# chzchzchz/raftsql

Hardware: AMD Instinct MI355X
Metric: quorum decisions/sec (commit+vote) across G groups (higher is better)
Workload: dtype u64

## Files before the change

### go/raftq/engine_more.go

```go
package raftq

import "C"

import "unsafe"

func ABIVersion() int { return int(C.raftq_abi_version()) }

func Quorum(peers uint32) uint32 { return uint32(C.raftq_quorum(C.uint32_t(peers))) }

func (e *Engine) NGroups() uint64 { return uint64(C.raftq_groups(e.h)) }
func (e *Engine) NPeers() uint32  { return uint32(C.raftq_peers(e.h)) }

func (e *Engine) SelfMax() (int, error) {
	var slot C.int32_t
	if err := e.err(C.raftq_self_max(e.h, &slot)); err != nil {
		return -1, err
	}
	return int(slot), nil
}

func (e *Engine) SetStream(stream unsafe.Pointer) error { return e.err(C.raftq_set_stream(e.h, stream)) }
func (e *Engine) Stream() unsafe.Pointer                { return C.raftq_get_stream(e.h) }

type TermDelta struct{ Group, CurTerm, FirstIdxCurTerm uint64 }

func (e *Engine) ApplyTermDeltas(d []TermDelta) error {
	if len(d) == 0 {
		return nil
	}
	return e.err(C.raftq_apply_term_deltas(e.h, (*C.raftq_term_delta_t)(unsafe.Pointer(&d[0])), C.uint64_t(len(d))))
}

func (e *Engine) CommitAdvance(gated bool, committedOut []uint64) (changed uint64, err error) {
	var p *C.uint64_t
	if committedOut != nil {
		p = (*C.uint64_t)(unsafe.Pointer(&committedOut[0]))
	}
	g := C.int(0)
	if gated {
		g = 1
	}
	var n C.uint64_t
	err = e.err(C.raftq_commit_advance(e.h, g, p, &n))
	return uint64(n), err
}

func (e *Engine) VoteTally(outcomeOut []uint8) (Counts, error) {
	var p *C.uint8_t
	if outcomeOut != nil {
		p = (*C.uint8_t)(unsafe.Pointer(&outcomeOut[0]))
	}
	var c C.raftq_counts_t
	if err := e.err(C.raftq_vote_tally(e.h, p, &c)); err != nil {
		return Counts{}, err
	}
	return Counts{uint64(c.n_changed), uint64(c.n_won), uint64(c.n_lost)}, nil
}

func (e *Engine) ReadVotes(out []uint8) error {
	return e.err(C.raftq_read_votes(e.h, (*C.uint8_t)(unsafe.Pointer(&out[0]))))
}

func (e *Engine) SetTimers(electionTick, heartbeatTick uint32, seed uint64) error {
	return e.err(C.raftq_set_timers(e.h, C.uint32_t(electionTick), C.uint32_t(heartbeatTick), C.uint64_t(seed)))
}

type TickCounts struct{ Hup, Beat uint64 }

func (e *Engine) Tick(wantCounts bool) (TickCounts, error) {
	var c C.raftq_tick_counts_t
	if !wantCounts {
		return TickCounts{}, e.err(C.raftq_tick(e.h, nil))
	}
	err := e.err(C.raftq_tick(e.h, &c))
	return TickCounts{uint64(c.n_hup), uint64(c.n_beat)}, err
}

func (e *Engine) CollectHups(out []uint64) (uint64, error) {
	var n C.uint64_t
	var p *C.uint64_t
	if len(out) > 0 {
		p = (*C.uint64_t)(unsafe.Pointer(&out[0]))
	}
	rc := C.raftq_collect_hups(e.h, p, C.uint64_t(len(out)), &n)
	return uint64(n), e.err(rc)
}

func (e *Engine) TickCollect(hups, beats []uint64) (nHup, nBeat uint64, err error) {
	var hp, bp *C.uint64_t
	if len(hups) > 0 {
		hp = (*C.uint64_t)(unsafe.Pointer(&hups[0]))
	}
	if len(beats) > 0 {
		bp = (*C.uint64_t)(unsafe.Pointer(&beats[0]))
	}
	var nh, nb C.uint64_t
	err = e.err(C.raftq_tick_collect(e.h, hp, C.uint64_t(len(hups)), &nh, bp, C.uint64_t(len(beats)), &nb))
	return uint64(nh), uint64(nb), err
}

const TickBeatBitmap = uint(C.RAFTQ_TICK_BEAT_BITMAP)

// ... 202 lines not shown
```

### include/raftq.h

```cpp
#ifndef RAFTQ_H
#define RAFTQ_H

#include <stddef.h>
#include <stdint.h>

#ifdef __cplusplus
extern "C" {
#endif

#define RAFTQ_ABI_VERSION 1
#define RAFTQ_MAX_PEERS 9

#define RAFTQ_OK 0
#define RAFTQ_EINVAL (-1)
#define RAFTQ_ENOMEM (-2)
#define RAFTQ_EHIP (-3)
#define RAFTQ_ESTATE (-4)
#define RAFTQ_ENODEV (-5)

#define RAFTQ_SWEEP_COMMIT 0x01u
#define RAFTQ_SWEEP_GATED 0x02u
#define RAFTQ_SWEEP_VOTES 0x04u
#define RAFTQ_SWEEP_NO_ADOPT 0x08u
#define RAFTQ_SWEEP_LDS 0x10u
// ... 14 lines not shown
typedef struct raftq_delta {
  uint64_t group;
  uint64_t match;
  uint32_t peer;
  uint32_t _pad;
} raftq_delta_t;

typedef struct raftq_vote_delta {
  uint64_t group;
  uint32_t peer;
  uint8_t vote;
  uint8_t _pad[3];
} raftq_vote_delta_t;

typedef struct raftq_term_delta {
  uint64_t group;
  uint64_t cur_term;
  uint64_t first_idx_cur_term;
} raftq_term_delta_t;

typedef struct raftq_advance {
  uint64_t group;
  uint64_t old_commit;
  uint64_t new_commit;
} raftq_advance_t;

typedef struct raftq_delta16 {
  uint64_t match;
  uint32_t group;
  uint32_t peer;
} raftq_delta16_t;
typedef struct raftq_advance16 {
  uint64_t new_commit;
  uint32_t group;
  uint32_t advanced_by;
} raftq_advance16_t;

int raftq_abi_version(void);
int raftq_device_count(int* n);
uint32_t raftq_quorum(uint32_t n_peers);

#define RAFTQ_MAX_GROUPS (1ull << 30)
int raftq_create(int device, uint64_t n_groups, uint32_t n_peers, raftq_t** out);
void raftq_destroy(raftq_t* h);
uint64_t raftq_groups(const raftq_t* h);
uint32_t raftq_peers(const raftq_t* h);
const char* raftq_last_error(const raftq_t* h);

int raftq_set_stream(raftq_t* h, void* stream);
void* raftq_get_stream(const raftq_t* h);

int raftq_load_match(raftq_t* h, const uint64_t* match ,
                     const uint64_t* committed );
int raftq_load_terms(raftq_t* h, const uint64_t* cur_term ,
                     const uint64_t* first_idx_cur_term );
int raftq_load_votes(raftq_t* h, const uint8_t* votes );

int raftq_apply_deltas(raftq_t* h, const raftq_delta_t* d, uint64_t n);
int raftq_apply_vote_deltas(raftq_t* h, const raftq_vote_delta_t* d, uint64_t n);
int raftq_apply_term_deltas(raftq_t* h, const raftq_term_delta_t* d, uint64_t n);

typedef struct raftq_voter_delta {
  uint64_t group;
  uint16_t voters;
  uint16_t reset;
  uint32_t _pad;
} raftq_voter_delta_t;
int raftq_load_voters(raftq_t* h, const uint16_t* voters);
int raftq_apply_voter_deltas(raftq_t* h, const raftq_voter_delta_t* d, uint64_t n);
int raftq_read_voters(raftq_t* h, uint16_t* voters_out);

int raftq_step_async(raftq_t* h, unsigned flags);
int raftq_wait(raftq_t* h, raftq_counts_t* counts);

int raftq_commit_advance(raftq_t* h, int gated, uint64_t* committed_out ,
                         uint64_t* n_changed );
int raftq_vote_tally(raftq_t* h, uint8_t* outcome_out ,
                     raftq_counts_t* counts );

int raftq_read_committed(raftq_t* h, uint64_t* committed_out );
int raftq_read_outcome(raftq_t* h, uint8_t* outcome_out );
int raftq_read_match(raftq_t* h, uint64_t* match_out );
int raftq_self_max(raftq_t* h, int32_t* slot_out);
int raftq_read_votes(raftq_t* h, uint8_t* votes_out );
int raftq_collect_changed(raftq_t* h, raftq_advance_t* out, uint64_t cap, uint64_t* n);

#define RAFTQ_ROLE_FOLLOWER 0
#define RAFTQ_ROLE_CANDIDATE 1
#define RAFTQ_ROLE_LEADER 2
typedef struct raftq_tick_counts {
  uint64_t n_hup;
  uint64_t n_beat;
} raftq_tick_counts_t;
int raftq_set_timers(raftq_t* h, uint32_t election_tick, uint32_t heartbeat_tick, uint64_t seed);
int raftq_load_roles(raftq_t* h, const uint8_t* role , const uint32_t* elapsed );
int raftq_tick(raftq_t* h, raftq_tick_counts_t* counts);
int raftq_read_tick(raftq_t* h, uint8_t* action , uint32_t* elapsed , uint8_t* role );
int raftq_collect_hups(raftq_t* h, uint64_t* groups, uint64_t cap, uint64_t* n);
int raftq_collect_beats(raftq_t* h, uint64_t* groups, uint64_t cap, uint64_t* n);
int raftq_tick_collect(raftq_t* h, uint64_t* hups, uint64_t hup_cap, uint64_t* n_hup, uint64_t* beats, uint64_t beat_cap,
                       uint64_t* n_beat);

#define RAFTQ_TICK_BEAT_BITMAP 1u
int raftq_tick_collect_lists(raftq_t* h, unsigned flags, uint64_t hup_cap, uint64_t beat_cap, uint64_t* n_hup, uint64_t* n_beat);
int raftq_last_tick_lists(raftq_t* h, const uint32_t** hups, uint64_t* n_hups, const uint32_t** beats, uint64_t* n_beats,
                          const uint64_t** beat_bitmap, uint64_t* bitmap_words);
int raftq_campaign(raftq_t* h, const uint64_t* groups, uint64_t n, uint32_t self_peer);

int raftq_cycle(raftq_t* h, const raftq_delta_t* deltas, uint64_t n_deltas,
                const raftq_vote_delta_t* vote_deltas, uint64_t n_vote_deltas, unsigned flags,
                raftq_advance_t* advances_out, uint64_t cap, uint64_t* n_advanced,
                raftq_counts_t* counts);

int raftq_stage(raftq_t* h, uint64_t n_deltas, uint64_t n_vote_deltas, raftq_delta_t** deltas,
                raftq_vote_delta_t** vote_deltas);
int raftq_last_advances(raftq_t* h, const raftq_advance_t** list, uint64_t* n_listed);

int raftq_cycle_packed(raftq_t* h, const raftq_delta16_t* deltas, uint64_t n_deltas,
                       const raftq_vote_delta_t* vote_deltas, uint64_t n_vote_deltas, unsigned flags,
                       raftq_advance16_t* advances_out, uint64_t cap, uint64_t* n_advanced,
                       raftq_counts_t* counts);
int raftq_stage_packed(raftq_t* h, uint64_t n_deltas, uint64_t n_vote_deltas, raftq_delta16_t** deltas,
                       raftq_vote_delta_t** vote_deltas);
int raftq_last_advances_packed(raftq_t* h, const raftq_advance16_t** list, uint64_t* n_listed);

#define RAFTQ_CYCLE_SEGMENTED 0x200u
int raftq_last_advance_segments(raftq_t* h, const raftq_advance16_t** recs, const uint32_t** counts, uint32_t* n_segments,
                                uint64_t* stride);

typedef struct raftq_set raftq_set_t;
#define RAFTQ_SET_GRID 0
#define RAFTQ_SET_PERSISTENT 1
int raftq_set_create(raftq_t* const* handles, uint32_t n, raftq_set_t** out);
void raftq_set_destroy(raftq_set_t* s);
uint32_t raftq_set_size(const raftq_set_t* s);
const char* raftq_set_last_error(const raftq_set_t* s);
void* raftq_set_get_stream(const raftq_set_t* s);
int raftq_set_mode(raftq_set_t* s, int mode, uint32_t persist_workgroups);
int raftq_set_sweep_async(raftq_set_t* s, unsigned flags);
int raftq_set_tick(raftq_set_t* s);
int raftq_set_wait(raftq_set_t* s, raftq_counts_t* per_member, raftq_counts_t* total);
int raftq_set_timer_begin(raftq_set_t* s);
int raftq_set_timer_end(raftq_set_t* s, float* elapsed_ms);
int raftq_sweep_many_async(raftq_t* const* handles, uint32_t n, unsigned flags);
int raftq_clone_state(raftq_t* dst, raftq_t* src);

int raftq_timer_begin(raftq_t* h);
int raftq_timer_end(raftq_t* h, float* elapsed_ms);

int raftq_host_alloc(void** p, uint64_t bytes);
void raftq_host_free(void* p);

#ifdef __cplusplus
}
#endif
#endif
```

### raftsql_amd/_lib.py

```python
from __future__ import annotations

import ctypes as C
import os

_HERE = os.path.dirname(os.path.abspath(__file__))
LIB_PATH = os.environ.get("RAFTQ_LIB") or os.path.join(_HERE, "libraftq.so")

RAFTQ_OK = 0
RAFTQ_EINVAL, RAFTQ_ENOMEM, RAFTQ_EHIP, RAFTQ_ESTATE, RAFTQ_ENODEV = -1, -2, -3, -4, -5

SWEEP_COMMIT = 0x01
SWEEP_GATED = 0x02
SWEEP_VOTES = 0x04
SWEEP_NO_ADOPT = 0x08
SWEEP_LDS = 0x10
SWEEP_CHANGED = 0x20
SWEEP_STREAM = 0x40
SWEEP_CACHED = 0x80
CYCLE_TRUSTED = 0x100
TICK_BEAT_BITMAP = 1
CYCLE_SEGMENTED = 0x200
SET_GRID, SET_PERSISTENT = 0, 1

MAX_PEERS = 9


class Counts(C.Structure):
    _fields_ = [("n_changed", C.c_uint64), ("n_won", C.c_uint64), ("n_lost", C.c_uint64)]


class TickCounts(C.Structure):
    _fields_ = [("n_hup", C.c_uint64), ("n_beat", C.c_uint64)]


class Delta(C.Structure):
    _fields_ = [("group", C.c_uint64), ("match", C.c_uint64), ("peer", C.c_uint32), ("_pad", C.c_uint32)]


class VoteDelta(C.Structure):
    _fields_ = [("group", C.c_uint64), ("peer", C.c_uint32), ("vote", C.c_uint8), ("_pad", C.c_uint8 * 3)]


class VoterDelta(C.Structure):
    _fields_ = [("group", C.c_uint64), ("voters", C.c_uint16), ("reset", C.c_uint16), ("_pad", C.c_uint32)]


class Advance(C.Structure):
    _fields_ = [("group", C.c_uint64), ("old_commit", C.c_uint64), ("new_commit", C.c_uint64)]


_H = C.c_void_p
_SIGS = [
    ("raftq_abi_version", C.c_int, []),
    ("raftq_device_count", C.c_int, [C.POINTER(C.c_int)]),
    ("raftq_quorum", C.c_uint32, [C.c_uint32]),
    ("raftq_create", C.c_int, [C.c_int, C.c_uint64, C.c_uint32, C.POINTER(_H)]),
    ("raftq_destroy", None, [_H]),
    ("raftq_groups", C.c_uint64, [_H]),
    ("raftq_peers", C.c_uint32, [_H]),
    ("raftq_last_error", C.c_char_p, [_H]),
    ("raftq_set_stream", C.c_int, [_H, C.c_void_p]),
    ("raftq_get_stream", C.c_void_p, [_H]),
    ("raftq_load_match", C.c_int, [_H, C.c_void_p, C.c_void_p]),
    ("raftq_load_terms", C.c_int, [_H, C.c_void_p, C.c_void_p]),
    ("raftq_load_votes", C.c_int, [_H, C.c_void_p]),
    ("raftq_apply_deltas", C.c_int, [_H, C.c_void_p, C.c_uint64]),
    ("raftq_apply_vote_deltas", C.c_int, [_H, C.c_void_p, C.c_uint64]),
    ("raftq_apply_term_deltas", C.c_int, [_H, C.c_void_p, C.c_uint64]),
    ("raftq_load_voters", C.c_int, [_H, C.c_void_p]),
    ("raftq_apply_voter_deltas", C.c_int, [_H, C.c_void_p, C.c_uint64]),
    ("raftq_read_voters", C.c_int, [_H, C.c_void_p]),
    ("raftq_step_async", C.c_int, [_H, C.c_uint]),
    ("raftq_wait", C.c_int, [_H, C.POINTER(Counts)]),
    ("raftq_commit_advance", C.c_int, [_H, C.c_int, C.c_void_p, C.POINTER(C.c_uint64)]),
    ("raftq_vote_tally", C.c_int, [_H, C.c_void_p, C.POINTER(Counts)]),
    ("raftq_read_committed", C.c_int, [_H, C.c_void_p]),
    ("raftq_read_outcome", C.c_int, [_H, C.c_void_p]),
    ("raftq_read_match", C.c_int, [_H, C.c_void_p]),
    ("raftq_self_max", C.c_int, [_H, C.POINTER(C.c_int32)]),
    ("raftq_read_votes", C.c_int, [_H, C.c_void_p]),
    ("raftq_collect_changed", C.c_int, [_H, C.c_void_p, C.c_uint64, C.POINTER(C.c_uint64)]),
    ("raftq_set_timers", C.c_int, [_H, C.c_uint32, C.c_uint32, C.c_uint64]),
    ("raftq_load_roles", C.c_int, [_H, C.c_void_p, C.c_void_p]),
    ("raftq_tick", C.c_int, [_H, C.POINTER(TickCounts)]),
    ("raftq_read_tick", C.c_int, [_H, C.c_void_p, C.c_void_p, C.c_void_p]),
    ("raftq_collect_hups", C.c_int, [_H, C.c_void_p, C.c_uint64, C.POINTER(C.c_uint64)]),
    ("raftq_collect_beats", C.c_int, [_H, C.c_void_p, C.c_uint64, C.POINTER(C.c_uint64)]),
    ("raftq_tick_collect", C.c_int, [_H, C.c_void_p, C.c_uint64, C.POINTER(C.c_uint64), C.c_void_p, C.c_uint64, C.POINTER(C.c_uint64)]),
    ("raftq_tick_collect_lists", C.c_int, [_H, C.c_uint, C.c_uint64, C.c_uint64, C.POINTER(C.c_uint64), C.POINTER(C.c_uint64)]),
    ("raftq_last_tick_lists", C.c_int, [_H, C.POINTER(C.c_void_p), C.POINTER(C.c_uint64), C.POINTER(C.c_void_p), C.POINTER(C.c_uint64),
                                        C.POINTER(C.c_void_p), C.POINTER(C.c_uint64)]),
    ("raftq_campaign", C.c_int, [_H, C.c_void_p, C.c_uint64, C.c_uint32]),
    ("raftq_cycle", C.c_int, [_H, C.c_void_p, C.c_uint64, C.c_void_p, C.c_uint64, C.c_uint, C.c_void_p, C.c_uint64,
                              C.POINTER(C.c_uint64), C.POINTER(Counts)]),
    ("raftq_stage", C.c_int, [_H, C.c_uint64, C.c_uint64, C.POINTER(C.c_void_p), C.POINTER(C.c_void_p)]),
    ("raftq_last_advances", C.c_int, [_H, C.POINTER(C.c_void_p), C.POINTER(C.c_uint64)]),
    ("raftq_cycle_packed", C.c_int, [_H, C.c_void_p, C.c_uint64, C.c_void_p, C.c_uint64, C.c_uint, C.c_void_p, C.c_uint64,
                                     C.POINTER(C.c_uint64), C.POINTER(Counts)]),
    ("raftq_stage_packed", C.c_int, [_H, C.c_uint64, C.c_uint64, C.POINTER(C.c_void_p), C.POINTER(C.c_void_p)]),
    ("raftq_last_advances_packed", C.c_int, [_H, C.POINTER(C.c_void_p), C.POINTER(C.c_uint64)]),
    ("raftq_last_advance_segments", C.c_int, [_H, C.POINTER(C.c_void_p), C.POINTER(C.c_void_p), C.POINTER(C.c_uint32), C.POINTER(C.c_uint64)]),
    ("raftq_set_create", C.c_int, [C.POINTER(_H), C.c_uint32, C.POINTER(_H)]),
    ("raftq_set_destroy", None, [_H]),
    ("raftq_set_size", C.c_uint32, [_H]),
    ("raftq_set_last_error", C.c_char_p, [_H]),
    ("raftq_set_get_stream", C.c_void_p, [_H]),
    ("raftq_set_mode", C.c_int, [_H, C.c_int, C.c_uint32]),
    ("raftq_set_sweep_async", C.c_int, [_H, C.c_uint]),
    ("raftq_set_wait", C.c_int, [_H, C.c_void_p, C.POINTER(Counts)]),
    ("raftq_set_tick", C.c_int, [_H]),
    ("raftq_set_timer_begin", C.c_int, [_H]),
    ("raftq_set_timer_end", C.c_int, [_H, C.POINTER(C.c_float)]),
    ("raftq_sweep_many_async", C.c_int, [C.POINTER(_H), C.c_uint32, C.c_uint]),
    ("raftq_clone_state", C.c_int, [_H, _H]),
    ("raftq_timer_begin", C.c_int, [_H]),
    ("raftq_timer_end", C.c_int, [_H, C.POINTER(C.c_float)]),
    ("raftq_host_alloc", C.c_int, [C.POINTER(C.c_void_p), C.c_uint64]),
    ("raftq_host_free", None, [C.c_void_p]),
]
EXPORTS = [s[0] for s in _SIGS]


class StepCounts(C.Structure):
    _fields_ = [("n_msgs", C.c_uint64), ("n_groups_touched", C.c_uint64)]


_STEP_SIGS = [
    ("raftq_set_self", C.c_int, [_H, C.c_uint32]),
    ("raftq_load_node", C.c_int, [_H, C.c_void_p, C.c_void_p, C.c_void_p, C.c_void_p, C.c_void_p]),
    ("raftq_read_node", C.c_int, [_H, C.c_void_p, C.c_void_p, C.c_void_p, C.c_void_p, C.c_void_p, C.c_void_p]),
    ("raftq_step_batch", C.c_int, [_H, C.c_void_p, C.c_uint64, C.c_void_p, C.POINTER(StepCounts)]),
    ("raftq_apply_log_deltas", C.c_int, [_H, C.c_void_p, C.c_uint64, C.c_void_p]),
    ("raftq_apply_log_deltas_nowait", C.c_int, [_H, C.c_void_p, C.c_uint64]),
    ("raftq_step_submit", C.c_int, [_H, C.c_void_p, C.c_uint64]),
    ("raftq_step_collect", C.c_int, [_H, C.c_void_p, C.POINTER(StepCounts)]),
    ("raftq_step_stage", C.c_int, [_H, C.c_uint64, C.POINTER(C.c_void_p)]),
    ("raftq_step_stage_packed", C.c_int, [_H, C.c_uint64, C.POINTER(C.c_void_p)]),
    ("raftq_step_submit_packed", C.c_int, [_H, C.c_void_p, C.c_uint64]),
    ("raftq_step_results", C.c_int, [_H, C.POINTER(C.c_void_p), C.POINTER(C.c_uint64)]),
    ("raftq_step_set_compact", C.c_int, [_H, C.c_int]),
    ("raftq_step_set_msg_flags", C.c_int, [_H, C.c_int]),
    ("raftq_step_set_voters", C.c_int, [_H, C.c_int]),
    ("raftq_step_results_c", C.c_int, [_H, C.POINTER(C.c_void_p), C.POINTER(C.c_uint64)]),
    ("raftq_step_results_s", C.c_int, [_H, C.POINTER(C.c_void_p), C.POINTER(C.c_uint64)]),
]
STEP_EXPORTS = [s[0] for s in _STEP_SIGS]



class WireCounts(C.Structure):
    _fields_ = [("n_msgs", C.c_uint64), ("n_ents", C.c_uint64), ("n_malformed", C.c_uint64), ("bytes", C.c_uint64)]


class WalCounts(C.Structure):
    _fields_ = [("n_recs", C.c_uint64), ("n_valid", C.c_uint64), ("bytes", C.c_uint64), ("last_crc", C.c_uint32),
                ("_pad", C.c_uint32)]


_WIRE_SIGS = [
    ("raftq_wire_encode", C.c_int, [_H, C.c_void_p, C.c_uint64, C.c_void_p, C.c_uint64, C.c_void_p, C.c_uint64, C.c_void_p,
                                    C.c_uint64, C.c_void_p, C.POINTER(WireCounts)]),
    ("raftq_wire_decode", C.c_int, [_H, C.c_void_p, C.c_uint64, C.c_void_p, C.c_uint64, C.c_void_p, C.c_void_p, C.c_uint64,
# ... 65 lines not shown
```

### raftsql_amd/csrc/raftq_capi.hip

```cpp
#include "raftq.h"

#include <hip/hip_runtime.h>

#include <algorithm>
#include <atomic>
#include <mutex>
#include <chrono>
#include <cstdlib>
#include <cstdio>
#include <cstring>
#include <new>
#include <string>
#include <unordered_set>
#include <vector>

#include "raftq_internal.hpp"

#ifndef RAFTQ_GPL
#define RAFTQ_GPL 4
#endif
#ifndef RAFTQ_AUTO_STREAM_BYTES
#define RAFTQ_AUTO_STREAM_BYTES (128ull << 20)
#endif
#ifndef RAFTQ_LDS_GPL
// ... 123 lines not shown

template <int N, bool COMMIT, bool GATED, bool VOTES>
hipError_t launch_voters_reg(const VoterSweepArgs& a, uint64_t gpad, int nt, hipStream_t s) {
  constexpr int G = voters_gpl(N);
  const dim3 grid((unsigned)(gpad / ((uint64_t)kBlock * G))), block(kBlock);
  if (nt == 3) hipLaunchKernelGGL((sweep_voters_kernel<N, G, COMMIT, GATED, VOTES, kLdNT | kStNT>), grid, block, 0, s, a);
  else if (nt == 1) hipLaunchKernelGGL((sweep_voters_kernel<N, G, COMMIT, GATED, VOTES, kLdNT>), grid, block, 0, s, a);
  else hipLaunchKernelGGL((sweep_voters_kernel<N, G, COMMIT, GATED, VOTES, 0>), grid, block, 0, s, a);
  return hipGetLastError();
}

template <int N>
hipError_t launch_voters_n(const VoterSweepArgs& a, uint64_t gpad, unsigned flags, int nt, hipStream_t s) {
  const bool commit = flags & (RAFTQ_SWEEP_COMMIT | RAFTQ_SWEEP_GATED);
  const bool gated = flags & RAFTQ_SWEEP_GATED;
  const bool votes = flags & RAFTQ_SWEEP_VOTES;
  if (commit && gated) return votes ? launch_voters_reg<N, true, true, true>(a, gpad, nt, s) : launch_voters_reg<N, true, true, false>(a, gpad, nt, s);
  if (commit) return votes ? launch_voters_reg<N, true, false, true>(a, gpad, nt, s) : launch_voters_reg<N, true, false, false>(a, gpad, nt, s);
  return launch_voters_reg<N, false, false, true>(a, gpad, nt, s);
}

hipError_t launch_voters(uint32_t N, const VoterSweepArgs& a, uint64_t gpad, unsigned flags, int nt, hipStream_t s) {
  switch (N) {
    case 1: return launch_voters_n<1>(a, gpad, flags, nt, s);
    case 2: return launch_voters_n<2>(a, gpad, flags, nt, s);
    case 3: return launch_voters_n<3>(a, gpad, flags, nt, s);
    case 4: return launch_voters_n<4>(a, gpad, flags, nt, s);
    case 5: return launch_voters_n<5>(a, gpad, flags, nt, s);
    case 6: return launch_voters_n<6>(a, gpad, flags, nt, s);
    case 7: return launch_voters_n<7>(a, gpad, flags, nt, s);
    case 8: return launch_voters_n<8>(a, gpad, flags, nt, s);
    case 9: return launch_voters_n<9>(a, gpad, flags, nt, s);
    default: return hipErrorInvalidValue;
  }
}

hipError_t launch_sweep(uint32_t N, const SweepLaunch& L, unsigned flags, int nt, hipStream_t s) {
  switch (N) {
    case 1: return launch_n<1>(L, flags, nt, s);
    case 2: return launch_n<2>(L, flags, nt, s);
    case 3: return launch_n<3>(L, flags, nt, s);
    case 4: return launch_n<4>(L, flags, nt, s);
    case 5: return launch_n<5>(L, flags, nt, s);
    case 6: return launch_n<6>(L, flags, nt, s);
    case 7: return launch_n<7>(L, flags, nt, s);
    case 8: return launch_n<8>(L, flags, nt, s);
    case 9: return launch_n<9>(L, flags, nt, s);
    default: return hipErrorInvalidValue;
  }
}

}
static inline void dense_changed(raftq_t* h) { h->node_mirror_fresh = false; }

int raftq_detail::ensure_staging(raftq_t* h, size_t bytes) {
  HIPCHK(h, h->stage.grow(bytes, std::max({bytes, h->stage.cap * 2, (size_t)1 << 20}), &h->stream));
  return RAFTQ_OK;
}

int raftq_detail::ensure_ingest(raftq_t* h, size_t bytes) {
  HIPCHK(h, h->ingest.grow(bytes, std::max({bytes, h->ingest.cap * 2, (size_t)1 << 20}), &h->stream, h->bar));
  return RAFTQ_OK;
}

namespace {
int ensure_adv(raftq_t* h, uint64_t entries) {
  const uint64_t have = h->adv.cap / sizeof(Advance);
  const uint64_t want = std::min<uint64_t>(std::max<uint64_t>({entries, have * 2, 4096}), h->gpad);
  HIPCHK(h, h->adv.grow(entries * sizeof(Advance), want * sizeof(Advance), &h->stream));
  return RAFTQ_OK;
}

}
int raftq_detail::self_max_check(raftq_t* h) {
  if (int rc = use_device(h)) return rc;
  if (h->step_collected != h->step_submitted) {
    HIPCHK(h, hipMemsetAsync(h->self_max, 0, sizeof(uint32_t), h->stream));
    return RAFTQ_OK;
  }
  HIPCHK(h, hipMemsetD32Async((hipDeviceptr_t)h->self_max, (int)(kSelfMaxValid | h->self_peer), 1, h->stream));
  const uint64_t blocks = std::min<uint64_t>((h->G + kBlock - 1) / kBlock, 4096);
  hipLaunchKernelGGL(self_max_check_kernel, dim3((unsigned)std::max<uint64_t>(blocks, 1)), dim3(kBlock), 0, h->stream,
                     (const uint64_t*)h->match, h->ld, h->G, h->N, h->self_peer, h->self_max);
  HIPCHK(h, hipGetLastError());
  return RAFTQ_OK;
}
int raftq_detail::use_device(raftq_t* h) {
  if (!h) return fail(nullptr, RAFTQ_EINVAL, "null handle");
  HIPCHK(h, hipSetDevice(h->device));
  return RAFTQ_OK;
}
int raftq_detail::use_device_idle(raftq_t* h, const char* who) {
  if (int rc = use_device(h)) return rc;
  if (h->step_collected != h->step_submitted)
    return fail(h, RAFTQ_ESTATE, std::string(who) + ": Step batches are in flight; collect them first");
  return RAFTQ_OK;
}
using raftq_detail::ensure_staging;
using raftq_detail::ensure_ingest;
using raftq_detail::use_device;
using raftq_detail::use_device_idle;
using raftq_detail::ensure_tick_state;

template <typename W>
static void pack_votes(const uint8_t* votes, uint64_t G, uint32_t N, W* out) {
  for (uint64_t g = 0; g < G; ++g) out[g] = 0;
  for (uint32_t p = 0; p < N; ++p) {
    const uint8_t* row = votes + (size_t)p * G;
    for (uint64_t g = 0; g < G; ++g) {
      const uint8_t v = row[g];
      out[g] = (W)(out[g] | (W)((v == 1 ? 1u : v == 2 ? 2u : 0u) << (2 * p)));
    }
  }
}
template <typename W>
static void unpack_votes(const W* in, uint64_t G, uint32_t N, uint8_t* votes) {
  for (uint32_t p = 0; p < N; ++p) {
    uint8_t* row = votes + (size_t)p * G;
    for (uint64_t g = 0; g < G; ++g) {
      const uint32_t f = ((uint32_t)in[g] >> (2 * p)) & 3u;
      row[g] = f == 3u ? 0 : (uint8_t)f;
    }
  }
}

extern "C" {

int raftq_abi_version(void) { return RAFTQ_ABI_VERSION; }

uint32_t raftq_quorum(uint32_t n_peers) { return n_peers / 2 + 1; }

int raftq_device_count(int* n) {
  if (!n) return fail(nullptr, RAFTQ_EINVAL, "raftq_device_count: null out");
  int c = 0;
  hipError_t e = hipGetDeviceCount(&c);
  if (e != hipSuccess) {
    *n = 0;
    return fail(nullptr, RAFTQ_ENODEV, std::string("hipGetDeviceCount: ") + hipGetErrorString(e));
  }
  *n = c;
  return RAFTQ_OK;
}

const char* raftq_last_error(const raftq_t* h) { return h ? h->err.c_str() : g_err.c_str(); }

uint64_t raftq_groups(const raftq_t* h) { return h ? h->G : 0; }
uint32_t raftq_peers(const raftq_t* h) { return h ? h->N : 0; }

int raftq_create(int device, uint64_t n_groups, uint32_t n_peers, raftq_t** out) {
  if (!out) return fail(nullptr, RAFTQ_EINVAL, "raftq_create: null out");
  *out = nullptr;
  if (n_groups == 0 || n_groups > RAFTQ_MAX_GROUPS)
    return fail(nullptr, RAFTQ_EINVAL, "raftq_create: n_groups out of range (1 .. RAFTQ_MAX_GROUPS = 2^30 per handle)");
  if (n_peers < 1 || n_peers > RAFTQ_MAX_PEERS) return fail(nullptr, RAFTQ_EINVAL, "raftq_create: n_peers must be 1..9");
  int ndev = 0;
  if (hipGetDeviceCount(&ndev) != hipSuccess || ndev <= 0)
    return fail(nullptr, RAFTQ_ENODEV, "raftq_create: no HIP device (this library has no CPU path)");
  if (device < 0 || device >= ndev) return fail(nullptr, RAFTQ_ENODEV, "raftq_create: device index out of range");
  raftq_t* h = new (std::nothrow) raftq();
  if (!h) return fail(nullptr, RAFTQ_ENOMEM, "raftq_create: host allocation failed");
  h->device = device;
  h->G = n_groups;
  h->N = n_peers;
  h->last_gpl = kGPL;
  h->gpad = (n_groups + kTileMax - 1) / kTileMax * kTileMax;
  h->ld = h->gpad + kRowStagger;
  const uint64_t ld = h->ld;
  h->max_partials = h->gpad / (kBlock * 2) * kWaves;
  int rc = RAFTQ_OK;
  do {
    if ((rc = use_device(h))) break;
    hipError_t e = hipStreamCreateWithFlags(&h->stream, hipStreamNonBlocking);
    if (e != hipSuccess) { rc = fail(h, RAFTQ_EHIP, std::string("hipStreamCreate: ") + hipGetErrorString(e)); break; }
    h->own_stream = true;
    {
      int large_bar = 0;
      (void)hipDeviceGetAttribute(&large_bar, hipDeviceAttributeIsLargeBar, device);
      const char* st = std::getenv("RAFTQ_STAGE");
      h->bar.staging = large_bar == 1 && !(st && std::strcmp(st, "host") == 0);
    }
    e = raftq_buf::alloc_group({{(void**)&h->match, (size_t)n_peers * ld * 8},
                                {(void**)&h->committed[0], ld * 8},
                                {(void**)&h->committed[1], ld * 8},
                                {(void**)&h->first_idx, ld * 8},
                                {(void**)&h->votes, (size_t)vote_word_bytes((int)n_peers) * ld},
                                {(void**)&h->outcome, ld / 4 + 64},
                                {(void**)&h->changed_bits, h->gpad / 8},
                                {(void**)&h->partials, h->max_partials * sizeof(uint4)},
                                {(void**)&h->offsets, (h->max_partials + 1) * 8},
                                {(void**)&h->self_max, 64}},
                               h->stream);
    if (e != hipSuccess) {
      rc = fail(h, e == hipErrorOutOfMemory ? RAFTQ_ENOMEM : RAFTQ_EHIP, std::string("device arrays: ") + hipGetErrorString(e));
      break;
    }
    e = hipMemsetD32Async((hipDeviceptr_t)h->self_max, (int)(kSelfMaxValid | 0u), 1, h->stream);
    if (e != hipSuccess) { rc = fail(h, RAFTQ_EHIP, std::string("hipMemsetD32Async: ") + hipGetErrorString(e)); break; }
    e = raftq_buf::alloc_group({{(void**)&h->h_partials, h->max_partials * sizeof(uint4), raftq_buf::Kind::pinned},
                                {(void**)&h->h_total, 64, raftq_buf::Kind::mapped_coherent, (void**)&h->d_total}},
                               h->stream);
    if (e != hipSuccess) { rc = fail(h, RAFTQ_ENOMEM, std::string("page-locked memory: ") + hipGetErrorString(e)); break; }
    e = hipEventCreate(&h->ev0);
    if (e == hipSuccess) e = hipEventCreate(&h->ev1);
    if (e != hipSuccess) { rc = fail(h, RAFTQ_EHIP, std::string("hipEventCreate: ") + hipGetErrorString(e)); break; }
    e = hipStreamSynchronize(h->stream);
    if (e != hipSuccess) { rc = fail(h, RAFTQ_EHIP, std::string("hipStreamSynchronize: ") + hipGetErrorString(e)); break; }
  } while (0);
  if (rc != RAFTQ_OK) {
    std::string keep = h->err;
    raftq_destroy(h);
    g_err = keep;
    return rc;
  }
  *out = h;
  return RAFTQ_OK;
}

void raftq_destroy(raftq_t* h) {
  if (!h) return;
  if (h->in_set) {
    raftq_set_t* s = h->in_set;
    s->broken = true;
    s->members.erase(std::remove(s->members.begin(), s->members.end(), h), s->members.end());
    (void)hipSetDevice(h->device);
    (void)hipStreamSynchronize(s->stream);
    h->stream = nullptr;
    h->own_stream = false;
  }
  if (h->prof_n && std::getenv("RAFTQ_PROFILE"))
    std::fprintf(stderr,
                 "[raftq] cycle phases, avg us over %llu calls: stage/validate %.1f | enqueue scatter %.1f | enqueue sweep "
                 "%.1f | enqueue collect %.1f | sync %.1f | copy-out %.1f | turns that ended in the blocking wait instead of the "
                 "polled flag: %llu\n",
                 (unsigned long long)h->prof_n, h->prof[0] / h->prof_n, h->prof[1] / h->prof_n, h->prof[2] / h->prof_n,
                 h->prof[3] / h->prof_n, h->prof[4] / h->prof_n, h->prof[5] / h->prof_n, (unsigned long long)h->flag_fallbacks);
  (void)hipSetDevice(h->device);
  if (h->stream) (void)hipStreamSynchronize(h->stream);
  if (h->many_aux) (void)hipStreamSynchronize(h->many_aux);
  raftq_detail::free_node_state(h);
  raftq_detail::free_wire_state(h);
  raftq_buf::free_device(h->match, h->committed[0], h->committed[1], h->first_idx, h->votes, h->voters, h->outcome, h->changed_bits,
                         h->partials, h->offsets, h->self_max, h->claim, h->delta_bad, h->role, h->elapsed, h->action, h->hup_bits,
                         h->beat_bits, h->tick_partials, h->tick_offsets2);
  raftq_buf::free_host(h->h_partials, h->h_total);
  if (h->ev0) (void)hipEventDestroy(h->ev0);
  if (h->ev1) (void)hipEventDestroy(h->ev1);
  if (h->many_aux) {
    (void)hipEventDestroy(h->many_fork);
    (void)hipEventDestroy(h->many_join);
  }
  const hipStream_t streams[4] = {h->many_aux, h->step_s_in, h->step_s_out, h->own_stream ? h->stream : nullptr};
  delete h;
  for (hipStream_t st : streams)
    if (st) (void)hipStreamDestroy(st);
}

int raftq_set_stream(raftq_t* h, void* stream) {
  if (int rc = use_device_idle(h, "raftq_set_stream")) return rc;
  if (h->in_set) return fail(h, RAFTQ_ESTATE, "raftq_set_stream: the handle is a member of a sweep set, which owns its stream");
  HIPCHK(h, hipStreamSynchronize(h->stream));
  if (h->own_stream) HIPCHK(h, hipStreamDestroy(h->stream));
  h->stream = (hipStream_t)stream;
  h->own_stream = false;
  return RAFTQ_OK;
}

void* raftq_get_stream(const raftq_t* h) { return h ? (void*)h->stream : nullptr; }

int raftq_load_match(raftq_t* h, const uint64_t* match, const uint64_t* committed) {
  if (int rc = use_device_idle(h, "raftq_load_match")) return rc;
  if (!match && !committed) return fail(h, RAFTQ_EINVAL, "raftq_load_match: nothing to load");
  if (match) {
    for (uint32_t p = 0; p < h->N; ++p)
      HIPCHK(h, hipMemcpyAsync(h->match + (size_t)p * h->ld, match + (size_t)p * h->G, h->G * 8, hipMemcpyHostToDevice, h->stream));
    if (int rc = raftq_detail::self_max_check(h)) return rc;
  }
  dense_changed(h);
  if (committed)
    HIPCHK(h, hipMemcpyAsync(h->committed[h->cur], committed, h->G * 8, hipMemcpyHostToDevice, h->stream));
  HIPCHK(h, hipStreamSynchronize(h->stream));
  return RAFTQ_OK;
}

int raftq_load_terms(raftq_t* h, const uint64_t* cur_term, const uint64_t* first_idx_cur_term) {
  if (int rc = use_device_idle(h, "raftq_load_terms")) return rc;
  if (!cur_term || !first_idx_cur_term) return fail(h, RAFTQ_EINVAL, "raftq_load_terms: null argument");
  std::vector<uint64_t> f;
  try {
    f.assign(first_idx_cur_term, first_idx_cur_term + h->G);
  } catch (...) {
    return fail(h, RAFTQ_ENOMEM, "raftq_load_terms: host allocation failed");
  }
  for (uint64_t g = 0; g < h->G; ++g)
    if (cur_term[g] == 0) f[g] = 0;
  HIPCHK(h, hipMemcpyAsync(h->first_idx, f.data(), h->G * 8, hipMemcpyHostToDevice, h->stream));
  dense_changed(h);
  HIPCHK(h, hipStreamSynchronize(h->stream));
  h->have_terms = true;
  return RAFTQ_OK;
}

int raftq_load_votes(raftq_t* h, const uint8_t* votes) {
  if (int rc = use_device_idle(h, "raftq_load_votes")) return rc;
  if (!votes) return fail(h, RAFTQ_EINVAL, "raftq_load_votes: null argument");
  const size_t wb = (size_t)vote_word_bytes((int)h->N);
  std::vector<uint8_t> packed;
  try {
    packed.resize(h->G * wb);
  } catch (...) {
    return fail(h, RAFTQ_ENOMEM, "raftq_load_votes: host allocation failed");
  }
  if (wb == 2) pack_votes(votes, h->G, h->N, reinterpret_cast<uint16_t*>(packed.data()));
  else pack_votes(votes, h->G, h->N, reinterpret_cast<uint32_t*>(packed.data()));
  HIPCHK(h, hipMemcpyAsync(h->votes, packed.data(), packed.size(), hipMemcpyHostToDevice, h->stream));
  HIPCHK(h, hipStreamSynchronize(h->stream));
  return RAFTQ_OK;
}

static int ensure_delta_dev(raftq_t* h, size_t bytes) {
  if (!h->delta_bad) HIPCHK(h, raftq_buf::alloc_zeroed((void**)&h->delta_bad, 64, h->stream));
  HIPCHK(h, h->delta_dev.grow(bytes, std::max(bytes * 2, (size_t)1 << 20), &h->stream));
  return RAFTQ_OK;
}

static int check_deltas(raftq_t* h, bool trusted = false) {
  int rc = RAFTQ_OK;
  const char* what = trusted ? "; that record was dropped, every other record of the turn was applied (RAFTQ_CYCLE_TRUSTED)"
                             : "; nothing applied";
  if (h->delta_check[0] && h->h_total[1] == h->delta_check[0])
    rc = fail(h, RAFTQ_EINVAL, std::string("a match delta is out of range (group >= G or peer >= N)") + what);
  if (h->delta_check[1] && h->h_total[2] == h->delta_check[1])
    rc = fail(h, RAFTQ_EINVAL, std::string("a vote delta is invalid (group/peer out of range or vote not 1/2)") + what);
  h->delta_check[0] = h->delta_check[1] = 0;
  return rc;
}

}

template <typename Rec, typename AbiRec>
static int enqueue_ingest(raftq_t* h, const AbiRec* d, uint64_t n, const raftq_vote_delta_t* vd, uint64_t nv, size_t off_votes,
                          bool trusted = false) {
  static_assert(sizeof(Rec) == sizeof(AbiRec), "ABI struct mismatch");
  static_assert(sizeof(VoteDeltaRec) == sizeof(raftq_vote_delta_t), "ABI struct mismatch");
  if (nv > 0xfffffffeull) return fail(h, RAFTQ_EINVAL, "vote delta batch too large");
  auto inside = [&](const void* q) {
    return (const uint8_t*)q >= (const uint8_t*)h->ingest.h && (const uint8_t*)q < (const uint8_t*)h->ingest.h + h->ingest.cap;
  };
  if (n) {
    AbiRec* dst = (AbiRec*)h->ingest.h;
    if ((const void*)d != (const void*)dst) {
      if (inside(d)) return fail(h, RAFTQ_EINVAL, "match deltas staged with other counts / another record layout than this call's");
      std::memcpy(dst, d, (size_t)n * sizeof(AbiRec));
    }
  }
  if (nv) {
    raftq_vote_delta_t* dst = (raftq_vote_delta_t*)((uint8_t*)h->ingest.h + off_votes);
    if ((const void*)vd != (const void*)dst) {
      if (inside(vd)) return fail(h, RAFTQ_EINVAL, "vote deltas staged with other counts / another record layout than this call's");
      std::memcpy(dst, vd, (size_t)nv * sizeof(raftq_vote_delta_t));
    }
    if (!h->claim) {
      HIPCHK(h, raftq_buf::alloc_filled((void**)&h->claim, (size_t)h->N * h->ld * sizeof(uint32_t), 0xff, h->stream));
    }
  }
  h->ingest.publish();
  if (int rc = ensure_delta_dev(h, h->ingest.cap)) return rc;
  const unsigned long long em = n ? ++h->delta_epoch : kNoEpoch, ev = nv ? ++h->delta_epoch : kNoEpoch;
  h->delta_check[0] = n ? em : 0;
  h->delta_check[1] = nv ? ev : 0;
  Rec* dev_m = (Rec*)h->delta_dev.d;
  VoteDeltaRec* dev_v = (VoteDeltaRec*)((uint8_t*)h->delta_dev.d + off_votes);
  const unsigned long long* bad = h->delta_bad;
  const dim3 gm((unsigned)((n + kBlock - 1) / kBlock)), gv((unsigned)((nv + kBlock - 1) / kBlock));
  if (n) dense_changed(h);
  if (n && trusted)
    hipLaunchKernelGGL((deltas_in_apply_kernel<Rec>), gm, dim3(kBlock), 0, h->stream, (const Rec*)h->ingest.d, n, h->match, h->ld,
                       h->G, h->N, h->delta_bad, h->d_total + 1, em, h->self_max);
  else if (n)
    hipLaunchKernelGGL((deltas_in_kernel<Rec>), gm, dim3(kBlock), 0, h->stream, (const Rec*)h->ingest.d, dev_m, n, h->G, h->N,
                       h->delta_bad, h->d_total + 1, em);
  if (nv)
    hipLaunchKernelGGL(vote_deltas_in_kernel, gv, dim3(kBlock), 0, h->stream,
                       (const VoteDeltaRec*)((uint8_t*)h->ingest.d + off_votes), dev_v, nv, h->G, h->N, h->delta_bad + 1,
                       h->d_total + 2, ev);
  if (n && !trusted)
    hipLaunchKernelGGL((apply_deltas_kernel<Rec>), gm, dim3(kBlock), 0, h->stream, h->match, h->ld, (const Rec*)dev_m, n, bad, em,
                       ev, h->self_max);
  if (nv) {
    const unsigned long long em_gate = trusted ? kNoEpoch : em;
    hipLaunchKernelGGL(vote_claim_kernel, gv, dim3(kBlock), 0, h->stream, h->claim, h->ld, (const VoteDeltaRec*)dev_v, nv, bad,
                       em_gate, ev, h->G, h->N, trusted ? 1 : 0);
    hipLaunchKernelGGL(vote_apply_kernel, gv, dim3(kBlock), 0, h->stream, h->votes, h->N > 8 ? 1 : 0, h->claim, h->ld,
                       (const VoteDeltaRec*)dev_v, nv, bad, em_gate, ev, h->G, h->N, trusted ? 1 : 0);
  }
  HIPCHK(h, hipGetLastError());
  return RAFTQ_OK;
}

extern "C" {

int raftq_apply_deltas(raftq_t* h, const raftq_delta_t* d, uint64_t n) {
  if (int rc = use_device_idle(h, "raftq_apply_deltas")) return rc;
  if (n == 0) return RAFTQ_OK;
  if (!d) return fail(h, RAFTQ_EINVAL, "raftq_apply_deltas: null argument");
  if (int rc = ensure_ingest(h, (size_t)n * sizeof(raftq_delta_t))) return rc;
  if (int rc = enqueue_ingest<DeltaRec>(h, d, n, nullptr, 0, 0)) return rc;
  HIPCHK(h, hipStreamSynchronize(h->stream));
  return check_deltas(h);
}

int raftq_apply_term_deltas(raftq_t* h, const raftq_term_delta_t* d, uint64_t n) {
  static_assert(sizeof(TermDeltaRec) == sizeof(raftq_term_delta_t), "ABI struct mismatch");
  if (int rc = use_device_idle(h, "raftq_apply_term_deltas")) return rc;
  if (n == 0) return RAFTQ_OK;
  if (!d) return fail(h, RAFTQ_EINVAL, "raftq_apply_term_deltas: null argument");
  for (uint64_t i = 0; i < n; ++i)
    if (d[i].group >= h->G) return fail(h, RAFTQ_EINVAL, "a term delta is out of range; nothing applied");
  if (int rc = ensure_staging(h, (size_t)n * sizeof(raftq_term_delta_t))) return rc;
  raftq_term_delta_t* dst = (raftq_term_delta_t*)h->stage.h;
  uint64_t m = 0;
  {
    std::unordered_set<uint64_t> seen;
    seen.reserve((size_t)n * 2);
    std::vector<uint64_t> keep;
    keep.reserve(n);
    for (uint64_t i = n; i-- > 0;)
      if (seen.insert(d[i].group).second) keep.push_back(i);
    for (auto it = keep.rbegin(); it != keep.rend(); ++it) dst[m++] = d[*it];
  }
  const dim3 grid((unsigned)((m + kBlock - 1) / kBlock));
  dense_changed(h);
  hipLaunchKernelGGL(apply_term_deltas_kernel, grid, dim3(kBlock), 0, h->stream, h->first_idx,
                     (const TermDeltaRec*)h->stage.d, m);
  HIPCHK(h, hipGetLastError());
  HIPCHK(h, hipStreamSynchronize(h->stream));
  h->have_terms = true;
  return RAFTQ_OK;
}

int raftq_apply_vote_deltas(raftq_t* h, const raftq_vote_delta_t* d, uint64_t n) {
  if (int rc = use_device_idle(h, "raftq_apply_vote_deltas")) return rc;
  if (n == 0) return RAFTQ_OK;
  if (!d) return fail(h, RAFTQ_EINVAL, "raftq_apply_vote_deltas: null argument");
  if (int rc = ensure_ingest(h, (size_t)n * sizeof(raftq_vote_delta_t))) return rc;
  if (int rc = enqueue_ingest<DeltaRec>(h, (const raftq_delta_t*)nullptr, 0, d, n, 0)) return rc;
  HIPCHK(h, hipStreamSynchronize(h->stream));
  return check_deltas(h);
}

}

static int ensure_voters(raftq_t* h) {
  if (h->voters) return RAFTQ_OK;
  HIPCHK(h, raftq_buf::alloc_zeroed((void**)&h->voters, h->ld * sizeof(uint16_t), h->stream));
  return RAFTQ_OK;
}
static int drop_voters(raftq_t* h) {
  if (!h->voters) return RAFTQ_OK;
  HIPCHK(h, hipStreamSynchronize(h->stream));
  raftq_buf::free_device(h->voters);
  return RAFTQ_OK;
}
static int voters_not_in_set(raftq_t* h, const char* who) {
  if (!h->in_set) return RAFTQ_OK;
  return fail(h, RAFTQ_ESTATE, std::string(who) + ": the handle is a member of a sweep set, whose dispatches count every slot "
                                                  "(voter masks on set members are out of scope)");
}
int raftq_detail::refuse_voters(raftq_t* h, const char* who, bool step_family) {
  if (!h || !h->voters) return RAFTQ_OK;
  if (h->step_voters) {
    if (step_family) return RAFTQ_OK;
    return fail(h, RAFTQ_ESTATE, std::string(who) + ": the handle has voter masks loaded; the broadcasts built on the device go to N - 1 slots, "
                                                    "not to a group's membership (out of scope, whatever raftq_step_set_voters says)");
  }
  return fail(h, RAFTQ_ESTATE, std::string(who) + ": the handle has voter masks loaded; Step's maybeCommit / poll on the device "
                                                  "count every slot (out of scope: raftq_load_voters(h, NULL) first)");
}

extern "C" {

int raftq_load_voters(raftq_t* h, const uint16_t* voters) {
  if (int rc = use_device_idle(h, "raftq_load_voters")) return rc;
  if (int rc = voters_not_in_set(h, "raftq_load_voters")) return rc;
  if (!voters) return drop_voters(h);
  const uint32_t beyond = 0xffffu & ~((1u << h->N) - 1u);
  for (uint64_t g = 0; g < h->G; ++g)
    if (voters[g] & beyond) return fail(h, RAFTQ_EINVAL, "raftq_load_voters: a mask names a peer slot >= N; nothing loaded");
  if (int rc = ensure_voters(h)) return rc;
  HIPCHK(h, hipMemcpyAsync(h->voters, voters, h->G * sizeof(uint16_t), hipMemcpyHostToDevice, h->stream));
  HIPCHK(h, hipStreamSynchronize(h->stream));
  return RAFTQ_OK;
}

int raftq_read_voters(raftq_t* h, uint16_t* voters_out) {
  if (int rc = use_device_idle(h, "raftq_read_voters")) return rc;
  if (!voters_out) return fail(h, RAFTQ_EINVAL, "raftq_read_voters: null argument");
  if (!h->voters) {
    std::fill(voters_out, voters_out + h->G, (uint16_t)((1u << h->N) - 1u));
    return RAFTQ_OK;
  }
  HIPCHK(h, hipMemcpyAsync(voters_out, h->voters, h->G * sizeof(uint16_t), hipMemcpyDeviceToHost, h->stream));
  HIPCHK(h, hipStreamSynchronize(h->stream));
  return RAFTQ_OK;
}

int raftq_apply_voter_deltas(raftq_t* h, const raftq_voter_delta_t* d, uint64_t n) {
  static_assert(sizeof(VoterDeltaRec) == sizeof(raftq_voter_delta_t), "ABI struct mismatch");
  if (int rc = use_device_idle(h, "raftq_apply_voter_deltas")) return rc;
  if (int rc = voters_not_in_set(h, "raftq_apply_voter_deltas")) return rc;
  if (n == 0) return RAFTQ_OK;
  if (!d) return fail(h, RAFTQ_EINVAL, "raftq_apply_voter_deltas: null argument");
  const uint32_t beyond = 0xffffu & ~((1u << h->N) - 1u);
  for (uint64_t i = 0; i < n; ++i)
    if (d[i].group >= h->G || ((d[i].voters | d[i].reset) & beyond))
      return fail(h, RAFTQ_EINVAL, "a voter delta is out of range (group >= G or a bit >= N); nothing applied");
  if (int rc = ensure_staging(h, (size_t)n * sizeof(raftq_voter_delta_t))) return rc;
  raftq_voter_delta_t* dst = (raftq_voter_delta_t*)h->stage.h;
  uint64_t m = 0;
  try {
    std::unordered_set<uint64_t> seen;
    seen.reserve((size_t)n * 2);
    std::vector<uint64_t> keep;
    keep.reserve(n);
    for (uint64_t i = n; i-- > 0;)
      if (seen.insert(d[i].group).second) keep.push_back(i);
    for (auto it = keep.rbegin(); it != keep.rend(); ++it) dst[m++] = d[*it];
  } catch (...) {
    return fail(h, RAFTQ_ENOMEM, "raftq_apply_voter_deltas: host allocation failed");
  }
  if (!h->voters) {
    if (int rc = ensure_voters(h)) return rc;
    hipLaunchKernelGGL(fill_voters_kernel, dim3((unsigned)((h->G + kBlock - 1) / kBlock)), dim3(kBlock), 0, h->stream, h->voters, h->G,
                       (uint16_t)((1u << h->N) - 1u));
    HIPCHK(h, hipGetLastError());
  }
  dense_changed(h);
  hipLaunchKernelGGL(apply_voter_deltas_kernel, dim3((unsigned)((m + kBlock - 1) / kBlock)), dim3(kBlock), 0, h->stream, h->voters, h->match,
                     h->ld, h->votes, h->N > 8 ? 1 : 0, h->N, (const VoterDeltaRec*)h->stage.d, m, h->self_max);
  HIPCHK(h, hipGetLastError());
  HIPCHK(h, hipStreamSynchronize(h->stream));
  return RAFTQ_OK;
}

static int sweep_check(raftq_t* h, unsigned flags, const char* who) {
  const unsigned known = RAFTQ_SWEEP_COMMIT | RAFTQ_SWEEP_GATED | RAFTQ_SWEEP_VOTES | RAFTQ_SWEEP_NO_ADOPT |
                         RAFTQ_SWEEP_LDS | RAFTQ_SWEEP_CHANGED | RAFTQ_SWEEP_STREAM | RAFTQ_SWEEP_CACHED;
  const std::string w(who);
  if (flags & ~known) return fail(h, RAFTQ_EINVAL, w + ": unknown flag");
  const bool commit = flags & (RAFTQ_SWEEP_COMMIT | RAFTQ_SWEEP_GATED);
  const bool votes = flags & RAFTQ_SWEEP_VOTES;
  if (!commit && !votes) return fail(h, RAFTQ_EINVAL, w + ": nothing to sweep");
  if ((flags & RAFTQ_SWEEP_GATED) && !h->have_terms)
    return fail(h, RAFTQ_ESTATE, w + ": gated sweep before raftq_load_terms");
  if ((flags & RAFTQ_SWEEP_STREAM) && (flags & RAFTQ_SWEEP_CACHED))
    return fail(h, RAFTQ_EINVAL, w + ": RAFTQ_SWEEP_STREAM and RAFTQ_SWEEP_CACHED are exclusive");
  if ((flags & RAFTQ_SWEEP_CHANGED) && !commit)
    return fail(h, RAFTQ_EINVAL, w + ": RAFTQ_SWEEP_CHANGED needs a commit sweep");
  if ((flags & RAFTQ_SWEEP_LDS) && h->voters)
    return fail(h, RAFTQ_EINVAL, w + ": RAFTQ_SWEEP_LDS has no form for a handle with voter masks loaded (the A/B variant counts every slot)");
  return RAFTQ_OK;
}

static SweepArgs sweep_args(const raftq_t* h, int cur, bool want_bits) {
  SweepArgs a;
  a.match = h->match;
  a.committed = h->committed[cur];
  a.committed_out = h->committed[cur ^ 1];
  a.first_idx = h->first_idx;
  a.votes = h->votes;
  a.outcome = h->outcome;
  a.changed_bits = want_bits ? h->changed_bits : nullptr;
  a.partials = h->partials;
  a.ld = h->ld;
  a.self_max = h->self_max;
  return a;
}

static uint64_t sweep_footprint(const raftq_t* h) { return h->ld * (8ull * h->N + 24 + vote_word_bytes((int)h->N) + 1 + (h->voters ? 2 : 0)); }

static int sweep_policy(unsigned flags, uint64_t footprint) {
  const bool stream = (flags & RAFTQ_SWEEP_STREAM) ? true
                      : (flags & RAFTQ_SWEEP_CACHED) ? false
                                                     : footprint >= RAFTQ_AUTO_STREAM_BYTES;
  return !stream ? 0 : footprint >= RAFTQ_AUTO_STREAM_BYTES ? 3 : 1;
}

static void sweep_done(raftq_t* h, unsigned flags, int gpl) {
  const bool commit = flags & (RAFTQ_SWEEP_COMMIT | RAFTQ_SWEEP_GATED);
  h->n_partials = h->gpad / ((uint64_t)kBlock * gpl) * kWaves;
  h->last_flags = flags;
  h->last_gpl = gpl;
  if (commit) {
    h->last_old = h->committed[h->cur];
    h->last_new = h->committed[h->cur ^ 1];
    if (!(flags & RAFTQ_SWEEP_NO_ADOPT)) {
      h->cur ^= 1;
      dense_changed(h);
    }
  }
}

static int sweep_on(raftq_t* h, unsigned flags, hipStream_t s, const char* who) {
  if (int rc = use_device_idle(h, who)) return rc;
  if (int rc = sweep_check(h, flags, who)) return rc;
  const bool commit = flags & (RAFTQ_SWEEP_COMMIT | RAFTQ_SWEEP_GATED);
  const SweepArgs a = sweep_args(h, h->cur, flags & RAFTQ_SWEEP_CHANGED);
  if (h->voters) {
    VoterSweepArgs va;
    va.s = a;
    va.voters = h->voters;
    HIPCHK(h, launch_voters(h->N, va, h->gpad, flags, sweep_policy(flags, sweep_footprint(h)), s));
    sweep_done(h, flags, voters_gpl((int)h->N));
    return RAFTQ_OK;
  }
  const bool lds = (flags & RAFTQ_SWEEP_LDS) && commit;
  SweepLaunch L;
  L.one = &a;
  L.gpad = h->gpad;
  HIPCHK(h, launch_sweep(h->N, L, flags, sweep_policy(flags, sweep_footprint(h)), s));
  sweep_done(h, flags, lds ? kLdsGPL : kGPL);
  return RAFTQ_OK;
}

int raftq_step_async(raftq_t* h, unsigned flags) {
  if (!h) return fail(nullptr, RAFTQ_EINVAL, "null handle");
  return sweep_on(h, flags, h->stream, "raftq_step_async");
}


int raftq_sweep_many_async(raftq_t* const* handles, uint32_t n, unsigned flags) {
  if (!handles && n) return fail(nullptr, RAFTQ_EINVAL, "raftq_sweep_many_async: null handle array");
  bool alternate = n >= 2;
  for (uint32_t i = 0; alternate && i < n; ++i) {
    if (!handles[i] || handles[i]->stream != handles[0]->stream || handles[i]->device != handles[0]->device) alternate = false;
    for (uint32_t j = 0; alternate && j < i; ++j)
      if (handles[j] == handles[i]) alternate = false;
  }
  if (!alternate) {
    for (uint32_t i = 0; i < n; ++i)
      if (int rc = raftq_step_async(handles[i], flags)) return rc;
    return RAFTQ_OK;
  }
  raftq_t* h0 = handles[0];
  if (int rc = use_device(h0)) return rc;
  if (!h0->many_aux) {
    HIPCHK(h0, hipStreamCreateWithFlags(&h0->many_aux, hipStreamNonBlocking));
    HIPCHK(h0, hipEventCreateWithFlags(&h0->many_fork, hipEventDisableTiming));
    HIPCHK(h0, hipEventCreateWithFlags(&h0->many_join, hipEventDisableTiming));
  }
  HIPCHK(h0, hipEventRecord(h0->many_fork, h0->stream));
  HIPCHK(h0, hipStreamWaitEvent(h0->many_aux, h0->many_fork, 0));
  int rc = RAFTQ_OK;
  for (uint32_t i = 0; i < n && rc == RAFTQ_OK; ++i)
    rc = sweep_on(handles[i], flags, (i & 1) ? h0->many_aux : h0->stream, "raftq_sweep_many_async");
  HIPCHK(h0, hipEventRecord(h0->many_join, h0->many_aux));
  HIPCHK(h0, hipStreamWaitEvent(h0->stream, h0->many_join, 0));
  return rc;
}

int raftq_wait(raftq_t* h, raftq_counts_t* counts) {
  if (int rc = use_device_idle(h, "raftq_wait")) return rc;
  if (counts) {
    if (h->n_partials == 0) return fail(h, RAFTQ_ESTATE, "raftq_wait: no sweep to report on");
    HIPCHK(h, hipMemcpyAsync(h->h_partials, h->partials, h->n_partials * sizeof(uint4), hipMemcpyDeviceToHost, h->stream));
  }
  HIPCHK(h, hipStreamSynchronize(h->stream));
  if (counts) {
    uint64_t c = 0, w = 0, l = 0;
    for (uint64_t i = 0; i < h->n_partials; ++i) {
      c += h->h_partials[i].x;
      w += h->h_partials[i].y;
      l += h->h_partials[i].z;
    }
    const bool commit = h->last_flags & (RAFTQ_SWEEP_COMMIT | RAFTQ_SWEEP_GATED);
    const bool votes = h->last_flags & RAFTQ_SWEEP_VOTES;
    counts->n_changed = commit ? c : 0;
    counts->n_won = votes ? w : 0;
    counts->n_lost = votes ? l : 0;
  }
  return RAFTQ_OK;
}

int raftq_read_committed(raftq_t* h, uint64_t* out) {
  if (int rc = use_device_idle(h, "raftq_read_committed")) return rc;
  if (!out) return fail(h, RAFTQ_EINVAL, "raftq_read_committed: null argument");
  const uint64_t* src = (h->last_flags & RAFTQ_SWEEP_NO_ADOPT) && h->last_new ? h->last_new : h->committed[h->cur];
  HIPCHK(h, hipMemcpyAsync(out, src, h->G * 8, hipMemcpyDeviceToHost, h->stream));
  HIPCHK(h, hipStreamSynchronize(h->stream));
  return RAFTQ_OK;
}

int raftq_read_outcome(raftq_t* h, uint8_t* out) {
  if (int rc = use_device_idle(h, "raftq_read_outcome")) return rc;
  if (!out) return fail(h, RAFTQ_EINVAL, "raftq_read_outcome: null argument");
  std::vector<uint8_t> packed;
  try {
    packed.resize((h->G + 3) / 4);
  } catch (...) {
    return fail(h, RAFTQ_ENOMEM, "raftq_read_outcome: host allocation failed");
  }
  HIPCHK(h, hipMemcpyAsync(packed.data(), h->outcome, packed.size(), hipMemcpyDeviceToHost, h->stream));
  HIPCHK(h, hipStreamSynchronize(h->stream));
  for (uint64_t g = 0; g < h->G; ++g) out[g] = (uint8_t)((packed[g >> 2] >> (2 * (g & 3))) & 3u);
  return RAFTQ_OK;
}

int raftq_self_max(raftq_t* h, int32_t* slot) {
  if (int rc = use_device_idle(h, "raftq_self_max")) return rc;
  if (!slot) return fail(h, RAFTQ_EINVAL, "raftq_self_max: null argument");
  uint32_t w = 0;
  HIPCHK(h, hipMemcpyAsync(&w, h->self_max, sizeof w, hipMemcpyDeviceToHost, h->stream));
  HIPCHK(h, hipStreamSynchronize(h->stream));
  *slot = (w & kSelfMaxValid) ? (int32_t)(w & 0xffu) : -1;
  return RAFTQ_OK;
}

int raftq_read_match(raftq_t* h, uint64_t* out) {
  if (int rc = use_device_idle(h, "raftq_read_match")) return rc;
  if (!out) return fail(h, RAFTQ_EINVAL, "raftq_read_match: null argument");
  for (uint32_t p = 0; p < h->N; ++p)
    HIPCHK(h, hipMemcpyAsync(out + (size_t)p * h->G, h->match + (size_t)p * h->ld, h->G * 8, hipMemcpyDeviceToHost, h->stream));
  HIPCHK(h, hipStreamSynchronize(h->stream));
  return RAFTQ_OK;
}

int raftq_read_votes(raftq_t* h, uint8_t* out) {
  if (int rc = use_device_idle(h, "raftq_read_votes")) return rc;
  if (!out) return fail(h, RAFTQ_EINVAL, "raftq_read_votes: null argument");
  const size_t wb = (size_t)vote_word_bytes((int)h->N);
  std::vector<uint8_t> packed;
  try {
    packed.resize(h->G * wb);
  } catch (...) {
    return fail(h, RAFTQ_ENOMEM, "raftq_read_votes: host allocation failed");
  }
  HIPCHK(h, hipMemcpyAsync(packed.data(), h->votes, packed.size(), hipMemcpyDeviceToHost, h->stream));
  HIPCHK(h, hipStreamSynchronize(h->stream));
  if (wb == 2) unpack_votes(reinterpret_cast<const uint16_t*>(packed.data()), h->G, h->N, out);
  else unpack_votes(reinterpret_cast<const uint32_t*>(packed.data()), h->G, h->N, out);
  return RAFTQ_OK;
}

int raftq_commit_advance(raftq_t* h, int gated, uint64_t* committed_out, uint64_t* n_changed) {
  if (int rc = raftq_step_async(h, gated ? (RAFTQ_SWEEP_COMMIT | RAFTQ_SWEEP_GATED) : RAFTQ_SWEEP_COMMIT)) return rc;
  raftq_counts_t c;
  if (int rc = raftq_wait(h, &c)) return rc;
  if (n_changed) *n_changed = c.n_changed;
  if (committed_out) return raftq_read_committed(h, committed_out);
  return RAFTQ_OK;
}

int raftq_vote_tally(raftq_t* h, uint8_t* outcome_out, raftq_counts_t* counts) {
  if (int rc = raftq_step_async(h, RAFTQ_SWEEP_VOTES)) return rc;
  raftq_counts_t c;
  if (int rc = raftq_wait(h, &c)) return rc;
  if (counts) *counts = c;
  if (outcome_out) return raftq_read_outcome(h, outcome_out);
  return RAFTQ_OK;
}

}

int raftq_detail::ensure_tick_state(raftq_t* h) {
  if (h->role) return RAFTQ_OK;
  HIPCHK(h, raftq_buf::alloc_group({{(void**)&h->role, h->ld},
                                    {(void**)&h->elapsed, h->ld * 4},
                                    {(void**)&h->action, h->ld},
                                    {(void**)&h->hup_bits, h->gpad / 8},
                                    {(void**)&h->beat_bits, h->gpad / 8},
                                    {(void**)&h->tick_partials, h->gpad / 256 * sizeof(uint4)}},
                                   h->stream));
  return RAFTQ_OK;
}

static int ensure_tick_offsets2(raftq_t* h, uint64_t nw);
static hipError_t wait_turn(raftq_t* h, uint64_t flag_epoch, int kind = 0);

extern "C" {

int raftq_set_timers(raftq_t* h, uint32_t election_tick, uint32_t heartbeat_tick, uint64_t seed) {
  if (!h) return fail(nullptr, RAFTQ_EINVAL, "null handle");
  if (election_tick == 0 || heartbeat_tick == 0)
    return fail(h, RAFTQ_EINVAL, "raftq_set_timers: ticks must be >= 1");
  h->election_tick = election_tick;
  h->heartbeat_tick = heartbeat_tick;
  h->tick_seed = seed;
  return RAFTQ_OK;
}

int raftq_load_roles(raftq_t* h, const uint8_t* role, const uint32_t* elapsed) {
  if (int rc = use_device_idle(h, "raftq_load_roles")) return rc;
  if (!role) return fail(h, RAFTQ_EINVAL, "raftq_load_roles: null role array");
  for (uint64_t g = 0; g < h->G; ++g)
    if (role[g] > RAFTQ_ROLE_LEADER) return fail(h, RAFTQ_EINVAL, "raftq_load_roles: role must be 0, 1 or 2");
  if (int rc = ensure_tick_state(h)) return rc;
  HIPCHK(h, hipMemcpyAsync(h->role, role, h->G, hipMemcpyHostToDevice, h->stream));
// ... 698 lines not shown
  auto bail = [&](int rc) {
    std::string keep = s->err;
    raftq_set_destroy(s);
    g_set_err = keep;
    return rc;
  };
  hipError_t e = hipSetDevice(s->device);
  if (e == hipSuccess) e = hipStreamCreateWithFlags(&s->stream, hipStreamNonBlocking);
  for (int k = 0; k < 3 && e == hipSuccess; ++k) e = hipMalloc((void**)&s->tab[k], (size_t)n * sizeof(SweepArgs));
  if (e == hipSuccess) e = hipMalloc((void**)&s->counts_d, (size_t)n * 32);
  if (e == hipSuccess) e = hipMalloc((void**)&s->np_d, (size_t)n * 8);
  if (e == hipSuccess) e = hipHostMalloc((void**)&s->counts_h, (size_t)n * 32, hipHostMallocDefault);
  if (e == hipSuccess) e = hipEventCreate(&s->ev0);
  if (e == hipSuccess) e = hipEventCreate(&s->ev1);
  if (e != hipSuccess)
    return bail(sfail(s, e == hipErrorOutOfMemory ? RAFTQ_ENOMEM : RAFTQ_EHIP, std::string("raftq_set_create: ") + hipGetErrorString(e)));
  for (uint32_t i = 0; i < n; ++i) {
    raftq_t* h = handles[i];
    e = hipStreamSynchronize(h->stream);
    if (e == hipSuccess && h->own_stream) e = hipStreamDestroy(h->stream);
    if (e != hipSuccess) return bail(sfail(s, RAFTQ_EHIP, std::string("raftq_set_create: ") + hipGetErrorString(e)));
    h->stream = s->stream;
    h->own_stream = false;
    h->in_set = s;
    s->members.push_back(h);
  }
  for (int cur = 0; cur < 2; ++cur) {
    set_fill_table(s, cur, s->tab_host);
    e = hipMemcpy(s->tab[cur], s->tab_host.data(), (size_t)n * sizeof(SweepArgs), hipMemcpyHostToDevice);
    if (e != hipSuccess) return bail(sfail(s, RAFTQ_EHIP, std::string("raftq_set_create: ") + hipGetErrorString(e)));
  }
  int cus = 0;
  (void)hipDeviceGetAttribute(&cus, hipDeviceAttributeMultiprocessorCount, s->device);
  s->persist_wgs = (uint32_t)std::max(cus, 1) * 3u;
  *out = s;
  return RAFTQ_OK;
}

void raftq_set_destroy(raftq_set_t* s) {
  if (!s) return;
  (void)hipSetDevice(s->device);
  if (s->stream) (void)hipStreamSynchronize(s->stream);
  for (raftq_t* h : s->members) {
    h->in_set = nullptr;
    h->stream = nullptr;
    h->own_stream = false;
    if (hipStreamCreateWithFlags(&h->stream, hipStreamNonBlocking) == hipSuccess) h->own_stream = true;
  }
  for (int k = 0; k < 3; ++k) (void)hipFree(s->tab[k]);
  (void)hipFree(s->counts_d);
  (void)hipFree(s->np_d);
  (void)hipFree(s->tick_tab);
  if (s->counts_h) (void)hipHostFree(s->counts_h);
  if (s->ev0) (void)hipEventDestroy(s->ev0);
  if (s->ev1) (void)hipEventDestroy(s->ev1);
  if (s->stream) (void)hipStreamDestroy(s->stream);
  delete s;
}

uint32_t raftq_set_size(const raftq_set_t* s) { return s ? (uint32_t)s->members.size() : 0; }
const char* raftq_set_last_error(const raftq_set_t* s) { return s ? s->err.c_str() : g_set_err.c_str(); }
void* raftq_set_get_stream(const raftq_set_t* s) { return s ? (void*)s->stream : nullptr; }

int raftq_set_mode(raftq_set_t* s, int mode, uint32_t persist_workgroups) {
  if (!s) return sfail(nullptr, RAFTQ_EINVAL, "raftq_set_mode: null set");
  if (mode != RAFTQ_SET_GRID && mode != RAFTQ_SET_PERSISTENT) return sfail(s, RAFTQ_EINVAL, "raftq_set_mode: unknown mode");
  s->mode = mode;
  if (persist_workgroups) s->persist_wgs = persist_workgroups;
  return RAFTQ_OK;
}

int raftq_set_sweep_async(raftq_set_t* s, unsigned flags) {
  if (int rc = set_ready(s, "raftq_set_sweep_async")) return rc;
  if (flags & RAFTQ_SWEEP_LDS) return sfail(s, RAFTQ_EINVAL, "raftq_set_sweep_async: RAFTQ_SWEEP_LDS sweeps one handle at a time");
  uint64_t footprint = 0;
  int cur = s->members[0]->cur;
  for (raftq_t* h : s->members) {
    if (h->step_collected != h->step_submitted)
      return sfail(s, RAFTQ_ESTATE, "raftq_set_sweep_async: a member has Step batches in flight; collect them first");
    if (int rc = sweep_check(h, flags, "raftq_set_sweep_async")) return sfail(s, rc, h->err);
    footprint += sweep_footprint(h);
    if (h->cur != cur) cur = -1;
  }
  const SweepArgs* tab = s->tab[cur < 0 ? 2 : cur];
  if (cur < 0) {
    set_fill_table(s, -1, s->tab_host);
    SETCHK(s, hipMemcpyAsync(s->tab[2], s->tab_host.data(), s->tab_host.size() * sizeof(SweepArgs), hipMemcpyHostToDevice,
                             s->stream));
  }
  SweepLaunch L;
  L.tab = tab;
  L.members = (uint32_t)s->members.size();
  L.want_bits = (flags & RAFTQ_SWEEP_CHANGED) ? 1u : 0u;
  L.persist_wgs = s->mode == RAFTQ_SET_PERSISTENT ? s->persist_wgs : 0u;
  L.gpad = s->gpad;
  int nt = sweep_policy(flags, footprint);
  if (nt == 1) nt = 3;
  SETCHK(s, launch_sweep(s->N, L, flags, nt, s->stream));
  const int gpl = s->mode == RAFTQ_SET_PERSISTENT ? kGPL : set_gpl((int)s->N);
  for (raftq_t* h : s->members) sweep_done(h, flags, gpl);
  s->swept = true;
  s->last_flags = flags;
  return RAFTQ_OK;
}

int raftq_set_tick(raftq_set_t* s) {
  if (int rc = set_ready(s, "raftq_set_tick")) return rc;
  const size_t K = s->members.size();
  bool stale = s->tick_tab == nullptr || s->tick_host.size() != K;
  for (size_t m = 0; m < K; ++m) {
    raftq_t* h = s->members[m];
    if (h->step_collected != h->step_submitted)
      return sfail(s, RAFTQ_ESTATE, "raftq_set_tick: a member has Step batches in flight; collect them first");
    const bool fresh = h->role == nullptr;
    if (int rc = ensure_tick_state(h)) return sfail(s, rc, h->err);
    if (stale || fresh) {
      stale = true;
      continue;
    }
    const TickArgs now = tick_args(h, h->tick_no), &was = s->tick_host[m];
    if (now.role != was.role || now.seed != was.seed || now.election_tick != was.election_tick || now.heartbeat_tick != was.heartbeat_tick ||
        now.tick_no != was.tick_no + s->tick_since)
      stale = true;
  }
  if (stale) {
    if (!s->tick_tab) SETCHK(s, hipMalloc((void**)&s->tick_tab, K * sizeof(TickArgs)));
    s->tick_host.resize(K);
    for (size_t m = 0; m < K; ++m) s->tick_host[m] = tick_args(s->members[m], s->members[m]->tick_no);
    SETCHK(s, hipMemcpyAsync(s->tick_tab, s->tick_host.data(), K * sizeof(TickArgs), hipMemcpyHostToDevice, s->stream));
    s->tick_since = 0;
  }
  const uint64_t n_blocks = s->gpad / 1024;
  int shape_now = 1;
  if (const char* e = std::getenv("RAFTQ_TICK_SHAPE"))
    shape_now = std::strcmp(e, "narrow") == 0 ? 0 : std::strcmp(e, "wide2") == 0 ? 2 : std::strcmp(e, "wide4") == 0 ? 4 : 1;
  auto wide_grid = [&](int r) { return dim3((unsigned)((n_blocks + (uint64_t)kWaves * r - 1) / ((uint64_t)kWaves * r)), (unsigned)K); };
  switch (shape_now) {
    case 0:
      hipLaunchKernelGGL(tick_set_kernel, dim3((unsigned)((n_blocks + kTickSetRounds - 1) / kTickSetRounds), (unsigned)K), dim3(kBlock), 0, s->stream,
                         (const TickArgs*)s->tick_tab, s->tick_since, n_blocks);
      break;
    case 2:
      hipLaunchKernelGGL((tick_set_wide_kernel<2>), wide_grid(2), dim3(kBlock), 0, s->stream, (const TickArgs*)s->tick_tab, s->tick_since, n_blocks);
      break;
    case 4:
      hipLaunchKernelGGL((tick_set_wide_kernel<4>), wide_grid(4), dim3(kBlock), 0, s->stream, (const TickArgs*)s->tick_tab, s->tick_since, n_blocks);
      break;
    default:
      hipLaunchKernelGGL((tick_set_wide_kernel<kTickWideBlocks>), wide_grid(kTickWideBlocks), dim3(kBlock), 0, s->stream, (const TickArgs*)s->tick_tab,
                         s->tick_since, n_blocks);
  }
  SETCHK(s, hipGetLastError());
  ++s->tick_since;
  for (raftq_t* h : s->members) {
    h->tl_valid = false;
    ++h->tick_no;
    h->ticked = true;
  }
  return RAFTQ_OK;
}

int raftq_set_wait(raftq_set_t* s, raftq_counts_t* per_member, raftq_counts_t* total) {
  if (int rc = set_ready(s, "raftq_set_wait")) return rc;
  const bool want = per_member || total;
  const size_t n = s->members.size();
  if (want) {
    if (!s->swept) return sfail(s, RAFTQ_ESTATE, "raftq_set_wait: no set sweep to report on");
    set_fill_table(s, -1, s->tab_host);
    SETCHK(s, hipMemcpyAsync(s->tab[2], s->tab_host.data(), n * sizeof(SweepArgs), hipMemcpyHostToDevice, s->stream));
    s->np_host.resize(n);
    for (size_t i = 0; i < n; ++i) s->np_host[i] = s->members[i]->n_partials;
    SETCHK(s, hipMemcpyAsync(s->np_d, s->np_host.data(), n * 8, hipMemcpyHostToDevice, s->stream));
    hipLaunchKernelGGL(set_counts_kernel, dim3((unsigned)n), dim3(kBlock), 0, s->stream, (const SweepArgs*)s->tab[2],
                       (const uint64_t*)s->np_d, s->counts_d);
    SETCHK(s, hipGetLastError());
    SETCHK(s, hipMemcpyAsync(s->counts_h, s->counts_d, n * 32, hipMemcpyDeviceToHost, s->stream));
  }
  SETCHK(s, hipStreamSynchronize(s->stream));
  if (want) {
    raftq_counts_t t{0, 0, 0};
    for (size_t i = 0; i < n; ++i) {
      const unsigned f = s->members[i]->last_flags;
      const bool commit = f & (RAFTQ_SWEEP_COMMIT | RAFTQ_SWEEP_GATED);
      const bool votes = f & RAFTQ_SWEEP_VOTES;
      raftq_counts_t c{commit ? s->counts_h[4 * i] : 0, votes ? s->counts_h[4 * i + 1] : 0, votes ? s->counts_h[4 * i + 2] : 0};
      if (per_member) per_member[i] = c;
      t.n_changed += c.n_changed;
      t.n_won += c.n_won;
      t.n_lost += c.n_lost;
    }
    if (total) *total = t;
  }
  return RAFTQ_OK;
}

int raftq_set_timer_begin(raftq_set_t* s) {
  if (int rc = set_ready(s, "raftq_set_timer_begin")) return rc;
  SETCHK(s, hipEventRecord(s->ev0, s->stream));
  return RAFTQ_OK;
}

int raftq_set_timer_end(raftq_set_t* s, float* elapsed_ms) {
  if (int rc = set_ready(s, "raftq_set_timer_end")) return rc;
  if (!elapsed_ms) return sfail(s, RAFTQ_EINVAL, "raftq_set_timer_end: null argument");
  SETCHK(s, hipEventRecord(s->ev1, s->stream));
  SETCHK(s, hipEventSynchronize(s->ev1));
  SETCHK(s, hipEventElapsedTime(elapsed_ms, s->ev0, s->ev1));
  return RAFTQ_OK;
}

int raftq_clone_state(raftq_t* dst, raftq_t* src) {
  if (int rc = use_device_idle(dst, "raftq_clone_state")) return rc;
  if (!src) return fail(dst, RAFTQ_EINVAL, "raftq_clone_state: null source");
  if (src == dst) return RAFTQ_OK;
  if (src->device != dst->device || src->N != dst->N || src->G != dst->G)
    return fail(dst, RAFTQ_EINVAL, "raftq_clone_state: source and destination must have the same device, groups and peers");
  if (src->step_collected != src->step_submitted)
    return fail(dst, RAFTQ_ESTATE, "raftq_clone_state: the source has Step batches in flight");
  if (src->voters && dst->in_set)
    return fail(dst, RAFTQ_ESTATE, "raftq_clone_state: the source has voter masks loaded and the destination is a member of a sweep "
                                   "set, whose dispatches count every slot (out of scope)");
  if (src->voters) {
    if (int rc = ensure_voters(dst)) return rc;
  } else if (int rc = drop_voters(dst)) {
    return rc;
  }
  HIPCHK(dst, hipStreamSynchronize(src->stream));
  const uint64_t ld = dst->ld;
  HIPCHK(dst, hipMemcpyAsync(dst->match, src->match, (size_t)dst->N * ld * 8, hipMemcpyDeviceToDevice, dst->stream));
  HIPCHK(dst, hipMemcpyAsync(dst->committed[dst->cur], src->committed[src->cur], ld * 8, hipMemcpyDeviceToDevice, dst->stream));
  HIPCHK(dst, hipMemcpyAsync(dst->first_idx, src->first_idx, ld * 8, hipMemcpyDeviceToDevice, dst->stream));
  HIPCHK(dst, hipMemcpyAsync(dst->votes, src->votes, (size_t)vote_word_bytes((int)dst->N) * ld, hipMemcpyDeviceToDevice,
                             dst->stream));
  HIPCHK(dst, hipMemcpyAsync(dst->self_max, src->self_max, sizeof(uint32_t), hipMemcpyDeviceToDevice, dst->stream));
  if (src->voters) HIPCHK(dst, hipMemcpyAsync(dst->voters, src->voters, ld * sizeof(uint16_t), hipMemcpyDeviceToDevice, dst->stream));
  HIPCHK(dst, hipStreamSynchronize(dst->stream));
  dst->have_terms = src->have_terms;
  dense_changed(dst);
  return RAFTQ_OK;
}

}
```

### raftsql_amd/csrc/raftq_internal.hpp

```cpp
#pragma once
#include <hip/hip_runtime.h>

#include <string>
#include <vector>

#include "raftq.h"
#include "raftq_wire.h"
#include "raftq_kernels.hpp"
#include "raftq_buffers.hpp"

struct raftq {
  int device = 0;
  uint64_t G = 0, gpad = 0, ld = 0;
  uint32_t N = 0;
  hipStream_t stream = nullptr;
  bool own_stream = false;
  struct raftq_set* in_set = nullptr;
  uint64_t* match = nullptr;
  uint64_t* committed[2] = {nullptr, nullptr};
  int cur = 0;
  uint64_t* first_idx = nullptr;
  uint8_t* votes = nullptr;
  uint16_t* voters = nullptr;
  uint8_t* outcome = nullptr;
  uint64_t* changed_bits = nullptr;
  uint4* partials = nullptr;
  uint4* h_partials = nullptr;
  uint64_t n_partials = 0;
  uint64_t max_partials = 0;
  uint64_t* offsets = nullptr;
  uint64_t* h_total = nullptr;
  raftq_buf::Buffer<> stage{raftq_buf::Kind::mapped};
  raftq_buf::HostWritable ingest;
  raftq_buf::BarRule bar;
  std::vector<uint64_t> ld_mark, ld_start;
  struct LdNowait {
    raftq_buf::Buffer<> buf{raftq_buf::Kind::mapped};
    hipEvent_t ev = nullptr;
  };
  LdNowait ld_nowait[2];
  uint32_t ld_nowait_next = 0;
  std::vector<uint32_t> ld_round, ld_pos;
  uint32_t ld_epoch = 0;
  raftq_buf::Buffer<raftqk::Advance> adv{raftq_buf::Kind::mapped_coherent};
  uint64_t adv_listed = 0;
  bool adv_packed = false;
  bool adv_segmented = false;
  raftq_buf::Buffer<uint32_t> seg_h{raftq_buf::Kind::mapped_coherent};
  raftq_buf::Buffer<unsigned int> seg_d{raftq_buf::Kind::device};
  uint32_t seg_tiles = 0, seg_stride = 0, seg_one = 0;
  uint64_t flag_mask = ~0ull;
  uint32_t* self_max = nullptr;
  uint64_t compact_epoch = 0;
  uint64_t compact_epoch_armed = 0;
  uint32_t flag_misses[2] = {0, 0}, flag_rested[2] = {0, 0};
  uint64_t flag_fallbacks = 0;
  uint32_t* claim = nullptr;
  raftq_buf::Buffer<> delta_dev{raftq_buf::Kind::device};
  unsigned long long* delta_bad = nullptr;
  unsigned long long delta_epoch = 0;
  unsigned long long delta_check[2] = {0, 0};
  uint8_t* role = nullptr;
  uint32_t* elapsed = nullptr;
  uint8_t* action = nullptr;
  uint64_t* hup_bits = nullptr;
  uint64_t* beat_bits = nullptr;
  uint4* tick_partials = nullptr;
  raftq_buf::Buffer<uint32_t> tl{raftq_buf::Kind::mapped_coherent};
  uint64_t tl_hup_cap = 0, tl_beat_cap = 0, tl_beat_at = 0, tl_map_off = 0;
  uint64_t tl_n_hup = 0, tl_n_beat = 0;
  unsigned tl_flags = 0;
  bool tl_valid = false;
  uint64_t* tick_offsets2 = nullptr;
  uint32_t election_tick = 10, heartbeat_tick = 1;
  uint64_t tick_seed = 0x1000, tick_no = 0;
  bool ticked = false;
  uint64_t* d_total = nullptr;
  bool have_terms = false;
  unsigned last_flags = 0;
  int last_gpl = 0;
  const uint64_t* last_old = nullptr;
  const uint64_t* last_new = nullptr;
  uint32_t self_peer = 0;
  bool self_set = false;
  bool node_mirror_fresh = false;
  uint64_t node_mirror_refreshes = 0;
  void* node_rec = nullptr;
  unsigned int* step_stall = nullptr;
  uint8_t step_compact = 0;
  bool step_msg_flags = false;
  bool step_voters = false;
  int step_walk_mode = 1;
  uint32_t step_stalls_in_a_row = 0, step_sorted_left = 0;
  uint64_t step_replays = 0;
  static constexpr int kStepSlots = 3;
  struct StepSlot {
    raftq_buf::Buffer<> in_h{raftq_buf::Kind::pinned};
    raftq_buf::HostWritable in_bar;
    raftq_buf::Buffer<> dev{raftq_buf::Kind::device};
    raftq_buf::Buffer<> out{raftq_buf::Kind::mapped};
    uint64_t n = 0;
    hipEvent_t ev_in = nullptr, ev_out = nullptr;
    bool busy = false;
    bool lists = false;
    bool replayed = false;
    bool copy_pending = false;
    const void* w_off_in_place = nullptr;
    const void* w_stream_in_place = nullptr;
    size_t w_stage_stream_off = 0;
    const void* msgs_in_place = nullptr;
    const void* outs_d = nullptr;
    uint64_t out_quads = 0;
    int end_bit = 0;
    uint32_t rec = 64;
    bool tail_zeroed = false;
    uint64_t tail_n = 0;
    uint32_t tail_rec = 0;
    const void* tail_dev = nullptr;
    uint64_t w_nbytes = 0;
    bool wire = false;
    uint8_t recs = 0;
    void* w_msgs_d = nullptr;
    void* w_ents_d = nullptr;
    const uint64_t* w_ent_total_d = nullptr;
    uint64_t w_ents_cap = 0;
    raftq_buf::Buffer<> w_pin{raftq_buf::Kind::pinned};
    bool w_msgs_fetched = false, w_ents_fetched = false;
    uint64_t w_n_ents = 0;
  } step_slot[kStepSlots];
  int step_last_slot = -1;
  uint64_t step_submitted = 0, step_collected = 0;
  hipStream_t step_s_in = nullptr, step_s_out = nullptr;
  bool step_defer_copy = true;
  const void* step_last_out = nullptr;
  uint64_t step_last_n = 0;
  uint32_t step_last_rec = 64;
  hipEvent_t ev0 = nullptr, ev1 = nullptr;
  hipStream_t many_aux = nullptr;
  hipEvent_t many_fork = nullptr, many_join = nullptr;
  raftq_buf::Buffer<> wire_dev{raftq_buf::Kind::device};
  raftq_buf::Buffer<> wire_out{raftq_buf::Kind::device};
  uint64_t* wire_pin = nullptr;
  uint64_t* wire_pin_d = nullptr;
  unsigned long long* wire_flags = nullptr;
  raftq_buf::Buffer<unsigned long long> wire_lb{raftq_buf::Kind::device};
  uint64_t wire_lb_tiles = 0;
  uint32_t wire_ticket_base = 0, wire_epoch = 0;
  uint32_t wire_chunk_base = 0, wire_chunk_pending = 0;
  bool wire_chunk_unknown = false;
  unsigned int prop_stamp = 0;
  raftq_buf::Buffer<> resp_dev{raftq_buf::Kind::device};
  bool resp_on = false;
  uint32_t resp_stamp = 0;
  const uint64_t* resp_at_tail_d = nullptr;
  bool wal_pending = false, wal_pending_done = false;
  bool wal_pending_waited = false;
  uint64_t wal_pending_n = 0, wal_pending_cap = 0;
  uint32_t wal_pending_prev = 0;
  int wal_pending_rc = 0;
  raftq_wal_counts_t wal_pending_counts{};
  std::string wal_pending_err;
  std::string err;
  double prof[6] = {0, 0, 0, 0, 0, 0};
  uint64_t prof_n = 0;
};


struct raftq_set {
  int device = 0;
  uint32_t N = 0;
  uint64_t gpad = 0;
  std::vector<raftq_t*> members;
  hipStream_t stream = nullptr;
  raftqk::SweepArgs* tab[3] = {nullptr, nullptr, nullptr};
  std::vector<raftqk::SweepArgs> tab_host;
  uint64_t* counts_d = nullptr;
  uint64_t* np_d = nullptr;
  std::vector<uint64_t> np_host;
  uint64_t* counts_h = nullptr;
  bool swept = false;
  bool broken = false;
  unsigned last_flags = 0;
  int mode = 0;
  uint32_t persist_wgs = 0;
  hipEvent_t ev0 = nullptr, ev1 = nullptr;
  raftqk::TickArgs* tick_tab = nullptr;
  std::vector<raftqk::TickArgs> tick_host;
  uint64_t tick_since = 0;
  std::string err;
};


struct raftq_wire_counts;
namespace raftqk {
struct NodeArrays;
}
namespace raftq_detail {
int node_arrays_of(raftq_t* h, raftqk::NodeArrays* out);
int fail(raftq_t* h, int code, const std::string& msg);
int use_device(raftq_t* h);
int use_device_idle(raftq_t* h, const char* who);
int refuse_voters(raftq_t* h, const char* who, bool step_family = false);
int self_max_check(raftq_t* h);
int ensure_staging(raftq_t* h, size_t bytes);
int ensure_ingest(raftq_t* h, size_t bytes);
int ensure_tick_state(raftq_t* h);
void free_node_state(raftq_t* h);
void free_wire_state(raftq_t* h);
struct PackedDst {
  int form;
  uint32_t head_types;
  void* wide;
  uint64_t wide_cap;
};
int wire_frames_enqueue(raftq_t* h, const void* stream, uint64_t nbytes, const uint64_t* frame_off, uint64_t n, void* msgs, void* ents,
                        uint64_t ents_cap, void* msgs_d, int tail_appends, void* zero2 ,
                        const PackedDst* packed = nullptr);
uint64_t wire_frames_n_wide(raftq_t* h);
int wire_frames_finish(raftq_t* h, const uint64_t* frame_off, uint64_t n, bool have_ents, uint64_t ents_cap, ::raftq_wire_counts* counts);
struct RespPlan {
  uint64_t n = 0, n_max = 0, cap = 0;
  void* v_out = nullptr;
  uint64_t* v_resp_off = nullptr;
  uint64_t* peer_off = nullptr;
};
int respond_prepare(raftq_t* h, const void* stream, uint64_t nbytes, const uint64_t* frame_off, const void* msgs, const void* ents,
                    const uint64_t* at_tail, void* out, uint64_t cap, uint64_t* resp_off, uint64_t* peer_off, uint64_t n, RespPlan* p);
int respond_enqueue(raftq_t* h, const RespPlan& p);
int respond_finish(raftq_t* h, const RespPlan& p, ::raftq_wire_counts* resp_counts);
struct TickLists {
  unsigned flags;
  uint64_t cap_h, cap_b, beat_at, map_off;
  const uint64_t* off_beat;
  const uint64_t* off_h = nullptr;
};
int tick_lists_prepare(raftq_t* h, const char* who, unsigned flags, uint64_t hup_cap, uint64_t beat_cap, TickLists* tl);
int tick_lists_enqueue(raftq_t* h, TickLists* tl);
int tick_lists_finish(raftq_t* h, const char* who, const TickLists& tl, uint64_t* n_hup, uint64_t* n_beat);
int node_records_of(raftq_t* h, const char* who, raftqk::NodeArrays* out);
int respond_pass_ok(raftq_t* h);
hipError_t wait_call(raftq_t* h);
}

#define HIPCHK(h, expr)                                                                        \
  do {                                                                                         \
    hipError_t _e = (expr);                                                                    \
    if (_e != hipSuccess) {                                                                    \
      return raftq_detail::fail((h), _e == hipErrorOutOfMemory ? RAFTQ_ENOMEM : RAFTQ_EHIP,    \
                                std::string(#expr) + ": " + hipGetErrorString(_e));            \
    }                                                                                          \
  } while (0)
```

### raftsql_amd/csrc/raftq_kernels.hpp

```cpp
#pragma once
#include <hip/hip_runtime.h>
#include <stdint.h>

#include <utility>

namespace raftqk {

typedef unsigned long long u64x2 __attribute__((ext_vector_type(2)));

constexpr int kBlock = 256;
constexpr int kWaves = kBlock / 64;
constexpr int kMaxPeers = 9;
constexpr int kTileMax = 2048;

struct SweepArgs {
  const uint64_t* match;
  const uint64_t* committed;
  uint64_t* committed_out;
  const uint64_t* first_idx;
  const uint8_t* votes;
  uint8_t* outcome;
  uint64_t* changed_bits;
  uint4* partials;
  uint64_t ld;
  const uint32_t* self_max = nullptr;
};

constexpr uint32_t kSelfMaxValid = 0x80000000u;

__device__ __forceinline__ void ce_desc(uint64_t& a, uint64_t& b) {
  const bool gt = a > b;
  const uint64_t hi = gt ? a : b;
  const uint64_t lo = gt ? b : a;
  a = hi;
  b = lo;
}

template <int N>
__device__ __forceinline__ uint64_t select_quorum_network(uint64_t (&v)[N]) {
#define CE(i, j) ce_desc(v[i], v[j])
  if constexpr (N == 2) { CE(0, 1); }
  if constexpr (N == 3) { CE(0, 2); CE(0, 1); CE(1, 2); }
  if constexpr (N == 4) { CE(0, 2); CE(1, 3); CE(0, 1); CE(2, 3); CE(1, 2); }
  if constexpr (N == 5) {
    CE(0, 3); CE(1, 4); CE(0, 2); CE(1, 3); CE(0, 1); CE(2, 4); CE(1, 2); CE(3, 4); CE(2, 3);
  }
  if constexpr (N == 6) {
    CE(0, 5); CE(1, 3); CE(2, 4); CE(1, 2); CE(3, 4); CE(0, 3);
    CE(2, 5); CE(0, 1); CE(2, 3); CE(4, 5); CE(1, 2); CE(3, 4);
  }
  if constexpr (N == 7) {
    CE(0, 6); CE(2, 3); CE(4, 5); CE(0, 2); CE(1, 4); CE(3, 6); CE(0, 1); CE(2, 5);
    CE(3, 4); CE(1, 2); CE(4, 6); CE(2, 3); CE(4, 5); CE(1, 2); CE(3, 4); CE(5, 6);
  }
  if constexpr (N == 8) {
    CE(0, 2); CE(1, 3); CE(4, 6); CE(5, 7); CE(0, 4); CE(1, 5); CE(2, 6); CE(3, 7); CE(0, 1); CE(2, 3);
    CE(4, 5); CE(6, 7); CE(2, 4); CE(3, 5); CE(1, 4); CE(3, 6); CE(1, 2); CE(3, 4); CE(5, 6);
  }
  if constexpr (N == 9) {
    CE(0, 3); CE(1, 7); CE(2, 5); CE(4, 8); CE(0, 7); CE(2, 4); CE(3, 8); CE(5, 6); CE(0, 2);
    CE(1, 3); CE(4, 5); CE(7, 8); CE(1, 4); CE(3, 6); CE(5, 7); CE(0, 1); CE(2, 4); CE(3, 5);
    CE(6, 8); CE(2, 3); CE(4, 5); CE(6, 7); CE(1, 2); CE(3, 4); CE(5, 6);
  }
#undef CE
  return v[N / 2];
}

template <int N>
__device__ __forceinline__ uint64_t select_other_network(uint64_t (&v)[N]) {
#define CE(i, j) ce_desc(v[i], v[j])
  if constexpr (N == 3) { CE(0, 1); }
  if constexpr (N == 4) { CE(0, 2); CE(0, 1); CE(1, 2); }
  if constexpr (N == 5) { CE(0, 2); CE(1, 3); CE(0, 1); CE(2, 3); CE(1, 2); }
  if constexpr (N == 6) {
    CE(0, 3); CE(1, 4); CE(0, 2); CE(1, 3); CE(0, 1); CE(2, 4); CE(1, 2); CE(3, 4); CE(2, 3);
  }
  if constexpr (N == 7) {
    CE(0, 5); CE(1, 3); CE(2, 4); CE(1, 2); CE(3, 4); CE(0, 3); CE(2, 5); CE(0, 1); CE(2, 3); CE(1, 2);
  }
  if constexpr (N == 8) {
    CE(0, 6); CE(2, 3); CE(4, 5); CE(0, 2); CE(1, 4); CE(3, 6); CE(0, 1);
    CE(2, 5); CE(3, 4); CE(1, 2); CE(4, 6); CE(2, 3); CE(4, 5); CE(3, 4);
  }
  if constexpr (N == 9) {
    CE(0, 2); CE(1, 3); CE(4, 6); CE(5, 7); CE(0, 4); CE(1, 5); CE(2, 6); CE(3, 7); CE(0, 1);
    CE(2, 3); CE(4, 5); CE(6, 7); CE(2, 4); CE(3, 5); CE(1, 4); CE(3, 6); CE(3, 4);
  }
#undef CE
  return v[N / 2 - 1];
}

template <int N>
__device__ __forceinline__ uint64_t select_quorum_oddeven(uint64_t (&v)[N]) {
#pragma unroll
  for (int r = 0; r < N; ++r) {
#pragma unroll
    for (int i = (r & 1); i + 1 < N; i += 2) ce_desc(v[i], v[i + 1]);
  }
  return v[N / 2];
}

template <bool GATED>
__device__ __forceinline__ uint64_t maybe_commit(uint64_t mci, uint64_t committed, uint64_t first_idx) {
  bool adv = mci > committed;
  if constexpr (GATED) adv = adv && (first_idx != 0) && (mci >= first_idx);
  return adv ? mci : committed;
}

__device__ __forceinline__ uint64_t bytes_equal(uint64_t v, uint64_t pattern) {
  const uint64_t k7f = 0x7f7f7f7f7f7f7f7full;
  const uint64_t x = v ^ pattern;
  uint64_t y = (x & k7f) + k7f;
  y = ~(y | x | k7f);
  return y >> 7;
}

__host__ __device__ constexpr int vote_word_bytes(int n_peers) { return n_peers <= 8 ? 2 : 4; }
typedef unsigned int u32x4p __attribute__((ext_vector_type(4)));

template <int N>
__device__ __forceinline__ uint32_t poll_word(uint32_t w) {
  constexpr uint32_t kLow = 0x55555555u & ((N >= 16) ? 0xffffffffu : ((1u << (2 * N)) - 1u));
  constexpr uint32_t q = N / 2 + 1;
  const uint32_t granted = __popc(w & ~(w >> 1) & kLow);
  const uint32_t rejected = __popc((w >> 1) & ~w & kLow);
  const uint32_t won = granted >= q ? 1u : 0u;
  const uint32_t lost = (won == 0u && rejected >= q) ? 2u : 0u;
  return won | lost;
}

template <typename T>
__device__ __forceinline__ T ld_stream(const T* p) {
  return __builtin_nontemporal_load(p);
}
template <typename T>
__device__ __forceinline__ void st_stream(T* p, T v) {
  __builtin_nontemporal_store(v, p);
}

#define RAFTQ_GLOBAL __attribute__((address_space(1)))
template <bool NT, typename T>
__device__ __forceinline__ T ldg(const T* p) {
  const RAFTQ_GLOBAL T* g = (const RAFTQ_GLOBAL T*)p;
  if constexpr (NT) return __builtin_nontemporal_load(g);
  else return *g;
}
template <bool NT, typename T>
__device__ __forceinline__ void stg(T* p, T v) {
  RAFTQ_GLOBAL T* g = (RAFTQ_GLOBAL T*)p;
  if constexpr (NT) __builtin_nontemporal_store(v, g);
  else *g = v;
}
typedef unsigned int u32x4 __attribute__((ext_vector_type(4)));
__device__ __forceinline__ void stg_u4(uint4* p, uint4 v) {
  u32x4 t;
  t.x = v.x; t.y = v.y; t.z = v.z; t.w = v.w;
  *(RAFTQ_GLOBAL u32x4*)p = t;
}

__device__ __forceinline__ uint32_t wave_sum_u32(uint32_t x) {
#pragma unroll
  for (int o = 32; o > 0; o >>= 1) x += __shfl_xor(x, o, 64);
  return x;
}

constexpr int kLdNT = 1, kStNT = 2, kNoStore = 4;
constexpr int kNoCompute = 8;

template <int N, int GPL, bool COMMIT, bool GATED, bool VOTES>
struct TileRegs {
  static constexpr int kRounds = GPL / 2;
  u64x2 m[COMMIT ? kRounds : 1][N];
  u64x2 c[COMMIT ? kRounds : 1];
  u64x2 f[COMMIT && GATED ? kRounds : 1];
  u32x4p vw[VOTES ? (N <= 8 ? 1 : 2) : 1];
  uint32_t skip = 0;
};

template <int N, bool COMMIT>
__device__ __forceinline__ uint32_t self_max_skip(const SweepArgs& a) {
  if constexpr (!COMMIT || N < 2) {
    return 0;
  } else {
    if (a.self_max == nullptr) return 0;
    const uint32_t w = __builtin_amdgcn_readfirstlane(ldg<false>(a.self_max));
    return (w & kSelfMaxValid) != 0 ? (w & 0xffu) + 1 : 0;
  }
}

template <int N, int GPL, bool COMMIT, bool GATED, bool VOTES, int POLICY, int BLOCK = kBlock, bool SKIP = false>
__device__ __forceinline__ void tile_load(TileRegs<N, GPL, COMMIT, GATED, VOTES>& r, const SweepArgs& a,
                                          const uint32_t tile) {
  constexpr bool NT = (POLICY & kLdNT) != 0;
  constexpr int kTile = BLOCK * GPL;
  constexpr int kRounds = GPL / 2;
  constexpr int kRows = SKIP && N >= 2 ? N - 1 : N;
  const uint32_t tid = threadIdx.x;
  const uint64_t tile0 = (uint64_t)tile * kTile;
  constexpr int kVoteLanes = kTile / 8;
  if constexpr (VOTES) {
    if (tid < kVoteLanes) {
      const uint8_t* src = a.votes + (tile0 + 8ull * tid) * vote_word_bytes(N);
      r.vw[0] = ldg<NT>(reinterpret_cast<const u32x4p*>(src));
      if constexpr (N > 8) r.vw[1] = ldg<NT>(reinterpret_cast<const u32x4p*>(src + 16));
    }
  }
  if constexpr (COMMIT) {
    const uint64_t* row[kRows];
#pragma unroll
    for (int p = 0; p < kRows; ++p) {
      const uint32_t slot = SKIP ? (uint32_t)p + ((uint32_t)p + 1 >= r.skip ? 1u : 0u) : (uint32_t)p;
      row[p] = a.match + (uint64_t)slot * a.ld;
    }
#pragma unroll
    for (int j = 0; j < kRounds; ++j) {
      const uint64_t g = tile0 + (uint64_t)(tid >> 6) * (64 * GPL) + (uint64_t)j * 128 + 2 * (tid & 63);
#pragma unroll
      for (int p = 0; p < kRows; ++p) {
        r.m[j][p] = ldg<NT>(reinterpret_cast<const u64x2*>(row[p] + g));
      }
      r.c[j] = ldg<NT>(reinterpret_cast<const u64x2*>(a.committed + g));
      if constexpr (GATED) r.f[j] = ldg<NT>(reinterpret_cast<const u64x2*>(a.first_idx + g));
    }
  }
}

template <int N, bool SKIP>
__device__ __forceinline__ uint64_t quorum_select(uint64_t (&v)[N]) {
  if constexpr (N == 1) return v[0];
  else if constexpr (SKIP) return select_other_network<N>(v);
  else return select_quorum_network<N>(v);
}

template <int N, int GPL, bool COMMIT, bool GATED, bool VOTES, int POLICY, bool BITS, int BLOCK = kBlock, bool SKIP = false>
__device__ __forceinline__ void tile_finish(const TileRegs<N, GPL, COMMIT, GATED, VOTES>& r, const SweepArgs& a,
                                            const uint32_t tile) {
  constexpr bool STNT = (POLICY & kStNT) != 0;
  constexpr bool NOSTORE = (POLICY & kNoStore) != 0;
  constexpr int kTile = BLOCK * GPL;
  constexpr int kWavesB = BLOCK / 64;
  constexpr int kRounds = GPL / 2;
  const uint32_t tid = threadIdx.x;
  const uint64_t tile0 = (uint64_t)tile * kTile;
  uint32_t n_changed = 0;
  uint32_t won_lost = 0;
  constexpr int kVoteLanes = kTile / 8;
  const bool vote_lane = VOTES && tid < kVoteLanes;

  if constexpr (COMMIT) {
#pragma unroll
    for (int j = 0; j < kRounds; ++j) {
      const uint64_t g = tile0 + (uint64_t)(tid >> 6) * (64 * GPL) + (uint64_t)j * 128 + 2 * (tid & 63);
      constexpr int kRows = SKIP && N >= 2 ? N - 1 : N;
      uint64_t v0[N], v1[N];
#pragma unroll
      for (int p = 0; p < kRows; ++p) {
        v0[p] = r.m[j][p].x;
        v1[p] = r.m[j][p].y;
      }
      uint64_t mci0, mci1;
      if constexpr ((POLICY & kNoCompute) != 0) {
        mci0 = v0[0];
        mci1 = v1[0];
#pragma unroll
        for (int p = 1; p < kRows; ++p) {
          mci0 ^= v0[p];
          mci1 ^= v1[p];
        }
      } else {
        mci0 = quorum_select<N, SKIP>(v0);
        mci1 = quorum_select<N, SKIP>(v1);
      }
      u64x2 o;
      if constexpr ((POLICY & kNoCompute) != 0) {
        o.x = mci0 ^ r.c[j].x;
        o.y = mci1 ^ r.c[j].y;
      } else {
        o.x = maybe_commit<GATED>(mci0, r.c[j].x, GATED ? r.f[j].x : 0);
        o.y = maybe_commit<GATED>(mci1, r.c[j].y, GATED ? r.f[j].y : 0);
      }
      const bool ch0 = o.x != r.c[j].x;
      const bool ch1 = o.y != r.c[j].y;
      const uint64_t b0 = __ballot(ch0);
      const uint64_t b1 = __ballot(ch1);
      n_changed += __popcll(b0) + __popcll(b1);
      if constexpr (BITS) {
        if (a.changed_bits != nullptr && (tid & 63) == 0) {
          u64x2 w;
          w.x = b0;
          w.y = b1;
          stg<false>(reinterpret_cast<u64x2*>(a.changed_bits + (g >> 6)), w);
        }
      }
      if constexpr (NOSTORE) {
        asm volatile("" ::"v"(o.x), "v"(o.y));
      } else {
        stg<STNT>(reinterpret_cast<u64x2*>(a.committed_out + g), o);
      }
    }
  }

  if constexpr (VOTES) {
    if (vote_lane) {
      const uint64_t g = tile0 + 8ull * tid;
      uint32_t out = 0, n_won = 0, n_lost = 0;
#pragma unroll
      for (int k = 0; k < 8; ++k) {
        uint32_t w;
        if constexpr (N <= 8) {
          const uint32_t pair = k < 2 ? r.vw[0].x : k < 4 ? r.vw[0].y : k < 6 ? r.vw[0].z : r.vw[0].w;
          w = (k & 1) ? pair >> 16 : pair & 0xffffu;
        } else {
          w = k == 0 ? r.vw[0].x : k == 1 ? r.vw[0].y : k == 2 ? r.vw[0].z : k == 3 ? r.vw[0].w
            : k == 4 ? r.vw[1].x : k == 5 ? r.vw[1].y : k == 6 ? r.vw[1].z : r.vw[1].w;
        }
        const uint32_t oc = poll_word<N>(w);
        out |= oc << (2 * k);
        n_won += oc & 1u;
        n_lost += oc >> 1;
      }
      uint16_t* dst = reinterpret_cast<uint16_t*>(a.outcome + (g >> 2));
      if constexpr (NOSTORE) {
        asm volatile("" ::"v"(out));
      } else {
        stg<STNT>(dst, (uint16_t)out);
      }
      won_lost = n_won | (n_lost << 16);
    }
  }

  const uint32_t wl = VOTES ? wave_sum_u32(won_lost) : 0u;
  if ((tid & 63) == 0) {
    uint4 t;
    t.x = n_changed;
    t.y = wl & 0xffffu;
    t.z = wl >> 16;
    t.w = 0;
    stg_u4(a.partials + ((uint64_t)tile * kWavesB + (tid >> 6)), t);
  }
}

template <int N, int GPL, bool COMMIT, bool GATED, bool VOTES, int POLICY, bool BITS, int BLOCK = kBlock>
__device__ __forceinline__ void sweep_tile(const SweepArgs& a, const uint32_t tile) {
  TileRegs<N, GPL, COMMIT, GATED, VOTES> r;
  r.skip = self_max_skip<N, COMMIT>(a);
  if (r.skip != 0) {
    tile_load<N, GPL, COMMIT, GATED, VOTES, POLICY, BLOCK, true>(r, a, tile);
    tile_finish<N, GPL, COMMIT, GATED, VOTES, POLICY, BITS, BLOCK, true>(r, a, tile);
  } else {
    tile_load<N, GPL, COMMIT, GATED, VOTES, POLICY, BLOCK>(r, a, tile);
    tile_finish<N, GPL, COMMIT, GATED, VOTES, POLICY, BITS, BLOCK>(r, a, tile);
  }
}

template <int N, int GPL, bool COMMIT, bool GATED, bool VOTES, int POLICY, bool BITS, int BLOCK = kBlock>
static __global__ __launch_bounds__(BLOCK) void sweep_kernel(SweepArgs a) {
  sweep_tile<N, GPL, COMMIT, GATED, VOTES, POLICY, BITS, BLOCK>(a, blockIdx.x);
}

template <int N, int GPL, bool COMMIT, bool GATED, bool VOTES, int POLICY, bool BITS, int BLOCK = kBlock>
static __global__ __launch_bounds__(BLOCK) void sweep_set_kernel(const SweepArgs* __restrict__ tab, uint32_t want_bits) {
  SweepArgs a = tab[blockIdx.y];
  if (!want_bits) a.changed_bits = nullptr;
  sweep_tile<N, GPL, COMMIT, GATED, VOTES, POLICY, BITS, BLOCK>(a, blockIdx.x);
}

template <int N, int GPL, bool COMMIT, bool GATED, bool VOTES, int POLICY, bool BITS, int MINW = 1>
static __global__ __launch_bounds__(kBlock, MINW) void sweep_persist_kernel(const SweepArgs* __restrict__ tab,
                                                                      uint32_t tiles_per_member, uint32_t total_tiles,
                                                                      uint32_t want_bits) {
  using Regs = TileRegs<N, GPL, COMMIT, GATED, VOTES>;
  const uint32_t stride = gridDim.x;
  uint32_t t = blockIdx.x;
  if (t >= total_tiles) return;
  auto locate = [&](uint32_t lin, SweepArgs& a, uint32_t& tile) {
    const uint32_t m = lin / tiles_per_member;
    tile = lin - m * tiles_per_member;
    a = tab[m];
    if (!want_bits) a.changed_bits = nullptr;
  };
  auto load = [&](Regs& r, const SweepArgs& a, uint32_t tile) {
    r.skip = self_max_skip<N, COMMIT>(a);
    if (r.skip != 0) tile_load<N, GPL, COMMIT, GATED, VOTES, POLICY, kBlock, true>(r, a, tile);
    else tile_load<N, GPL, COMMIT, GATED, VOTES, POLICY>(r, a, tile);
  };
  auto finish = [&](const Regs& r, const SweepArgs& a, uint32_t tile) {
    if (r.skip != 0) tile_finish<N, GPL, COMMIT, GATED, VOTES, POLICY, BITS, kBlock, true>(r, a, tile);
    else tile_finish<N, GPL, COMMIT, GATED, VOTES, POLICY, BITS>(r, a, tile);
  };
  Regs A, B;
  SweepArgs aA, aB;
  uint32_t tileA, tileB;
  locate(t, aA, tileA);
  load(A, aA, tileA);
  while (true) {
    t += stride;
    if (t >= total_tiles) {
      finish(A, aA, tileA);
      break;
    }
    locate(t, aB, tileB);
    load(B, aB, tileB);
    finish(A, aA, tileA);
    t += stride;
    if (t >= total_tiles) {
      finish(B, aB, tileB);
      break;
    }
    locate(t, aA, tileA);
    load(A, aA, tileA);
    finish(B, aB, tileB);
  }
}

static __global__ __launch_bounds__(kBlock) void set_counts_kernel(const SweepArgs* __restrict__ tab,
                                                                    const uint64_t* __restrict__ n_partials_of,
                                                                    uint64_t* __restrict__ out) {
  __shared__ uint64_t red[3][kWaves];
  const uint4* p = tab[blockIdx.x].partials;
  const uint64_t n_partials = n_partials_of[blockIdx.x];
  uint64_t c = 0, w = 0, l = 0;
  for (uint64_t i = threadIdx.x; i < n_partials; i += kBlock) {
    const uint4 v = p[i];
    c += v.x;
    w += v.y;
    l += v.z;
  }
#pragma unroll
  for (int o = 32; o > 0; o >>= 1) {
    c += __shfl_xor(c, o, 64);
    w += __shfl_xor(w, o, 64);
    l += __shfl_xor(l, o, 64);
  }
  if ((threadIdx.x & 63) == 0) {
    red[0][threadIdx.x >> 6] = c;
    red[1][threadIdx.x >> 6] = w;
    red[2][threadIdx.x >> 6] = l;
  }
  __syncthreads();
  if (threadIdx.x < 3) {
    uint64_t t = 0;
    for (int k = 0; k < kWaves; ++k) t += red[threadIdx.x][k];
    out[(uint64_t)blockIdx.x * 4 + threadIdx.x] = t;
  }
  if (threadIdx.x == 3) out[(uint64_t)blockIdx.x * 4 + 3] = 0;
}

typedef __attribute__((address_space(3))) void lds_void_t;
typedef const __attribute__((address_space(1))) void global_cvoid_t;

template <int N, int GPL, bool GATED, bool VOTES, bool BITS>
static __global__ __launch_bounds__(kBlock) void sweep_lds_kernel(SweepArgs a) {
  constexpr int kTile = kBlock * GPL;
  constexpr int kRounds = GPL / 2;
  constexpr int kRows = N + 1 + (GATED ? 1 : 0);
  constexpr int kRowBytes = 64 * 16;
  extern __shared__ __attribute__((aligned(16))) unsigned char smem[];
  const uint32_t tid = threadIdx.x;
  const uint32_t lane = tid & 63;
  const uint32_t wave = tid >> 6;
  unsigned char* wbase = smem + (size_t)wave * (kRounds * kRows * kRowBytes);
  const uint64_t tile0 = (uint64_t)blockIdx.x * kTile;
  uint32_t n_changed = 0;
  uint32_t won_lost = 0;

#pragma unroll
  for (int j = 0; j < kRounds; ++j) {
    const uint64_t g = tile0 + (uint64_t)(tid >> 6) * (64 * GPL) + (uint64_t)j * 128 + 2 * (tid & 63);
    unsigned char* rbase = wbase + (size_t)j * kRows * kRowBytes;
#pragma unroll
// ... 44 lines not shown
  }

  if constexpr (VOTES) {
    constexpr int kVoteLanes = kTile / 8;
    if (tid < kVoteLanes) {
      const uint64_t g = tile0 + 8ull * tid;
      const uint8_t* src = a.votes + g * vote_word_bytes(N);
      uint32_t words[8];
      if constexpr (N <= 8) {
        const u32x4p v = *reinterpret_cast<const u32x4p*>(src);
        const uint32_t pr[4] = {v.x, v.y, v.z, v.w};
#pragma unroll
        for (int k = 0; k < 8; ++k) words[k] = (k & 1) ? pr[k >> 1] >> 16 : pr[k >> 1] & 0xffffu;
      } else {
        const u32x4p v0 = *reinterpret_cast<const u32x4p*>(src), v1 = *reinterpret_cast<const u32x4p*>(src + 16);
        words[0] = v0.x; words[1] = v0.y; words[2] = v0.z; words[3] = v0.w;
        words[4] = v1.x; words[5] = v1.y; words[6] = v1.z; words[7] = v1.w;
      }
      uint32_t out = 0, n_won = 0, n_lost = 0;
#pragma unroll
      for (int k = 0; k < 8; ++k) {
        const uint32_t oc = poll_word<N>(words[k]);
        out |= oc << (2 * k);
        n_won += oc & 1u;
        n_lost += oc >> 1;
      }
      *reinterpret_cast<uint16_t*>(a.outcome + (g >> 2)) = (uint16_t)out;
      won_lost = n_won | (n_lost << 16);
    }
  }
  const uint32_t wl = VOTES ? wave_sum_u32(won_lost) : 0u;
  if (lane == 0) {
    uint4 r;
    r.x = n_changed;
    r.y = wl & 0xffffu;
    r.z = wl >> 16;
    r.w = 0;
    a.partials[(uint64_t)blockIdx.x * kWaves + wave] = r;
  }
}

struct DeltaRec {
  uint64_t group, match;
  uint32_t peer, pad;
};
struct Delta16Rec {
  uint64_t match;
  uint32_t group, peer;
};
struct VoteDeltaRec {
  uint64_t group;
  uint32_t peer;
  uint8_t vote, pad[3];
};

constexpr unsigned long long kNoEpoch = ~0ull;
__device__ __forceinline__ bool batch_is_bad(const unsigned long long* bad, unsigned long long epoch_match,
                                             unsigned long long epoch_votes) {
  return bad[0] == epoch_match || bad[1] == epoch_votes;
}

static __global__ __launch_bounds__(kBlock) void self_max_check_kernel(const uint64_t* __restrict__ match, uint64_t ld,
                                                                       uint64_t n_groups, uint32_t n_peers, uint32_t slot,
                                                                       uint32_t* word) {
  bool broken = false;
  for (uint64_t g = (uint64_t)blockIdx.x * kBlock + threadIdx.x; g < n_groups; g += (uint64_t)gridDim.x * kBlock) {
    const uint64_t own = match[(uint64_t)slot * ld + g];
    for (uint32_t p = 0; p < n_peers; ++p) broken |= match[(uint64_t)p * ld + g] > own;
  }
  if (__ballot(broken) != 0 && (threadIdx.x & 63) == 0) *word = 0u;
}

__device__ __forceinline__ bool breaks_self_max(uint32_t w, const uint64_t* match, uint64_t ld, uint64_t group, uint32_t peer,
                                                uint64_t value) {
  if ((w & kSelfMaxValid) == 0) return false;
  const uint32_t slot = w & 0xffu;
  return peer != slot && value > match[(uint64_t)slot * ld + group];
}
__device__ __forceinline__ void clear_self_max_if(bool broken, uint32_t* word) {
  const uint64_t b = __ballot(broken);
  if (b != 0 && (threadIdx.x & 63) == (uint32_t)(__ffsll((unsigned long long)b) - 1)) *word = 0u;
}

template <typename Rec>
static __global__ __launch_bounds__(kBlock) void deltas_in_kernel(const Rec* __restrict__ src, Rec* __restrict__ dst,
                                                                  uint64_t n, uint64_t n_groups, uint32_t n_peers,
                                                                  unsigned long long* bad_epoch, uint64_t* bad_host,
                                                                  unsigned long long epoch) {
  const uint64_t i = (uint64_t)blockIdx.x * kBlock + threadIdx.x;
  bool bad = false;
  if (i < n) {
    const Rec r = src[i];
    dst[i] = r;
    bad = r.group >= n_groups || r.peer >= n_peers;
  }
  if (__ballot(bad) != 0 && (threadIdx.x & 63) == 0) {
    atomicMax(bad_epoch, epoch);
    *bad_host = epoch;
  }
}

template <typename Rec>
static __global__ __launch_bounds__(kBlock) void deltas_in_apply_kernel(const Rec* __restrict__ src, uint64_t n, uint64_t* match,
                                                                        uint64_t ld, uint64_t n_groups, uint32_t n_peers,
                                                                        unsigned long long* bad_epoch, uint64_t* bad_host,
                                                                        unsigned long long epoch, uint32_t* self_max) {
  const uint64_t i = (uint64_t)blockIdx.x * kBlock + threadIdx.x;
  const uint32_t w = *self_max;
  bool bad = false, broken = false;
  if (i < n) {
    const Rec r = src[i];
    bad = r.group >= n_groups || r.peer >= n_peers;
    if (!bad) {
      broken = breaks_self_max(w, match, ld, r.group, r.peer, r.match);
      atomicMax(reinterpret_cast<unsigned long long*>(match + (uint64_t)r.peer * ld + r.group), (unsigned long long)r.match);
    }
  }
  clear_self_max_if(broken, self_max);
  if (__ballot(bad) != 0 && (threadIdx.x & 63) == 0) {
    atomicMax(bad_epoch, epoch);
    *bad_host = epoch;
  }
}

template <typename Rec>
static __global__ __launch_bounds__(kBlock) void apply_deltas_kernel(uint64_t* match, uint64_t ld,
                                                              const Rec* __restrict__ d, uint64_t n,
                                                              const unsigned long long* bad,
                                                              unsigned long long epoch_match, unsigned long long epoch_votes,
                                                              uint32_t* self_max) {
  if (batch_is_bad(bad, epoch_match, epoch_votes)) return;
  const uint64_t i = (uint64_t)blockIdx.x * kBlock + threadIdx.x;
  const uint32_t w = *self_max;
  bool broken = false;
  if (i < n) {
    const Rec r = d[i];
    broken = breaks_self_max(w, match, ld, r.group, r.peer, r.match);
    atomicMax(reinterpret_cast<unsigned long long*>(match + (uint64_t)r.peer * ld + r.group),
              (unsigned long long)r.match);
  }
  clear_self_max_if(broken, self_max);
}

struct TermDeltaRec {
  uint64_t group, cur_term, first_idx_cur_term;
};
static __global__ __launch_bounds__(kBlock) void apply_term_deltas_kernel(uint64_t* first_idx,
                                                                   const TermDeltaRec* __restrict__ d, uint64_t n) {
  const uint64_t i = (uint64_t)blockIdx.x * kBlock + threadIdx.x;
  if (i >= n) return;
  const TermDeltaRec r = d[i];
  first_idx[r.group] = r.cur_term == 0 ? 0ull : r.first_idx_cur_term;
}

static __global__ __launch_bounds__(kBlock) void vote_deltas_in_kernel(const VoteDeltaRec* __restrict__ src,
                                                                       VoteDeltaRec* __restrict__ dst, uint64_t n,
                                                                       uint64_t n_groups, uint32_t n_peers,
                                                                       unsigned long long* bad_epoch, uint64_t* bad_host,
                                                                       unsigned long long epoch) {
  const uint64_t i = (uint64_t)blockIdx.x * kBlock + threadIdx.x;
  bool bad = false;
  if (i < n) {
    const VoteDeltaRec r = src[i];
    dst[i] = r;
    bad = r.group >= n_groups || r.peer >= n_peers || (unsigned)(r.vote - 1) > 1u;
  }
  if (__ballot(bad) != 0 && (threadIdx.x & 63) == 0) {
    atomicMax(bad_epoch, epoch);
    *bad_host = epoch;
  }
}

__device__ __forceinline__ bool vote_rec_ok(const VoteDeltaRec& r, uint64_t n_groups, uint32_t n_peers) {
  return r.group < n_groups && r.peer < n_peers && (unsigned)(r.vote - 1) <= 1u;
}

static __global__ __launch_bounds__(kBlock) void vote_claim_kernel(uint32_t* claim, uint64_t ld,
                                                            const VoteDeltaRec* __restrict__ d, uint64_t n,
                                                            const unsigned long long* bad, unsigned long long epoch_match,
                                                            unsigned long long epoch_votes, uint64_t n_groups,
                                                            uint32_t n_peers, int each) {
  if (!each && batch_is_bad(bad, epoch_match, epoch_votes)) return;
  const uint64_t i = (uint64_t)blockIdx.x * kBlock + threadIdx.x;
  if (i >= n) return;
  const VoteDeltaRec r = d[i];
  if (each && !vote_rec_ok(r, n_groups, n_peers)) return;
  atomicMin(claim + (uint64_t)r.peer * ld + r.group, (uint32_t)i);
}

static __global__ __launch_bounds__(kBlock) void vote_apply_kernel(uint8_t* votes, int wide, uint32_t* claim, uint64_t ld,
                                                            const VoteDeltaRec* __restrict__ d, uint64_t n,
                                                            const unsigned long long* bad, unsigned long long epoch_match,
                                                            unsigned long long epoch_votes, uint64_t n_groups,
                                                            uint32_t n_peers, int each) {
  if (!each && batch_is_bad(bad, epoch_match, epoch_votes)) return;
  const uint64_t i = (uint64_t)blockIdx.x * kBlock + threadIdx.x;
  if (i >= n) return;
  const VoteDeltaRec r = d[i];
  if (each && !vote_rec_ok(r, n_groups, n_peers)) return;
  const uint64_t slot = (uint64_t)r.peer * ld + r.group;
  if (claim[slot] != (uint32_t)i) return;
  unsigned int* word = reinterpret_cast<unsigned int*>(votes) + (wide ? r.group : r.group >> 1);
  const unsigned sh = (wide ? 0u : (unsigned)(r.group & 1ull) * 16u) + 2u * r.peer;
  const unsigned nv = (unsigned)r.vote << sh;
  unsigned old = *word;
  while (true) {
    const unsigned cur = (old >> sh) & 3u;
    if (cur == 1u || cur == 2u) break;
    const unsigned seen = atomicCAS(word, old, (old & ~(3u << sh)) | nv);
    if (seen == old) break;
    old = seen;
  }
  claim[slot] = 0xffffffffu;
}

struct Advance {
  uint64_t group, old_commit, new_commit;
};
struct Advance16 {
  uint64_t new_commit;
  uint32_t group, advanced_by;
};
__device__ __forceinline__ Advance make_advance(Advance*, uint64_t g, uint64_t o, uint64_t n) { return Advance{g, o, n}; }
__device__ __forceinline__ Advance16 make_advance(Advance16*, uint64_t g, uint64_t o, uint64_t n) {
// ... 41 lines not shown
    for (uint64_t i = lo; i < hi; ++i) {
      offsets[i] = run;
      run += p32[i * 4];
    }
  }
  if (tid == 1023) *total = pre + incl;
}

template <int GPL, typename Adv>
static __global__ __launch_bounds__(kBlock) void compact_changed_kernel(const uint64_t* changed_bits,
                                                                 const uint4* __restrict__ partials,
                                                                 const uint64_t* old_commit,
                                                                 const uint64_t* new_commit,
                                                                 Adv* out, uint64_t cap, uint64_t* total,
                                                                 const uint64_t* __restrict__ wave_offsets) {
  constexpr int kTile = kBlock * GPL;
  constexpr int kRounds = GPL / 2;
  __shared__ uint64_t red[kWaves];
  __shared__ uint32_t mine[kWaves];
  const uint32_t tid = threadIdx.x, lane = tid & 63, wave = tid >> 6;
  const uint64_t first_wave = (uint64_t)blockIdx.x * kWaves;
  const uint32_t* cnt = reinterpret_cast<const uint32_t*>(partials);
  uint64_t acc = 0;
  if (wave_offsets == nullptr) {
    uint32_t a0 = 0, a1 = 0, a2 = 0, a3 = 0;
    uint64_t i = tid;
    for (; i + 3 * kBlock < first_wave; i += 4 * kBlock) {
      a0 += cnt[4 * i];
      a1 += cnt[4 * (i + kBlock)];
      a2 += cnt[4 * (i + 2 * kBlock)];
      a3 += cnt[4 * (i + 3 * kBlock)];
    }
    for (; i < first_wave; i += kBlock) a0 += cnt[4 * i];
    acc = (uint64_t)a0 + a1 + a2 + a3;
#pragma unroll
    for (int o = 32; o > 0; o >>= 1) acc += __shfl_xor(acc, o, 64);
  } else if (lane == 0 && wave == 0) {
    acc = wave_offsets[first_wave];
  }
  if (lane == 0) red[wave] = acc;
  if (tid < kWaves) mine[tid] = cnt[4 * (first_wave + tid)];
  __syncthreads();
  uint64_t pos = 0;
#pragma unroll
  for (int k = 0; k < kWaves; ++k) pos += red[k];
  if (blockIdx.x == gridDim.x - 1 && tid == 0) {
    uint64_t t = pos;
    for (int k = 0; k < kWaves; ++k) t += mine[k];
    *total = t;
  }
  for (uint32_t k = 0; k < wave; ++k) pos += mine[k];
  const uint64_t below = lane == 0 ? 0ull : (~0ull >> (64 - lane));
#pragma unroll
  for (int j = 0; j < kRounds; ++j) {
    const uint64_t g0 = (uint64_t)blockIdx.x * kTile + (uint64_t)wave * (64 * GPL) + (uint64_t)j * 128;
    const uint64_t b0 = changed_bits[(g0 >> 6)];
    const uint64_t b1 = changed_bits[(g0 >> 6) + 1];
    const bool e = (b0 >> lane) & 1, o = (b1 >> lane) & 1;
    const uint64_t rank = __popcll(b0 & below) + __popcll(b1 & below);
    if (e) {
      const uint64_t g = g0 + 2 * lane, s = pos + rank;
      if (s < cap) out[s] = make_advance((Adv*)nullptr, g, old_commit[g], new_commit[g]);
    }
    if (o) {
      const uint64_t g = g0 + 2 * lane + 1, s = pos + rank + (e ? 1 : 0);
      if (s < cap) out[s] = make_advance((Adv*)nullptr, g, old_commit[g], new_commit[g]);
    }
    pos += __popcll(b0) + __popcll(b1);
  }
}

static __global__ void raise_flag_kernel(uint64_t* flag, uint64_t epoch) {
  if (threadIdx.x == 0 && blockIdx.x == 0) __hip_atomic_store(flag, epoch, __ATOMIC_RELAXED, __HIP_MEMORY_SCOPE_SYSTEM);
}

template <int N, int GPL, bool GATED, int POLICY>
static __global__ __launch_bounds__(kBlock) void sweep_segments_kernel(SweepArgs a, Advance16* list, unsigned int* counts_host, unsigned int* counts_dev) {
  constexpr bool STNT = (POLICY & kStNT) != 0;
  constexpr int kTile = kBlock * GPL;
  constexpr int kRounds = GPL / 2;
  __shared__ uint32_t wave_cnt[kWaves];
  const uint32_t tid = threadIdx.x, lane = tid & 63, wave = tid >> 6, tile = blockIdx.x;
  TileRegs<N, GPL, true, GATED, false> r;
  r.skip = self_max_skip<N, true>(a);
  if (r.skip != 0) tile_load<N, GPL, true, GATED, false, POLICY, kBlock, true>(r, a, tile);
  else tile_load<N, GPL, true, GATED, false, POLICY>(r, a, tile);
  const uint64_t tile0 = (uint64_t)tile * kTile;
  u64x2 nw[kRounds];
  uint64_t even[kRounds], odd[kRounds];
  uint32_t n_changed = 0;
#pragma unroll
  for (int j = 0; j < kRounds; ++j) {
    const uint64_t g = tile0 + (uint64_t)wave * (64 * GPL) + (uint64_t)j * 128 + 2 * lane;
    uint64_t v0[N], v1[N];
#pragma unroll
    for (int p = 0; p < N; ++p) {
      v0[p] = r.m[j][p].x;
      v1[p] = r.m[j][p].y;
    }
    uint64_t mci0, mci1;
    if (r.skip != 0) {
      mci0 = quorum_select<N, true>(v0);
      mci1 = quorum_select<N, true>(v1);
    } else {
      mci0 = quorum_select<N, false>(v0);
      mci1 = quorum_select<N, false>(v1);
    }
    u64x2 o;
    o.x = maybe_commit<GATED>(mci0, r.c[j].x, GATED ? r.f[j].x : 0);
    o.y = maybe_commit<GATED>(mci1, r.c[j].y, GATED ? r.f[j].y : 0);
    even[j] = __ballot(o.x != r.c[j].x);
    odd[j] = __ballot(o.y != r.c[j].y);
    n_changed += __popcll(even[j]) + __popcll(odd[j]);
    nw[j] = o;
    if (a.changed_bits != nullptr && lane == 0) {
      u64x2 w;
      w.x = even[j];
      w.y = odd[j];
      stg<false>(reinterpret_cast<u64x2*>(a.changed_bits + (g >> 6)), w);
    }
    stg<STNT>(reinterpret_cast<u64x2*>(a.committed_out + g), o);
  }
  if (lane == 0) {
    uint4 t;
    t.x = n_changed;
    t.y = t.z = t.w = 0;
    stg_u4(a.partials + ((uint64_t)tile * kWaves + wave), t);
    wave_cnt[wave] = n_changed;
  }
  __syncthreads();
  uint64_t pos = tile0;
  for (uint32_t k = 0; k < wave; ++k) pos += wave_cnt[k];
  if (tid == 0) {
    uint32_t tile_cnt = 0;
#pragma unroll
    for (int k = 0; k < kWaves; ++k) tile_cnt += wave_cnt[k];
    counts_host[tile] = tile_cnt;
    counts_dev[tile] = tile_cnt;
  }
  const uint64_t below = lane == 0 ? 0ull : (~0ull >> (64 - lane));
#pragma unroll
  for (int j = 0; j < kRounds; ++j) {
    const uint64_t g0 = tile0 + (uint64_t)wave * (64 * GPL) + (uint64_t)j * 128;
    const bool e = (even[j] >> lane) & 1, o = (odd[j] >> lane) & 1;
    const uint64_t rank = __popcll(even[j] & below) + __popcll(odd[j] & below);
    if (e) list[pos + rank] = make_advance((Advance16*)nullptr, g0 + 2 * lane, r.c[j].x, nw[j].x);
    if (o) list[pos + rank + (e ? 1 : 0)] = make_advance((Advance16*)nullptr, g0 + 2 * lane + 1, r.c[j].y, nw[j].y);
    pos += __popcll(even[j]) + __popcll(odd[j]);
  }
}

static __global__ __launch_bounds__(kBlock) void raise_flag_segments_kernel(uint64_t* flag, uint32_t epoch, const unsigned int* counts_dev, uint32_t n_tiles) {
  __shared__ uint32_t red[kWaves];
  uint32_t acc = 0;
  for (uint32_t i = threadIdx.x; i < n_tiles; i += kBlock) acc += counts_dev[i];
#pragma unroll
  for (int o = 32; o > 0; o >>= 1) acc += __shfl_xor(acc, o, 64);
  if ((threadIdx.x & 63) == 0) red[threadIdx.x >> 6] = acc;
  __syncthreads();
  if (threadIdx.x == 0) {
    uint32_t total = 0;
#pragma unroll
    for (int k = 0; k < kWaves; ++k) total += red[k];
    __hip_atomic_store(flag, ((uint64_t)epoch << 32) | total, __ATOMIC_RELAXED, __HIP_MEMORY_SCOPE_SYSTEM);
  }
}

struct VoterSweepArgs {
  SweepArgs s;
  const uint16_t* voters;
};

__device__ __forceinline__ uint64_t sel_u64(bool c, uint64_t a, uint64_t b) { return c ? a : b; }

template <int N, int... I>
__device__ __forceinline__ uint64_t pick_sorted(const uint64_t (&v)[N], uint32_t idx, std::integer_sequence<int, I...>) {
  uint64_t r = v[0];
  ((r = sel_u64(idx == (uint32_t)(I + 1), v[I + 1], r)), ...);
  return r;
}
template <int N, int... I>
__device__ __forceinline__ void zero_non_voters(uint64_t (&v)[N], uint32_t mask, std::integer_sequence<int, I...>) {
  ((v[I] = sel_u64(((mask >> I) & 1u) != 0, v[I], 0ull)), ...);
}

template <int N>
__device__ __forceinline__ uint64_t select_quorum_voters(uint64_t (&v)[N], uint32_t mask) {
  zero_non_voters<N>(v, mask, std::make_integer_sequence<int, N>{});
  if constexpr (N >= 2) (void)select_quorum_network<N>(v);
// ... 42 lines not shown
      const uint64_t g = tile0 + (uint64_t)(tid >> 6) * (64 * GPL) + (uint64_t)j * 128 + 2 * (tid & 63);
      cmask[j] = ldg<NT>(reinterpret_cast<const uint32_t*>(va.voters + g));
    }
  }

  uint32_t n_changed = 0;
  uint32_t won_lost = 0;
  if constexpr (COMMIT) {
#pragma unroll
    for (int j = 0; j < kRounds; ++j) {
      const uint64_t g = tile0 + (uint64_t)(tid >> 6) * (64 * GPL) + (uint64_t)j * 128 + 2 * (tid & 63);
      uint64_t v0[N], v1[N];
#pragma unroll
      for (int p = 0; p < N; ++p) {
        v0[p] = r.m[j][p].x;
        v1[p] = r.m[j][p].y;
      }
      const uint64_t mci0 = select_quorum_voters<N>(v0, cmask[j] & 0xffffu);
      const uint64_t mci1 = select_quorum_voters<N>(v1, cmask[j] >> 16);
      u64x2 o;
      o.x = maybe_commit<GATED>(mci0, r.c[j].x, GATED ? r.f[j].x : 0);
      o.y = maybe_commit<GATED>(mci1, r.c[j].y, GATED ? r.f[j].y : 0);
      const uint64_t b0 = __ballot(o.x != r.c[j].x);
      const uint64_t b1 = __ballot(o.y != r.c[j].y);
      n_changed += __popcll(b0) + __popcll(b1);
      if (a.changed_bits != nullptr && (tid & 63) == 0) {
        u64x2 w;
        w.x = b0;
        w.y = b1;
        stg<false>(reinterpret_cast<u64x2*>(a.changed_bits + (g >> 6)), w);
      }
      stg<STNT>(reinterpret_cast<u64x2*>(a.committed_out + g), o);
    }
  }

  if constexpr (VOTES) {
    if (vote_lane) {
      const uint64_t g = tile0 + 8ull * tid;
      uint32_t out = 0, n_won = 0, n_lost = 0;
#pragma unroll
      for (int k = 0; k < 8; ++k) {
        uint32_t w;
        if constexpr (N <= 8) {
          const uint32_t pair = k < 2 ? r.vw[0].x : k < 4 ? r.vw[0].y : k < 6 ? r.vw[0].z : r.vw[0].w;
          w = (k & 1) ? pair >> 16 : pair & 0xffffu;
        } else {
          w = k == 0 ? r.vw[0].x : k == 1 ? r.vw[0].y : k == 2 ? r.vw[0].z : k == 3 ? r.vw[0].w
            : k == 4 ? r.vw[1].x : k == 5 ? r.vw[1].y : k == 6 ? r.vw[1].z : r.vw[1].w;
        }
        const uint32_t mpair = k < 2 ? vmask.x : k < 4 ? vmask.y : k < 6 ? vmask.z : vmask.w;
        const uint32_t oc = poll_word_voters(w, (k & 1) ? mpair >> 16 : mpair & 0xffffu);
        out |= oc << (2 * k);
        n_won += oc & 1u;
        n_lost += oc >> 1;
      }
      stg<STNT>(reinterpret_cast<uint16_t*>(a.outcome + (g >> 2)), (uint16_t)out);
      won_lost = n_won | (n_lost << 16);
    }
  }

  const uint32_t wl = VOTES ? wave_sum_u32(won_lost) : 0u;
  if ((tid & 63) == 0) {
    uint4 t;
    t.x = n_changed;
    t.y = wl & 0xffffu;
    t.z = wl >> 16;
    t.w = 0;
    stg_u4(a.partials + ((uint64_t)tile * kWaves + (tid >> 6)), t);
  }
}

static __global__ __launch_bounds__(kBlock) void fill_voters_kernel(uint16_t* voters, uint64_t n_groups, uint16_t full) {
  const uint64_t g = (uint64_t)blockIdx.x * kBlock + threadIdx.x;
  if (g < n_groups) voters[g] = full;
}

struct VoterDeltaRec {
  uint64_t group;
  uint16_t voters, reset;
  uint32_t pad;
};
static __global__ __launch_bounds__(kBlock) void apply_voter_deltas_kernel(uint16_t* voters, uint64_t* match, uint64_t ld, uint8_t* votes,
                                                                           int wide, uint32_t n_peers, const VoterDeltaRec* __restrict__ d,
                                                                           uint64_t n, uint32_t* self_max) {
  const uint64_t i = (uint64_t)blockIdx.x * kBlock + threadIdx.x;
  bool resets = false;
  if (i < n) {
    const VoterDeltaRec r = d[i];
    voters[r.group] = r.voters;
    resets = r.reset != 0;
    if (resets) {
      const uint32_t fields = spread_even(r.reset) * 3u;
      for (uint32_t p = 0; p < n_peers; ++p)
        if ((r.reset >> p) & 1u) match[(uint64_t)p * ld + r.group] = 0ull;
      if (wide) reinterpret_cast<uint32_t*>(votes)[r.group] &= ~fields;
      else reinterpret_cast<uint16_t*>(votes)[r.group] &= (uint16_t)~fields;
    }
  }
  clear_self_max_if(resets, self_max);
}

struct TickArgs {
  const uint8_t* role;
  uint32_t* elapsed;
  uint8_t* action;
  uint64_t* hup_bits;
  uint64_t* beat_bits;
  uint4* partials;
  uint64_t n_groups;
  uint64_t seed, tick_no;
  uint32_t election_tick, heartbeat_tick;
  uint32_t et_magic;
};

__device__ __forceinline__ uint64_t tick_key(uint64_t seed, uint64_t tick_no) {
  uint64_t z = seed ^ (tick_no * 0xD1B54A32D192ED03ull);
  z += 0x9E3779B97F4A7C15ull;
  z = (z ^ (z >> 30)) * 0xBF58476D1CE4E5B9ull;
  z = (z ^ (z >> 27)) * 0x94D049BB133111EBull;
  return z ^ (z >> 31);
}
__device__ __forceinline__ uint32_t tick_rand(uint64_t key, uint32_t group ) {
  uint32_t x = group ^ (uint32_t)key;
  x ^= x >> 16;
  x *= 0x85EBCA6Bu;
  x ^= x >> 13;
  x *= 0xC2B2AE35u;
  x ^= x >> 16;
  return x ^ (uint32_t)(key >> 32);
}

__device__ __forceinline__ uint32_t tick_mod(uint32_t x, uint32_t d, uint32_t magic) {
  uint32_t r = x - __umulhi(x, magic) * d;
  r = r >= d ? r - d : r;
  return r >= d ? r - d : r;
}

template <int L>
__device__ __forceinline__ uint32_t write_lane(uint32_t v, uint32_t x ) {
  asm("v_writelane_b32 %0, %1, %2" : "+v"(v) : "s"(x), "n"(L));
  return v;
}

__device__ __forceinline__ void tick_chunk_out(const TickArgs& a, uint64_t chunk , uint32_t lane, const uint64_t (&hb)[4],
                                               const uint64_t (&bb)[4], uint32_t n_hup, uint32_t n_beat) {
  uint32_t v = 0;
  v = write_lane<0>(v, (uint32_t)hb[0]);  v = write_lane<1>(v, (uint32_t)(hb[0] >> 32));
  v = write_lane<2>(v, (uint32_t)hb[1]);  v = write_lane<3>(v, (uint32_t)(hb[1] >> 32));
  v = write_lane<4>(v, (uint32_t)hb[2]);  v = write_lane<5>(v, (uint32_t)(hb[2] >> 32));
  v = write_lane<6>(v, (uint32_t)hb[3]);  v = write_lane<7>(v, (uint32_t)(hb[3] >> 32));
  v = write_lane<8>(v, (uint32_t)bb[0]);  v = write_lane<9>(v, (uint32_t)(bb[0] >> 32));
  v = write_lane<10>(v, (uint32_t)bb[1]); v = write_lane<11>(v, (uint32_t)(bb[1] >> 32));
  v = write_lane<12>(v, (uint32_t)bb[2]); v = write_lane<13>(v, (uint32_t)(bb[2] >> 32));
  v = write_lane<14>(v, (uint32_t)bb[3]); v = write_lane<15>(v, (uint32_t)(bb[3] >> 32));
  v = write_lane<16>(v, n_hup);
  v = write_lane<17>(v, n_beat);
  const uint64_t at_hup = (uint64_t)(uintptr_t)a.hup_bits + chunk * 32 + 4ull * lane;
  const uint64_t at_beat = (uint64_t)(uintptr_t)a.beat_bits + chunk * 32 + 4ull * lane - 32;
  const uint64_t at_part = (uint64_t)(uintptr_t)a.partials + chunk * 16 + 4ull * lane - 64;
  const uint64_t at = lane < 8 ? at_hup : (lane < 16 ? at_beat : at_part);
  if (lane < 20) stg<false>(reinterpret_cast<uint32_t*>((uintptr_t)at), v);
}

template <int R, bool NT = false>
__device__ __forceinline__ void tick_tile(const TickArgs& a, uint64_t n_blocks) {
  const uint32_t tid = threadIdx.x, lane = tid & 63, wave = tid >> 6;
  const uint64_t key = tick_key(a.seed, a.tick_no);
  uint32_t roles[R];
  uint4 el[R];
#pragma unroll
  for (int r = 0; r < R; ++r) {
    const uint64_t blk = (uint64_t)blockIdx.x * R + r;
    if (blk < n_blocks) {
      const uint64_t g = (blk * kBlock + tid) * 4;
      roles[r] = ldg<NT>(reinterpret_cast<const uint32_t*>(a.role + g));
      const u32x4 v = ldg<NT>(reinterpret_cast<const u32x4*>(a.elapsed + g));
      el[r].x = v.x; el[r].y = v.y; el[r].z = v.z; el[r].w = v.w;
    }
  }
#pragma unroll
  for (int r = 0; r < R; ++r) {
    const uint64_t blk = (uint64_t)blockIdx.x * R + r;
// ... 361 lines not shown
```

### raftsql_amd/csrc/raftq_step_kernels.hpp

```cpp
#pragma once
#include <hip/hip_runtime.h>
#include <stdint.h>

#include "raftq_kernels.hpp"

namespace raftqk {

struct MsgRec {
  uint64_t group, term, log_term, index, commit, reject_hint;
  uint32_t from;
  uint8_t type, reject, pad[2];
  uint64_t resv;
};
struct StepOutRec {
  uint64_t group, term, index, log_term, commit, last_index;
  uint32_t to, vote, lead;
  uint8_t type, reject, flags, role;
};
struct LogDeltaRec {
  uint64_t group, last_index, last_term, commit_to;
};
struct StepOutC {
  uint64_t term, index, commit, aux;
  uint8_t vote, lead, type, reject, flags, role, pad[2];
// ... 144 lines not shown
}

static __global__ __launch_bounds__(kBlock) void step_keys_kernel(const MsgRec* __restrict__ msgs,
                                                                  uint64_t* __restrict__ keys,
                                                                  uint32_t* __restrict__ order, uint64_t n,
                                                                  uint64_t n_groups, uint32_t n_peers,
                                                                  unsigned int* bad, bool msg_flags, uint8_t recs,
                                                                  void* __restrict__ out, uint8_t compact) {
  const uint64_t i = (uint64_t)blockIdx.x * kBlock + threadIdx.x;
  bool is_bad = false;
  if (i < n) {
    const RecClass c = classify(msgs[i], n_groups, n_peers, msg_flags, recs);
    is_bad = c == kBad;
    keys[i] = c == kTake ? msgs[i].group : c == kSkip ? n_groups : 0;
    order[i] = (uint32_t)i;
    if (c == kSkip) put_skipped(out, i, compact);
  }
  if (__ballot(is_bad) != 0 && (threadIdx.x & 63) == 0) atomicOr(bad, 1u);
}

constexpr uint32_t kMaxRun = 32;
constexpr uint32_t kNil = 0xffffffffu;

template <bool MASKED>
struct NodeT {
  const NodeArrays& a;
  uint64_t g;
  uint64_t term, last_index, last_term, committed, first_idx;
  uint64_t mt[kMaxPeers];
  uint32_t mt_dirty = 0;
  uint32_t vote, lead;
  uint32_t vw = 0;
  uint32_t lst_head, lst_cnt, lst_min;
  uint8_t role;
  bool held = false;
  bool at_tail = false, host_owns = false;
  uint64_t committed0, first_idx0;
  uint8_t role0;
  bool vw_known = false, vw_dirty = false, elapsed_reset = false;
  uint32_t vmask = 0;

  __device__ NodeT(const NodeArrays& arr, uint64_t group, const uint16_t* voters = nullptr) : a(arr), g(group) {
    if constexpr (MASKED) vmask = voters[g];
    const NodeRec r = a.rec[g];
    term = r.term; last_index = r.last_index; last_term = r.last_term;
    vote = r.vote; lead = r.lead;
    lst_head = r.lst_head; lst_cnt = r.lst_cnt; lst_min = r.lst_min;
    committed = committed0 = r.committed;
    first_idx = first_idx0 = r.first_idx;
    role = role0 = r.role;
#pragma unroll
    for (int p = 0; p < kMaxPeers; ++p) mt[p] = r.match[p];
    if (a.at_tail != nullptr) at_tail = ((a.at_tail[g >> 6] >> (g & 63)) & 1ull) != 0;
  }
  __device__ void store(bool list_reset = true) const {
    NodeRec r;
    r.term = term; r.last_index = last_index; r.last_term = last_term;
    r.vote = (uint8_t)vote; r.lead = (uint8_t)lead;
    r.role = role; r.pad = 0;
    r.lst_head = list_reset ? kNil : lst_head;
    r.lst_cnt = list_reset ? 0u : lst_cnt;
    r.lst_min = list_reset ? kNil : lst_min;
    r.committed = committed;
    r.first_idx = first_idx;
#pragma unroll
    for (int p = 0; p < kMaxPeers; ++p) r.match[p] = mt[p];
    a.rec[g] = r;
    if (committed != committed0) a.committed[g] = committed;
    if (role != role0) a.role[g] = role;
    if (first_idx != first_idx0) a.first_idx[g] = first_idx;
#pragma unroll
    for (int p = 0; p < kMaxPeers; ++p)
      if ((mt_dirty >> p) & 1u) a.match[(uint64_t)p * a.ld + g] = mt[p];
    if (mt_dirty != 0 && a.self_max != nullptr) {
      const uint32_t w = *a.self_max;
      if ((w & kSelfMaxValid) != 0) {
        const uint64_t own = match(w & 0xffu);
        bool broken = false;
#pragma unroll
        for (uint32_t p = 0; p < (uint32_t)kMaxPeers; ++p) broken |= p < a.n_peers && mt[p] > own;
        if (broken) *a.self_max = 0u;
      }
    }
    if (elapsed_reset) a.elapsed[g] = 0;
    if (vw_dirty) {
      if (a.n_peers <= 8) reinterpret_cast<uint16_t*>(a.votes)[g] = (uint16_t)vw;
      else reinterpret_cast<uint32_t*>(a.votes)[g] = vw;
    }
  }
  __device__ void set_first_idx(uint64_t v) { first_idx = v; }
  __device__ uint64_t get_first_idx() const { return first_idx; }
  __device__ void set_votes(uint32_t w) {
    vw = w;
    vw_known = vw_dirty = true;
  }
  __device__ uint32_t get_votes() {
    if (!vw_known) {
      vw = a.n_peers <= 8 ? (uint32_t)reinterpret_cast<const uint16_t*>(a.votes)[g] : reinterpret_cast<const uint32_t*>(a.votes)[g];
      vw_known = true;
    }
    return vw;
  }
  __device__ uint64_t match(uint32_t p) const {
    uint64_t v = 0;
#pragma unroll
    for (uint32_t k = 0; k < (uint32_t)kMaxPeers; ++k) v = k == p ? mt[k] : v;
    return v;
  }
  __device__ void set_match(uint32_t p, uint64_t v) {
#pragma unroll
    for (uint32_t k = 0; k < (uint32_t)kMaxPeers; ++k) mt[k] = k == p ? v : mt[k];
    mt_dirty |= 1u << p;
  }
  __device__ uint32_t quorum() const {
    if constexpr (MASKED) return ((uint32_t)__popc(vmask) >> 1) + 1u;
    else return a.n_peers / 2 + 1;
  }
  __device__ bool counts(uint32_t p, uint32_t n) const {
    if constexpr (MASKED) return ((vmask >> p) & 1u) != 0;
    else return p < n;
  }

  __device__ void reset(uint64_t t) {
    if (term != t) { term = t; vote = 0; }
    lead = 0;
    elapsed_reset = true;
    set_votes(0);
#pragma unroll
    for (uint32_t p = 0; p < (uint32_t)kMaxPeers; ++p)
      if (p < a.n_peers) {
        const uint64_t v = p == a.self ? last_index : 0;
        if (mt[p] != v) mt_dirty |= 1u << p;
        mt[p] = v;
      }
  }
  __device__ void become_follower(uint64_t t, uint32_t new_lead) {
    reset(t);
    lead = new_lead;
    role = kFollower;
    set_first_idx(0);
  }
  __device__ void become_candidate() {
    reset(term + 1);
    vote = a.self + 1;
    role = kCandidate;
    set_first_idx(0);
  }
  __device__ bool maybe_commit() {
    uint64_t m[kMaxPeers];
    const uint32_t n = a.n_peers, q = quorum();
#pragma unroll
    for (uint32_t p = 0; p < kMaxPeers; ++p) m[p] = counts(p, n) ? mt[p] : 0;
    uint64_t mci = 0;
#pragma unroll
    for (uint32_t c = 0; c < kMaxPeers; ++c) {
      uint32_t ge = 0;
#pragma unroll
      for (uint32_t p = 0; p < kMaxPeers; ++p) ge += (counts(p, n) && m[p] >= m[c]) ? 1u : 0u;
      if (counts(c, n) && ge >= q && m[c] > mci) mci = m[c];
    }
    if (mci > committed) {
      const uint64_t fi = get_first_idx();
      if (fi != 0 && mci >= fi) {
        committed = mci;
        return true;
      }
// ... 293 lines not shown
```

### raftsql_amd/engine.py

```python
from __future__ import annotations

import ctypes as C
from dataclasses import dataclass
from typing import Optional

import numpy as np

from . import _lib
from ._lib import (SWEEP_CACHED, SWEEP_CHANGED, SWEEP_COMMIT, SWEEP_GATED, SWEEP_LDS, SWEEP_NO_ADOPT,
                   SWEEP_STREAM, SWEEP_VOTES, Advance, Counts, Delta, RaftqError, VoteDelta)

__all__ = ["QuorumEngine", "SweepSet", "sweep_many_async", "SweepCounts", "device_count", "RaftqError", "pinned_empty", "pinned_copy", "SWEEP_COMMIT", "SWEEP_GATED",
           "SWEEP_VOTES", "SWEEP_NO_ADOPT", "SWEEP_LDS", "SWEEP_CHANGED", "SWEEP_STREAM", "SWEEP_CACHED"]


@dataclass
class SweepCounts:
    n_changed: int
    n_won: int
    n_lost: int


def device_count() -> int:
    lib = _lib.load()
# ... 259 lines not shown
        self._chk(self._lib.raftq_last_advances(self._h, C.byref(p), C.byref(n)))
        if n.value == 0:
            return np.empty(0, dtype=self._ADV_DT)
        buf = (C.c_char * (n.value * self._ADV_DT.itemsize)).from_address(p.value)
        return np.frombuffer(buf, dtype=self._ADV_DT, count=n.value)

    def cycle_inplace(self, flags: int, deltas: Optional[np.ndarray], vote_deltas: Optional[np.ndarray],
                      cap: int):
        nd = 0 if deltas is None else len(deltas)
        nv = 0 if vote_deltas is None else len(vote_deltas)
        n = C.c_uint64(0)
        self._chk(self._lib.raftq_cycle(
            self._h, _ptr(deltas) if nd else None, nd, _ptr(vote_deltas) if nv else None, nv, flags,
            None, int(cap), C.byref(n), None))
        return int(n.value)

    def cycle(self, flags: int, deltas: Optional[np.ndarray] = None, vote_deltas: Optional[np.ndarray] = None,
              cap: Optional[int] = None, out: Optional[np.ndarray] = None, want_counts: bool = True):
        nd = 0 if deltas is None else len(deltas)
        nv = 0 if vote_deltas is None else len(vote_deltas)
        if nd:
            assert deltas.dtype == self._DELTA_DT and deltas.flags.c_contiguous
        if nv:
            assert vote_deltas.dtype == self._VDELTA_DT and vote_deltas.flags.c_contiguous
        cap = (self.n_groups if cap is None else int(cap))
        if out is None:
            out = np.empty(cap, dtype=self._ADV_DT)
        n = C.c_uint64(0)
        c = Counts()
        self._chk(self._lib.raftq_cycle(
            self._h, _ptr(deltas) if nd else None, nd, _ptr(vote_deltas) if nv else None, nv, flags,
            _ptr(out) if cap else None, cap, C.byref(n), C.byref(c) if want_counts else None))
        total = int(n.value)
        cnt = SweepCounts(int(c.n_changed), int(c.n_won), int(c.n_lost)) if want_counts else None
        return out[: min(total, cap)], total, cnt

    def step_async(self, flags: int) -> None:
        self._chk(self._lib.raftq_step_async(self._h, flags))

    def wait(self, want_counts: bool = False) -> Optional[SweepCounts]:
        if not want_counts:
            self._chk(self._lib.raftq_wait(self._h, None))
            return None
        c = Counts()
        self._chk(self._lib.raftq_wait(self._h, C.byref(c)))
        return SweepCounts(int(c.n_changed), int(c.n_won), int(c.n_lost))

    def sweep(self, flags: int) -> SweepCounts:
        self.step_async(flags)
        return self.wait(want_counts=True)

    def commit_advance(self, gated: bool = False):
        out = np.empty(self.n_groups, dtype=np.uint64)
        n = C.c_uint64(0)
        self._chk(self._lib.raftq_commit_advance(self._h, int(gated), _ptr(out), C.byref(n)))
        return out, int(n.value)

    def vote_tally(self):
        out = np.empty(self.n_groups, dtype=np.uint8)
        c = Counts()
        self._chk(self._lib.raftq_vote_tally(self._h, _ptr(out), C.byref(c)))
        return out, SweepCounts(int(c.n_changed), int(c.n_won), int(c.n_lost))

    def read_committed(self) -> np.ndarray:
        out = np.empty(self.n_groups, dtype=np.uint64)
        self._chk(self._lib.raftq_read_committed(self._h, _ptr(out)))
        return out

    def read_outcome(self) -> np.ndarray:
        out = np.empty(self.n_groups, dtype=np.uint8)
        self._chk(self._lib.raftq_read_outcome(self._h, _ptr(out)))
        return out

    def read_match(self) -> np.ndarray:
        out = np.empty((self.n_peers, self.n_groups), dtype=np.uint64)
        self._chk(self._lib.raftq_read_match(self._h, _ptr(out)))
        return out

    def self_max(self) -> int:
        s = C.c_int32(-1)
        self._chk(self._lib.raftq_self_max(self._h, C.byref(s)))
        return int(s.value)

    def read_votes(self) -> np.ndarray:
        out = np.empty((self.n_peers, self.n_groups), dtype=np.uint8)
        self._chk(self._lib.raftq_read_votes(self._h, _ptr(out)))
        return out

    def collect_changed(self, cap: Optional[int] = None):
        cap = self.n_groups if cap is None else int(cap)
        arr = (Advance * cap)()
        n = C.c_uint64(0)
        self._chk(self._lib.raftq_collect_changed(self._h, C.addressof(arr) if cap else None, cap, C.byref(n)))
        a = np.frombuffer(arr, dtype=np.dtype([("group", "<u8"), ("old_commit", "<u8"), ("new_commit", "<u8")]))
        return a[: min(int(n.value), cap)].copy(), int(n.value)

    def set_timers(self, election_tick: int = 10, heartbeat_tick: int = 1, seed: int = 0x1000) -> None:
        self._chk(self._lib.raftq_set_timers(self._h, election_tick, heartbeat_tick, seed))

    def load_roles(self, role: np.ndarray, elapsed: Optional[np.ndarray] = None) -> None:
        r = np.ascontiguousarray(role, dtype=np.uint8)
        if r.shape != (self.n_groups,):
            raise ValueError("role must be [G]")
        e = None if elapsed is None else np.ascontiguousarray(elapsed, dtype=np.uint32)
        self._chk(self._lib.raftq_load_roles(self._h, _ptr(r), _ptr(e) if e is not None else None))

    def tick(self, want_counts: bool = True):
        if not want_counts:
            self._chk(self._lib.raftq_tick(self._h, None))
            return None
        c = _lib.TickCounts()
        self._chk(self._lib.raftq_tick(self._h, C.byref(c)))
        return int(c.n_hup), int(c.n_beat)

    def read_tick(self):
        a = np.empty(self.n_groups, dtype=np.uint8)
        e = np.empty(self.n_groups, dtype=np.uint32)
        r = np.empty(self.n_groups, dtype=np.uint8)
        self._chk(self._lib.raftq_read_tick(self._h, _ptr(a), _ptr(e), _ptr(r)))
        return a, e, r

    def collect_hups(self, cap: Optional[int] = None):
        cap = self.n_groups if cap is None else int(cap)
        out = np.empty(cap, dtype=np.uint64)
        n = C.c_uint64(0)
        self._chk(self._lib.raftq_collect_hups(self._h, _ptr(out) if cap else None, cap, C.byref(n)))
        return out[: min(cap, int(n.value))], int(n.value)

    def collect_beats(self, cap: Optional[int] = None):
        cap = self.n_groups if cap is None else int(cap)
        out = np.empty(cap, dtype=np.uint64)
        n = C.c_uint64(0)
        self._chk(self._lib.raftq_collect_beats(self._h, _ptr(out) if cap else None, cap, C.byref(n)))
        return out[: min(cap, int(n.value))], int(n.value)

    def tick_collect(self, hup_cap: Optional[int] = None, beat_cap: Optional[int] = None):
        hc = self.n_groups if hup_cap is None else int(hup_cap)
        bc = self.n_groups if beat_cap is None else int(beat_cap)
        hups, beats = np.empty(hc, dtype=np.uint64), np.empty(bc, dtype=np.uint64)
        nh, nb = C.c_uint64(0), C.c_uint64(0)
        self._chk(self._lib.raftq_tick_collect(self._h, _ptr(hups) if hc else None, hc, C.byref(nh), _ptr(beats) if bc else None, bc,
                                               C.byref(nb)))
        return hups[: min(hc, int(nh.value))], int(nh.value), beats[: min(bc, int(nb.value))], int(nb.value)

    def tick_collect_lists(self, hup_cap: Optional[int] = None, beat_cap: Optional[int] = None, beat_bitmap: bool = False):
        hc = self.n_groups if hup_cap is None else int(hup_cap)
        bc = self.n_groups if beat_cap is None else int(beat_cap)
        nh, nb = C.c_uint64(0), C.c_uint64(0)
        self._chk(self._lib.raftq_tick_collect_lists(self._h, _lib.TICK_BEAT_BITMAP if beat_bitmap else 0, hc, bc, C.byref(nh), C.byref(nb)))
        ph, pb, pm = C.c_void_p(None), C.c_void_p(None), C.c_void_p(None)
        lh, lb, lm = C.c_uint64(0), C.c_uint64(0), C.c_uint64(0)
        self._chk(self._lib.raftq_last_tick_lists(self._h, C.byref(ph), C.byref(lh), C.byref(pb), C.byref(lb), C.byref(pm), C.byref(lm)))

        def view(p, n, dt):
            if not n:
                return np.empty(0, dtype=dt)
            return np.frombuffer((C.c_char * (int(n) * np.dtype(dt).itemsize)).from_address(p.value), dtype=dt)

        hups = view(ph, lh.value, np.uint32)
        second = view(pm, lm.value, np.uint64) if beat_bitmap else view(pb, lb.value, np.uint32)
        return hups, int(nh.value), second, int(nb.value)

    def campaign(self, groups, self_peer: int = 0) -> None:
        g = np.ascontiguousarray(groups, dtype=np.uint64)
        self._chk(self._lib.raftq_campaign(self._h, _ptr(g) if len(g) else None, len(g), self_peer))

# ... 93 lines not shown
```

Measured before the change: 121.1 billion.

## Add narrow 32-bit match offset mirror for commit quorum selection

Keeps a per-group 64-bit anchor (the minimum match) plus 32-bit per-peer offsets, built when match is loaded and updated by the delta-apply kernels. When a device-side valid word is set and N>=3, the commit sweep reads the 32-bit offsets instead of the 64-bit match rows and runs the sorting network on 32-bit values. This halves the bytes read per peer row and makes each compare-exchange cheaper. The cost is extra memory, atomicMax updates on deltas, invalidation paths whenever an offset would overflow, and a table refresh when the new buffers are first allocated.

Result: faster. 129.7 billion (median of 6 runs) (+7.1%).

```diff
diff --git a/go/raftq/engine_more.go b/go/raftq/engine_more.go
--- a/go/raftq/engine_more.go
+++ b/go/raftq/engine_more.go
@@ -18,6 +18,16 @@
 	}
 	return int(slot), nil
 }
+
+func (e *Engine) Narrow() (bool, error) {
+	var valid C.int32_t
+	if err := e.err(C.raftq_narrow(e.h, &valid)); err != nil {
+		return false, err
+	}
+	return valid != 0, nil
+}
+
+func (e *Engine) NarrowRebuild() error { return e.err(C.raftq_narrow_rebuild(e.h)) }
 
 func (e *Engine) SetStream(stream unsafe.Pointer) error { return e.err(C.raftq_set_stream(e.h, stream)) }
 func (e *Engine) Stream() unsafe.Pointer                { return C.raftq_get_stream(e.h) }
diff --git a/include/raftq.h b/include/raftq.h
--- a/include/raftq.h
+++ b/include/raftq.h
@@ -120,6 +120,8 @@
 int raftq_read_outcome(raftq_t* h, uint8_t* outcome_out );
 int raftq_read_match(raftq_t* h, uint64_t* match_out );
 int raftq_self_max(raftq_t* h, int32_t* slot_out);
+int raftq_narrow(raftq_t* h, int32_t* valid_out);
+int raftq_narrow_rebuild(raftq_t* h);
 int raftq_read_votes(raftq_t* h, uint8_t* votes_out );
 int raftq_collect_changed(raftq_t* h, raftq_advance_t* out, uint64_t cap, uint64_t* n);
 
diff --git a/raftsql_amd/_lib.py b/raftsql_amd/_lib.py
--- a/raftsql_amd/_lib.py
+++ b/raftsql_amd/_lib.py
@@ -78,6 +78,8 @@
     ("raftq_read_outcome", C.c_int, [_H, C.c_void_p]),
     ("raftq_read_match", C.c_int, [_H, C.c_void_p]),
     ("raftq_self_max", C.c_int, [_H, C.POINTER(C.c_int32)]),
+    ("raftq_narrow", C.c_int, [_H, C.POINTER(C.c_int32)]),
+    ("raftq_narrow_rebuild", C.c_int, [_H]),
     ("raftq_read_votes", C.c_int, [_H, C.c_void_p]),
     ("raftq_collect_changed", C.c_int, [_H, C.c_void_p, C.c_uint64, C.POINTER(C.c_uint64)]),
     ("raftq_set_timers", C.c_int, [_H, C.c_uint32, C.c_uint32, C.c_uint64]),
diff --git a/raftsql_amd/csrc/raftq_capi.hip b/raftsql_amd/csrc/raftq_capi.hip
--- a/raftsql_amd/csrc/raftq_capi.hip
+++ b/raftsql_amd/csrc/raftq_capi.hip
@@ -229,6 +229,30 @@
   const uint64_t blocks = std::min<uint64_t>((h->G + kBlock - 1) / kBlock, 4096);
   hipLaunchKernelGGL(self_max_check_kernel, dim3((unsigned)std::max<uint64_t>(blocks, 1)), dim3(kBlock), 0, h->stream,
                      (const uint64_t*)h->match, h->ld, h->G, h->N, h->self_peer, h->self_max);
+  HIPCHK(h, hipGetLastError());
+  return RAFTQ_OK;
+}
+int raftq_detail::narrow_build(raftq_t* h) {
+  if (int rc = use_device(h)) return rc;
+  if (h->narrow_off) return RAFTQ_OK;
+  if (h->step_collected != h->step_submitted) {
+    HIPCHK(h, hipMemsetAsync(h->narrow_word(), 0, sizeof(uint32_t), h->stream));
+    return RAFTQ_OK;
+  }
+  if (!h->anchor) {
+    const hipError_t e = raftq_buf::alloc_group({{(void**)&h->anchor, h->ld * sizeof(uint64_t)},
+                                                 {(void**)&h->moff, (size_t)h->N * h->ld * sizeof(uint32_t)}},
+                                                h->stream);
+    if (e != hipSuccess) {
+      (void)hipGetLastError();
+      return RAFTQ_OK;
+    }
+    if (h->in_set) h->in_set->tab_stale = true;
+  }
+  HIPCHK(h, hipMemsetD32Async((hipDeviceptr_t)h->narrow_word(), (int)kNarrowValid, 1, h->stream));
+  const uint64_t blocks = std::min<uint64_t>((h->G + kBlock - 1) / kBlock, 4096);
+  hipLaunchKernelGGL(narrow_build_kernel, dim3((unsigned)std::max<uint64_t>(blocks, 1)), dim3(kBlock), 0, h->stream,
+                     (const uint64_t*)h->match, h->ld, h->G, h->N, h->anchor, h->moff, h->narrow_word());
   HIPCHK(h, hipGetLastError());
   return RAFTQ_OK;
 }
@@ -341,6 +365,10 @@
       rc = fail(h, e == hipErrorOutOfMemory ? RAFTQ_ENOMEM : RAFTQ_EHIP, std::string("device arrays: ") + hipGetErrorString(e));
       break;
     }
+    {
+      const char* nr = std::getenv("RAFTQ_NARROW");
+      h->narrow_off = nr && std::strcmp(nr, "0") == 0;
+    }
     e = hipMemsetD32Async((hipDeviceptr_t)h->self_max, (int)(kSelfMaxValid | 0u), 1, h->stream);
     if (e != hipSuccess) { rc = fail(h, RAFTQ_EHIP, std::string("hipMemsetD32Async: ") + hipGetErrorString(e)); break; }
     e = raftq_buf::alloc_group({{(void**)&h->h_partials, h->max_partials * sizeof(uint4), raftq_buf::Kind::pinned},
@@ -387,7 +415,7 @@
   raftq_detail::free_node_state(h);
   raftq_detail::free_wire_state(h);
   raftq_buf::free_device(h->match, h->committed[0], h->committed[1], h->first_idx, h->votes, h->voters, h->outcome, h->changed_bits,
-                         h->partials, h->offsets, h->self_max, h->claim, h->delta_bad, h->role, h->elapsed, h->action, h->hup_bits,
+                         h->partials, h->offsets, h->self_max, h->anchor, h->moff, h->claim, h->delta_bad, h->role, h->elapsed, h->action, h->hup_bits,
                          h->beat_bits, h->tick_partials, h->tick_offsets2);
   raftq_buf::free_host(h->h_partials, h->h_total);
   if (h->ev0) (void)hipEventDestroy(h->ev0);
@@ -421,6 +449,7 @@
     for (uint32_t p = 0; p < h->N; ++p)
       HIPCHK(h, hipMemcpyAsync(h->match + (size_t)p * h->ld, match + (size_t)p * h->G, h->G * 8, hipMemcpyHostToDevice, h->stream));
     if (int rc = raftq_detail::self_max_check(h)) return rc;
+    if (int rc = raftq_detail::narrow_build(h)) return rc;
   }
   dense_changed(h);
   if (committed)
@@ -522,7 +551,7 @@
   if (n) dense_changed(h);
   if (n && trusted)
     hipLaunchKernelGGL((deltas_in_apply_kernel<Rec>), gm, dim3(kBlock), 0, h->stream, (const Rec*)h->ingest.d, n, h->match, h->ld,
-                       h->G, h->N, h->delta_bad, h->d_total + 1, em, h->self_max);
+                       h->G, h->N, h->delta_bad, h->d_total + 1, em, h->self_max, h->narrow_mirror());
   else if (n)
     hipLaunchKernelGGL((deltas_in_kernel<Rec>), gm, dim3(kBlock), 0, h->stream, (const Rec*)h->ingest.d, dev_m, n, h->G, h->N,
                        h->delta_bad, h->d_total + 1, em);
@@ -532,7 +561,7 @@
                        h->d_total + 2, ev);
   if (n && !trusted)
     hipLaunchKernelGGL((apply_deltas_kernel<Rec>), gm, dim3(kBlock), 0, h->stream, h->match, h->ld, (const Rec*)dev_m, n, bad, em,
-                       ev, h->self_max);
+                       ev, h->self_max, h->narrow_mirror());
   if (nv) {
     const unsigned long long em_gate = trusted ? kNoEpoch : em;
     hipLaunchKernelGGL(vote_claim_kernel, gv, dim3(kBlock), 0, h->stream, h->claim, h->ld, (const VoteDeltaRec*)dev_v, nv, bad,
@@ -683,7 +712,7 @@
   }
   dense_changed(h);
   hipLaunchKernelGGL(apply_voter_deltas_kernel, dim3((unsigned)((m + kBlock - 1) / kBlock)), dim3(kBlock), 0, h->stream, h->voters, h->match,
-                     h->ld, h->votes, h->N > 8 ? 1 : 0, h->N, (const VoterDeltaRec*)h->stage.d, m, h->self_max);
+                     h->ld, h->votes, h->N > 8 ? 1 : 0, h->N, (const VoterDeltaRec*)h->stage.d, m, h->self_max, h->narrow_word());
   HIPCHK(h, hipGetLastError());
   HIPCHK(h, hipStreamSynchronize(h->stream));
   return RAFTQ_OK;
@@ -720,6 +749,9 @@
   a.partials = h->partials;
   a.ld = h->ld;
   a.self_max = h->self_max;
+  a.narrow = h->anchor ? h->narrow_word() : nullptr;
+  a.anchor = h->anchor;
+  a.moff = h->moff;
   return a;
 }
 
@@ -859,6 +891,23 @@
   HIPCHK(h, hipMemcpyAsync(&w, h->self_max, sizeof w, hipMemcpyDeviceToHost, h->stream));
   HIPCHK(h, hipStreamSynchronize(h->stream));
   *slot = (w & kSelfMaxValid) ? (int32_t)(w & 0xffu) : -1;
+  return RAFTQ_OK;
+}
+
+int raftq_narrow(raftq_t* h, int32_t* valid) {
+  if (int rc = use_device_idle(h, "raftq_narrow")) return rc;
+  if (!valid) return fail(h, RAFTQ_EINVAL, "raftq_narrow: null argument");
+  uint32_t w = 0;
+  HIPCHK(h, hipMemcpyAsync(&w, h->narrow_word(), sizeof w, hipMemcpyDeviceToHost, h->stream));
+  HIPCHK(h, hipStreamSynchronize(h->stream));
+  *valid = w == kNarrowValid ? 1 : 0;
+  return RAFTQ_OK;
+}
+
+int raftq_narrow_rebuild(raftq_t* h) {
+  if (int rc = use_device_idle(h, "raftq_narrow_rebuild")) return rc;
+  if (int rc = raftq_detail::narrow_build(h)) return rc;
+  HIPCHK(h, hipStreamSynchronize(h->stream));
   return RAFTQ_OK;
 }
 
@@ -1723,6 +1772,13 @@
     footprint += sweep_footprint(h);
     if (h->cur != cur) cur = -1;
   }
+  if (s->tab_stale) {
+    for (int k = 0; k < 2; ++k) {
+      set_fill_table(s, k, s->tab_host);
+      SETCHK(s, hipMemcpy(s->tab[k], s->tab_host.data(), s->tab_host.size() * sizeof(SweepArgs), hipMemcpyHostToDevice));
+    }
+    s->tab_stale = false;
+  }
   const SweepArgs* tab = s->tab[cur < 0 ? 2 : cur];
   if (cur < 0) {
     set_fill_table(s, -1, s->tab_host);
@@ -1874,6 +1930,20 @@
   HIPCHK(dst, hipMemcpyAsync(dst->votes, src->votes, (size_t)vote_word_bytes((int)dst->N) * ld, hipMemcpyDeviceToDevice,
                              dst->stream));
   HIPCHK(dst, hipMemcpyAsync(dst->self_max, src->self_max, sizeof(uint32_t), hipMemcpyDeviceToDevice, dst->stream));
+  if (src->anchor && !dst->narrow_off && !dst->anchor) {
+    if (raftq_buf::alloc_group({{(void**)&dst->anchor, ld * sizeof(uint64_t), raftq_buf::Kind::device, nullptr, false},
+                                {(void**)&dst->moff, (size_t)dst->N * ld * sizeof(uint32_t), raftq_buf::Kind::device, nullptr, false}},
+                               dst->stream) != hipSuccess)
+      (void)hipGetLastError();
+    else if (dst->in_set) dst->in_set->tab_stale = true;
+  }
+  if (src->anchor && dst->anchor && !dst->narrow_off) {
+    HIPCHK(dst, hipMemcpyAsync(dst->anchor, src->anchor, ld * sizeof(uint64_t), hipMemcpyDeviceToDevice, dst->stream));
+    HIPCHK(dst, hipMemcpyAsync(dst->moff, src->moff, (size_t)dst->N * ld * sizeof(uint32_t), hipMemcpyDeviceToDevice, dst->stream));
+    HIPCHK(dst, hipMemcpyAsync(dst->narrow_word(), src->narrow_word(), sizeof(uint32_t), hipMemcpyDeviceToDevice, dst->stream));
+  } else {
+    HIPCHK(dst, hipMemsetAsync(dst->narrow_word(), 0, sizeof(uint32_t), dst->stream));
+  }
   if (src->voters) HIPCHK(dst, hipMemcpyAsync(dst->voters, src->voters, ld * sizeof(uint16_t), hipMemcpyDeviceToDevice, dst->stream));
   HIPCHK(dst, hipStreamSynchronize(dst->stream));
   dst->have_terms = src->have_terms;
diff --git a/raftsql_amd/csrc/raftq_internal.hpp b/raftsql_amd/csrc/raftq_internal.hpp
--- a/raftsql_amd/csrc/raftq_internal.hpp
+++ b/raftsql_amd/csrc/raftq_internal.hpp
@@ -51,6 +51,11 @@
   uint32_t seg_tiles = 0, seg_stride = 0, seg_one = 0;
   uint64_t flag_mask = ~0ull;
   uint32_t* self_max = nullptr;
+  uint64_t* anchor = nullptr;
+  uint32_t* moff = nullptr;
+  bool narrow_off = false;
+  uint32_t* narrow_word() const { return self_max + 1; }
+  raftqk::NarrowMirror narrow_mirror() const { return raftqk::NarrowMirror{self_max + 1, anchor, moff}; }
   uint64_t compact_epoch = 0;
   uint64_t compact_epoch_armed = 0;
   uint32_t flag_misses[2] = {0, 0}, flag_rested[2] = {0, 0};
@@ -180,6 +185,7 @@
   uint64_t* counts_h = nullptr;
   bool swept = false;
   bool broken = false;
+  bool tab_stale = false;
   unsigned last_flags = 0;
   int mode = 0;
   uint32_t persist_wgs = 0;
@@ -202,6 +208,7 @@
 int use_device_idle(raftq_t* h, const char* who);
 int refuse_voters(raftq_t* h, const char* who, bool step_family = false);
 int self_max_check(raftq_t* h);
+int narrow_build(raftq_t* h);
 int ensure_staging(raftq_t* h, size_t bytes);
 int ensure_ingest(raftq_t* h, size_t bytes);
 int ensure_tick_state(raftq_t* h);
diff --git a/raftsql_amd/csrc/raftq_kernels.hpp b/raftsql_amd/csrc/raftq_kernels.hpp
--- a/raftsql_amd/csrc/raftq_kernels.hpp
+++ b/raftsql_amd/csrc/raftq_kernels.hpp
@@ -24,20 +24,26 @@
   uint4* partials;
   uint64_t ld;
   const uint32_t* self_max = nullptr;
+  const uint32_t* narrow = nullptr;
+  const uint64_t* anchor = nullptr;
+  const uint32_t* moff = nullptr;
 };
 
 constexpr uint32_t kSelfMaxValid = 0x80000000u;
 
-__device__ __forceinline__ void ce_desc(uint64_t& a, uint64_t& b) {
+constexpr uint32_t kNarrowValid = 1u;
+
+template <typename T>
+__device__ __forceinline__ void ce_desc(T& a, T& b) {
   const bool gt = a > b;
-  const uint64_t hi = gt ? a : b;
-  const uint64_t lo = gt ? b : a;
+  const T hi = gt ? a : b;
+  const T lo = gt ? b : a;
   a = hi;
   b = lo;
 }
 
-template <int N>
-__device__ __forceinline__ uint64_t select_quorum_network(uint64_t (&v)[N]) {
+template <int N, typename T = uint64_t>
+__device__ __forceinline__ T select_quorum_network(T (&v)[N]) {
 #define CE(i, j) ce_desc(v[i], v[j])
   if constexpr (N == 2) { CE(0, 1); }
   if constexpr (N == 3) { CE(0, 2); CE(0, 1); CE(1, 2); }
@@ -177,6 +183,9 @@
   uint32_t skip = 0;
 };
 
+constexpr int kBodyAll = 0, kBodySkip = 1, kBodyNarrow = 2;
+constexpr uint32_t kSkipNarrow = 0x100u;
+
 template <int N, bool COMMIT>
 __device__ __forceinline__ uint32_t self_max_skip(const SweepArgs& a) {
   if constexpr (!COMMIT || N < 2) {
@@ -188,13 +197,28 @@
   }
 }
 
-template <int N, int GPL, bool COMMIT, bool GATED, bool VOTES, int POLICY, int BLOCK = kBlock, bool SKIP = false>
+template <int N, bool COMMIT>
+__device__ __forceinline__ uint32_t tile_body(const SweepArgs& a) {
+  const uint32_t skip = self_max_skip<N, COMMIT>(a);
+  if constexpr (!COMMIT || N < 3) {
+    return skip;
+  } else {
+    if (N < 5 && skip != 0) return skip;
+    if (a.narrow == nullptr) return skip;
+    const uint32_t w = __builtin_amdgcn_readfirstlane(ldg<false>(a.narrow));
+    return w == kNarrowValid ? kSkipNarrow : skip;
+  }
+}
+
+template <int N, int GPL, bool COMMIT, bool GATED, bool VOTES, int POLICY, int BLOCK = kBlock, int BODY = kBodyAll>
 __device__ __forceinline__ void tile_load(TileRegs<N, GPL, COMMIT, GATED, VOTES>& r, const SweepArgs& a,
                                           const uint32_t tile) {
   constexpr bool NT = (POLICY & kLdNT) != 0;
   constexpr int kTile = BLOCK * GPL;
   constexpr int kRounds = GPL / 2;
+  constexpr bool SKIP = BODY == kBodySkip;
   constexpr int kRows = SKIP && N >= 2 ? N - 1 : N;
+  static_assert(BODY != kBodyNarrow || N >= 3, "the narrow body is chosen from N = 3 (tile_body)");
   const uint32_t tid = threadIdx.x;
   const uint64_t tile0 = (uint64_t)tile * kTile;
   constexpr int kVoteLanes = kTile / 8;
@@ -215,9 +239,19 @@
 #pragma unroll
     for (int j = 0; j < kRounds; ++j) {
       const uint64_t g = tile0 + (uint64_t)(tid >> 6) * (64 * GPL) + (uint64_t)j * 128 + 2 * (tid & 63);
-#pragma unroll
-      for (int p = 0; p < kRows; ++p) {
-        r.m[j][p] = ldg<NT>(reinterpret_cast<const u64x2*>(row[p] + g));
+      if constexpr (BODY == kBodyNarrow) {
+#pragma unroll
+        for (int p = 0; p < N; ++p) {
+          const uint64_t w = ldg<NT>(reinterpret_cast<const uint64_t*>(a.moff + (uint64_t)p * a.ld + g));
+          if (p & 1) r.m[j][p >> 1].y = w;
+          else r.m[j][p >> 1].x = w;
+        }
+        r.m[j][N - 1] = ldg<NT>(reinterpret_cast<const u64x2*>(a.anchor + g));
+      } else {
+#pragma unroll
+        for (int p = 0; p < kRows; ++p) {
+          r.m[j][p] = ldg<NT>(reinterpret_cast<const u64x2*>(row[p] + g));
+        }
       }
       r.c[j] = ldg<NT>(reinterpret_cast<const u64x2*>(a.committed + g));
       if constexpr (GATED) r.f[j] = ldg<NT>(reinterpret_cast<const u64x2*>(a.first_idx + g));
@@ -232,7 +266,56 @@
   else return select_quorum_network<N>(v);
 }
 
-template <int N, int GPL, bool COMMIT, bool GATED, bool VOTES, int POLICY, bool BITS, int BLOCK = kBlock, bool SKIP = false>
+template <int N, int BODY, bool XOR, typename Regs>
+__device__ __forceinline__ void tile_mci(const Regs& r, const int j, uint64_t& mci0, uint64_t& mci1) {
+  if constexpr (BODY == kBodyNarrow) {
+    uint32_t v0[N], v1[N];
+#pragma unroll
+    for (int p = 0; p < N; ++p) {
+      const uint64_t w = (p & 1) ? r.m[j][p >> 1].y : r.m[j][p >> 1].x;
+      v0[p] = (uint32_t)w;
+      v1[p] = (uint32_t)(w >> 32);
+    }
+    uint32_t s0, s1;
+    if constexpr (XOR) {
+      s0 = v0[0];
+      s1 = v1[0];
+#pragma unroll
+      for (int p = 1; p < N; ++p) {
+        s0 ^= v0[p];
+        s1 ^= v1[p];
+      }
+    } else {
+      s0 = select_quorum_network<N, uint32_t>(v0);
+      s1 = select_quorum_network<N, uint32_t>(v1);
+    }
+    mci0 = r.m[j][N - 1].x + s0;
+    mci1 = r.m[j][N - 1].y + s1;
+  } else {
+    constexpr bool SKIP = BODY == kBodySkip;
+    constexpr int kRows = SKIP && N >= 2 ? N - 1 : N;
+    uint64_t v0[N], v1[N];
+#pragma unroll
+    for (int p = 0; p < kRows; ++p) {
+      v0[p] = r.m[j][p].x;
+      v1[p] = r.m[j][p].y;
+    }
+    if constexpr (XOR) {
+      mci0 = v0[0];
+      mci1 = v1[0];
+#pragma unroll
+      for (int p = 1; p < kRows; ++p) {
+        mci0 ^= v0[p];
+        mci1 ^= v1[p];
+      }
+    } else {
+      mci0 = quorum_select<N, SKIP>(v0);
+      mci1 = quorum_select<N, SKIP>(v1);
+    }
+  }
+}
+
+template <int N, int GPL, bool COMMIT, bool GATED, bool VOTES, int POLICY, bool BITS, int BLOCK = kBlock, int BODY = kBodyAll>
 __device__ __forceinline__ void tile_finish(const TileRegs<N, GPL, COMMIT, GATED, VOTES>& r, const SweepArgs& a,
                                             const uint32_t tile) {
   constexpr bool STNT = (POLICY & kStNT) != 0;
@@ -251,26 +334,8 @@
 #pragma unroll
     for (int j = 0; j < kRounds; ++j) {
       const uint64_t g = tile0 + (uint64_t)(tid >> 6) * (64 * GPL) + (uint64_t)j * 128 + 2 * (tid & 63);
-      constexpr int kRows = SKIP && N >= 2 ? N - 1 : N;
-      uint64_t v0[N], v1[N];
-#pragma unroll
-      for (int p = 0; p < kRows; ++p) {
-        v0[p] = r.m[j][p].x;
-        v1[p] = r.m[j][p].y;
-      }
       uint64_t mci0, mci1;
-      if constexpr ((POLICY & kNoCompute) != 0) {
-        mci0 = v0[0];
-        mci1 = v1[0];
-#pragma unroll
-        for (int p = 1; p < kRows; ++p) {
-          mci0 ^= v0[p];
-          mci1 ^= v1[p];
-        }
-      } else {
-        mci0 = quorum_select<N, SKIP>(v0);
-        mci1 = quorum_select<N, SKIP>(v1);
-      }
+      tile_mci<N, BODY, (POLICY & kNoCompute) != 0>(r, j, mci0, mci1);
       u64x2 o;
       if constexpr ((POLICY & kNoCompute) != 0) {
         o.x = mci0 ^ r.c[j].x;
@@ -343,10 +408,17 @@
 template <int N, int GPL, bool COMMIT, bool GATED, bool VOTES, int POLICY, bool BITS, int BLOCK = kBlock>
 __device__ __forceinline__ void sweep_tile(const SweepArgs& a, const uint32_t tile) {
   TileRegs<N, GPL, COMMIT, GATED, VOTES> r;
-  r.skip = self_max_skip<N, COMMIT>(a);
+  r.skip = tile_body<N, COMMIT>(a);
+  if constexpr (COMMIT && N >= 3) {
+    if (r.skip == kSkipNarrow) {
+      tile_load<N, GPL, COMMIT, GATED, VOTES, POLICY, BLOCK, kBodyNarrow>(r, a, tile);
+      tile_finish<N, GPL, COMMIT, GATED, VOTES, POLICY, BITS, BLOCK, kBodyNarrow>(r, a, tile);
+      return;
+    }
+  }
   if (r.skip != 0) {
-    tile_load<N, GPL, COMMIT, GATED, VOTES, POLICY, BLOCK, true>(r, a, tile);
-    tile_finish<N, GPL, COMMIT, GATED, VOTES, POLICY, BITS, BLOCK, true>(r, a, tile);
+    tile_load<N, GPL, COMMIT, GATED, VOTES, POLICY, BLOCK, kBodySkip>(r, a, tile);
+    tile_finish<N, GPL, COMMIT, GATED, VOTES, POLICY, BITS, BLOCK, kBodySkip>(r, a, tile);
   } else {
     tile_load<N, GPL, COMMIT, GATED, VOTES, POLICY, BLOCK>(r, a, tile);
     tile_finish<N, GPL, COMMIT, GATED, VOTES, POLICY, BITS, BLOCK>(r, a, tile);
@@ -380,12 +452,24 @@
     if (!want_bits) a.changed_bits = nullptr;
   };
   auto load = [&](Regs& r, const SweepArgs& a, uint32_t tile) {
-    r.skip = self_max_skip<N, COMMIT>(a);
-    if (r.skip != 0) tile_load<N, GPL, COMMIT, GATED, VOTES, POLICY, kBlock, true>(r, a, tile);
+    r.skip = tile_body<N, COMMIT>(a);
+    if constexpr (COMMIT && N >= 3) {
+      if (r.skip == kSkipNarrow) {
+        tile_load<N, GPL, COMMIT, GATED, VOTES, POLICY, kBlock, kBodyNarrow>(r, a, tile);
+        return;
+      }
+    }
+    if (r.skip != 0) tile_load<N, GPL, COMMIT, GATED, VOTES, POLICY, kBlock, kBodySkip>(r, a, tile);
     else tile_load<N, GPL, COMMIT, GATED, VOTES, POLICY>(r, a, tile);
   };
   auto finish = [&](const Regs& r, const SweepArgs& a, uint32_t tile) {
-    if (r.skip != 0) tile_finish<N, GPL, COMMIT, GATED, VOTES, POLICY, BITS, kBlock, true>(r, a, tile);
+    if constexpr (COMMIT && N >= 3) {
+      if (r.skip == kSkipNarrow) {
+        tile_finish<N, GPL, COMMIT, GATED, VOTES, POLICY, BITS, kBlock, kBodyNarrow>(r, a, tile);
+        return;
+      }
+    }
+    if (r.skip != 0) tile_finish<N, GPL, COMMIT, GATED, VOTES, POLICY, BITS, kBlock, kBodySkip>(r, a, tile);
     else tile_finish<N, GPL, COMMIT, GATED, VOTES, POLICY, BITS>(r, a, tile);
   };
   Regs A, B;
@@ -596,6 +680,44 @@
   if (b != 0 && (threadIdx.x & 63) == (uint32_t)(__ffsll((unsigned long long)b) - 1)) *word = 0u;
 }
 
+static __global__ __launch_bounds__(kBlock) void narrow_build_kernel(const uint64_t* __restrict__ match, uint64_t ld,
+                                                                     uint64_t n_groups, uint32_t n_peers,
+                                                                     uint64_t* __restrict__ anchor, uint32_t* __restrict__ moff,
+                                                                     uint32_t* word) {
+  bool broken = false;
+  for (uint64_t g = (uint64_t)blockIdx.x * kBlock + threadIdx.x; g < n_groups; g += (uint64_t)gridDim.x * kBlock) {
+    uint64_t lo = match[g], hi = lo;
+    for (uint32_t p = 1; p < n_peers; ++p) {
+      const uint64_t v = match[(uint64_t)p * ld + g];
+      lo = v < lo ? v : lo;
+      hi = v > hi ? v : hi;
+    }
+    anchor[g] = lo;
+    if (hi - lo > 0xffffffffull) {
+      broken = true;
+    } else {
+      for (uint32_t p = 0; p < n_peers; ++p) moff[(uint64_t)p * ld + g] = (uint32_t)(match[(uint64_t)p * ld + g] - lo);
+    }
+  }
+  if (__ballot(broken) != 0 && (threadIdx.x & 63) == 0) *word = 0u;
+}
+
+struct NarrowMirror {
+  uint32_t* word;
+  const uint64_t* anchor;
+  uint32_t* moff;
+};
+__device__ __forceinline__ bool narrow_follow(uint32_t w, const NarrowMirror& m, uint64_t ld, uint64_t group, uint32_t peer,
+                                              uint64_t value) {
+  if (w != kNarrowValid) return false;
+  const uint64_t base = m.anchor[group];
+  if (value < base) return false;
+  if (value - base > 0xffffffffull) return true;
+  atomicMax(m.moff + (uint64_t)peer * ld + group, (uint32_t)(value - base));
+  return false;
+}
+__device__ __forceinline__ void clear_narrow_if(bool broken, uint32_t* word) { clear_self_max_if(broken, word); }
+
 template <typename Rec>
 static __global__ __launch_bounds__(kBlock) void deltas_in_kernel(const Rec* __restrict__ src, Rec* __restrict__ dst,
                                                                   uint64_t n, uint64_t n_groups, uint32_t n_peers,
@@ -618,19 +740,23 @@
 static __global__ __launch_bounds__(kBlock) void deltas_in_apply_kernel(const Rec* __restrict__ src, uint64_t n, uint64_t* match,
                                                                         uint64_t ld, uint64_t n_groups, uint32_t n_peers,
                                                                         unsigned long long* bad_epoch, uint64_t* bad_host,
-                                                                        unsigned long long epoch, uint32_t* self_max) {
+                                                                        unsigned long long epoch, uint32_t* self_max,
+                                                                        NarrowMirror mirror) {
   const uint64_t i = (uint64_t)blockIdx.x * kBlock + threadIdx.x;
   const uint32_t w = *self_max;
-  bool bad = false, broken = false;
+  const uint32_t nw = *mirror.word;
+  bool bad = false, broken = false, wide = false;
   if (i < n) {
     const Rec r = src[i];
     bad = r.group >= n_groups || r.peer >= n_peers;
     if (!bad) {
       broken = breaks_self_max(w, match, ld, r.group, r.peer, r.match);
+      wide = narrow_follow(nw, mirror, ld, r.group, r.peer, r.match);
       atomicMax(reinterpret_cast<unsigned long long*>(match + (uint64_t)r.peer * ld + r.group), (unsigned long long)r.match);
     }
   }
   clear_self_max_if(broken, self_max);
+  clear_narrow_if(wide, mirror.word);
   if (__ballot(bad) != 0 && (threadIdx.x & 63) == 0) {
     atomicMax(bad_epoch, epoch);
     *bad_host = epoch;
@@ -642,18 +768,21 @@
                                                               const Rec* __restrict__ d, uint64_t n,
                                                               const unsigned long long* bad,
                                                               unsigned long long epoch_match, unsigned long long epoch_votes,
-                                                              uint32_t* self_max) {
+                                                              uint32_t* self_max, NarrowMirror mirror) {
   if (batch_is_bad(bad, epoch_match, epoch_votes)) return;
   const uint64_t i = (uint64_t)blockIdx.x * kBlock + threadIdx.x;
   const uint32_t w = *self_max;
-  bool broken = false;
+  const uint32_t nw = *mirror.word;
+  bool broken = false, wide = false;
   if (i < n) {
     const Rec r = d[i];
     broken = breaks_self_max(w, match, ld, r.group, r.peer, r.match);
+    wide = narrow_follow(nw, mirror, ld, r.group, r.peer, r.match);
     atomicMax(reinterpret_cast<unsigned long long*>(match + (uint64_t)r.peer * ld + r.group),
               (unsigned long long)r.match);
   }
   clear_self_max_if(broken, self_max);
+  clear_narrow_if(wide, mirror.word);
 }
 
 struct TermDeltaRec {
@@ -861,9 +990,15 @@
   __shared__ uint32_t wave_cnt[kWaves];
   const uint32_t tid = threadIdx.x, lane = tid & 63, wave = tid >> 6, tile = blockIdx.x;
   TileRegs<N, GPL, true, GATED, false> r;
-  r.skip = self_max_skip<N, true>(a);
-  if (r.skip != 0) tile_load<N, GPL, true, GATED, false, POLICY, kBlock, true>(r, a, tile);
-  else tile_load<N, GPL, true, GATED, false, POLICY>(r, a, tile);
+  r.skip = tile_body<N, true>(a);
+  const bool narrow = N >= 3 && r.skip == kSkipNarrow;
+  if (narrow) {
+    if constexpr (N >= 3) tile_load<N, GPL, true, GATED, false, POLICY, kBlock, kBodyNarrow>(r, a, tile);
+  } else if (r.skip != 0) {
+    tile_load<N, GPL, true, GATED, false, POLICY, kBlock, kBodySkip>(r, a, tile);
+  } else {
+    tile_load<N, GPL, true, GATED, false, POLICY>(r, a, tile);
+  }
   const uint64_t tile0 = (uint64_t)tile * kTile;
   u64x2 nw[kRounds];
   uint64_t even[kRounds], odd[kRounds];
@@ -871,19 +1006,13 @@
 #pragma unroll
   for (int j = 0; j < kRounds; ++j) {
     const uint64_t g = tile0 + (uint64_t)wave * (64 * GPL) + (uint64_t)j * 128 + 2 * lane;
-    uint64_t v0[N], v1[N];
-#pragma unroll
-    for (int p = 0; p < N; ++p) {
-      v0[p] = r.m[j][p].x;
-      v1[p] = r.m[j][p].y;
-    }
-    uint64_t mci0, mci1;
-    if (r.skip != 0) {
-      mci0 = quorum_select<N, true>(v0);
-      mci1 = quorum_select<N, true>(v1);
+    uint64_t mci0 = 0, mci1 = 0;
+    if (narrow) {
+      if constexpr (N >= 3) tile_mci<N, kBodyNarrow, false>(r, j, mci0, mci1);
+    } else if (r.skip != 0) {
+      tile_mci<N, kBodySkip, false>(r, j, mci0, mci1);
     } else {
-      mci0 = quorum_select<N, false>(v0);
-      mci1 = quorum_select<N, false>(v1);
+      tile_mci<N, kBodyAll, false>(r, j, mci0, mci1);
     }
     u64x2 o;
     o.x = maybe_commit<GATED>(mci0, r.c[j].x, GATED ? r.f[j].x : 0);
@@ -1092,7 +1221,7 @@
 };
 static __global__ __launch_bounds__(kBlock) void apply_voter_deltas_kernel(uint16_t* voters, uint64_t* match, uint64_t ld, uint8_t* votes,
                                                                            int wide, uint32_t n_peers, const VoterDeltaRec* __restrict__ d,
-                                                                           uint64_t n, uint32_t* self_max) {
+                                                                           uint64_t n, uint32_t* self_max, uint32_t* narrow) {
   const uint64_t i = (uint64_t)blockIdx.x * kBlock + threadIdx.x;
   bool resets = false;
   if (i < n) {
@@ -1108,6 +1237,7 @@
     }
   }
   clear_self_max_if(resets, self_max);
+  clear_narrow_if(resets, narrow);
 }
 
 struct TickArgs {
diff --git a/raftsql_amd/csrc/raftq_step_kernels.hpp b/raftsql_amd/csrc/raftq_step_kernels.hpp
--- a/raftsql_amd/csrc/raftq_step_kernels.hpp
+++ b/raftsql_amd/csrc/raftq_step_kernels.hpp
@@ -250,6 +250,7 @@
         if (broken) *a.self_max = 0u;
       }
     }
+    if (mt_dirty != 0 && a.self_max != nullptr && a.self_max[1] != 0u) a.self_max[1] = 0u;
     if (elapsed_reset) a.elapsed[g] = 0;
     if (vw_dirty) {
       if (a.n_peers <= 8) reinterpret_cast<uint16_t*>(a.votes)[g] = (uint16_t)vw;
diff --git a/raftsql_amd/engine.py b/raftsql_amd/engine.py
--- a/raftsql_amd/engine.py
+++ b/raftsql_amd/engine.py
@@ -365,6 +365,15 @@
         self._chk(self._lib.raftq_self_max(self._h, C.byref(s)))
         return int(s.value)
 
+    def narrow(self) -> bool:
+        v = C.c_int32(0)
+        self._chk(self._lib.raftq_narrow(self._h, C.byref(v)))
+        return bool(v.value)
+
+    def narrow_rebuild(self) -> bool:
+        self._chk(self._lib.raftq_narrow_rebuild(self._h))
+        return self.narrow()
+
     def read_votes(self) -> np.ndarray:
         out = np.empty((self.n_peers, self.n_groups), dtype=np.uint8)
         self._chk(self._lib.raftq_read_votes(self._h, _ptr(out)))
```
